# yell/boltzmann-machines

Hardware: AMD Instinct MI355X
Metric: Gibbs-steps/sec (CD-k, 784x1024 RBM, batch 512) (higher is better)
Workload: dtype f32

## Files before the change

### boltzmann_machines_amd/_ffi.py

```python
import ctypes as C
import os

import numpy as np

from . import build as _build

MAX_LAYERS = 4
UNIT_BERNOULLI, UNIT_GAUSSIAN, UNIT_MULTINOMIAL = 0, 1, 2


class Bm355Error(RuntimeError):
    pass


class RbmConfig(C.Structure):
    _fields_ = [('n_visible', C.c_int32), ('n_hidden', C.c_int32), ('v_unit', C.c_int32),
                ('sample_v_states', C.c_int32), ('sample_h_states', C.c_int32),
                ('dbm_first', C.c_int32), ('dbm_last', C.c_int32), ('max_batch', C.c_int32),
                ('l2', C.c_float), ('sparsity_target', C.c_float), ('sparsity_cost', C.c_float),
                ('sparsity_damping', C.c_float), ('dropout', C.c_float),
                ('h_unit', C.c_int32), ('n_samples', C.c_int32)]


class DbmConfig(C.Structure):
# ... 29 lines not shown
    'bm_comm_rank': [_vp, C.POINTER(C.c_int32), C.POINTER(C.c_int32)],
    'bm_rbm_allreduce_grads': [_vp, _vp],
    'bm_rbm_set_grad_slot': [_vp, _i32],
    'bm_rbm_allreduce_grads_async': [_vp, _vp],
    'bm_rbm_wait_grads': [_vp, _i32],
    'bm_dbm_allreduce_grads': [_vp, _vp],
    'bm_xchg_create': [C.c_int32, C.c_int32, _vp, _sz, C.POINTER(_vp)],
    'bm_xchg_blob_bytes': [],
    'bm_xchg_export': [_vp, _vp],
    'bm_xchg_attach': [_vp, _vp],
    'bm_xchg_destroy': [_vp],
    'bm_xchg_allreduce_sum': [_vp, _vp],
    'bm_xchg_allreduce_max1': [_vp, _vp, _vp],
    'bm_xchg_status': [_vp, C.POINTER(C.c_int32)],
    'bm_xchg_info': [_vp, C.POINTER(C.c_int32), C.POINTER(C.c_int32), C.POINTER(_sz)],
    'bm_rbm_xchg_create': [_vp, C.c_int32, C.c_int32, C.POINTER(_vp)],
    'bm_dbm_xchg_create': [_vp, C.c_int32, C.c_int32, C.POINTER(_vp)],
    'bm_rbm_allreduce_grads_direct': [_vp, _vp],
    'bm_dbm_allreduce_grads_direct': [_vp, _vp],
    'bm_rbm_exchange_apply_direct': [_vp, _vp, _i32, C.c_float, C.c_float],
    'bm_rbm_exchange_gather_dw': [_vp, _vp],
    'bm_dbm_exchange_apply_ok': [_vp, _vp, C.POINTER(_i32)],
    'bm_dbm_exchange_apply_direct': [_vp, _vp, _i32, _i32, C.c_float, C.c_float],
    'bm_dbm_exchange_gather_dw': [_vp, _vp],
    'bm_xchg_set_timeout': [_vp, C.c_double],
    'bm_xchg_set_max_workgroups': [_vp, _i32],
    'bm_dbm_set_xchg': [_vp, _vp],
    'bm_dbm_set_fast_binary': [_vp, _i32],
    'bm_dbm_set_ais_literal': [_vp, _i32],
    'bm_dbm_set_sigmoid_literal': [_vp, _i32],
    'bm_rbm_set_fast_binary': [_vp, _i32],
    'bm_rbm64_create': [C.POINTER(RbmConfig), C.POINTER(C.c_double), C.POINTER(_vp)],
    'bm_rbm64_destroy': [_vp],
    'bm_rbm64_sync': [_vp],
    'bm_rbm64_seed': [_vp, C.c_uint64],
    'bm_rbm64_set_row_offset': [_vp, C.c_int64],
    'bm_rbm64_set_param': [_vp, C.c_char_p, _vp, _sz],
    'bm_rbm64_get_param': [_vp, C.c_char_p, _vp, _sz],
    'bm_rbm64_train_step': [_vp, _vp, C.c_int32, C.c_double, C.c_double, C.c_int32],
    'bm_rbm64_train_step_metrics': [_vp, _vp, C.c_int32, C.c_double, C.c_double, C.c_int32, C.POINTER(C.c_double)],
    'bm_rbm64_transform': [_vp, _vp, C.c_int32, C.c_int32, _vp],
    'bm_rbm64_metrics': [_vp, _vp, C.c_int32, C.c_int32, C.POINTER(C.c_double)],
    'bm_rbm64_free_energy': [_vp, _vp, C.c_int32, C.POINTER(C.c_double)],
    'bm_dbm64_create': [C.POINTER(DbmConfig), C.POINTER(C.c_double), C.POINTER(_vp)],
    'bm_dbm64_destroy': [_vp],
    'bm_dbm64_sync': [_vp],
    'bm_dbm64_seed': [_vp, C.c_uint64],
    'bm_dbm64_set_row_offset': [_vp, C.c_int64, C.c_int64],
    'bm_dbm64_set_param': [_vp, C.c_char_p, _vp, _sz],
    'bm_dbm64_get_param': [_vp, C.c_char_p, _vp, _sz],
    'bm_dbm64_train_step': [_vp, _vp, C.c_double, C.c_double, C.c_int32, C.POINTER(C.c_int32), C.POINTER(C.c_double)],
    'bm_dbm64_metrics': [_vp, _vp, C.c_int32, C.POINTER(C.c_int32), C.POINTER(C.c_double)],
    'bm_dbm64_mean_field': [_vp, _vp, _vp, C.POINTER(C.c_int32)],
    'bm_dbm64_reconstruct': [_vp, _vp, _vp],
    'bm_dbm64_sample_v': [_vp, C.c_int32, _vp],
    'bm_dbm64_ais': [_vp, C.c_int32, C.c_int32, C.c_int32, C.c_uint64, C.c_int64, _vp],
    'bm_dbm64_log_proba': [_vp, _vp, _vp],
    'bm_rbm_create': [C.POINTER(RbmConfig), C.POINTER(_vp)],
    'bm_rbm_destroy': [_vp],
    'bm_rbm_sync': [_vp],
    'bm_rbm_set_param': [_vp, C.c_char_p, _vp, _sz],
    'bm_rbm_get_param': [_vp, C.c_char_p, _vp, _sz],
    'bm_rbm_set_param_dev': [_vp, C.c_char_p, _vp, _sz],
    'bm_rbm_dev_ptr': [_vp, C.c_char_p, C.POINTER(_vp), C.POINTER(_sz)],
    'bm_rbm_seed': [_vp, _u64],
    'bm_rbm_set_row_offset': [_vp, _i64],
    'bm_rbm_train_step': [_vp, _vp, _i32, _f32, _f32, _i32],
    'bm_rbm_train_step_metrics': [_vp, _vp, _i32, _f32, _f32, _i32, _fp],
    'bm_rbm_train_step_metrics_async': [_vp, _vp, _i32, _f32, _f32, _i32],
    'bm_rbm_collect_metrics': [_vp, _fp, _i32, C.POINTER(C.c_int32)],
    'bm_rbm_train_epoch': [_vp, _vp, _i64, _i32, _f32, _f32, _i32],
    'bm_rbm_stage': [_vp, _i32],
    'bm_rbm_get_staged': [_vp, _i32, C.c_char_p, _vp, _sz],
    'bm_rbm_grad_step': [_vp, _vp, _i32, _i32],
    'bm_rbm_apply_step': [_vp, _i32, _f32, _f32],
    'bm_rbm_transform': [_vp, _vp, _i32, _i32, _vp],
    'bm_rbm_metrics': [_vp, _vp, _i32, _i32, _fp],
    'bm_rbm_free_energy': [_vp, _vp, _i32, _fp],
    'bm_rbm_gibbs': [_vp, _vp, _vp, _i32, _i32],
    'bm_rbm_stream': [_vp, C.POINTER(_vp)],
    'bm_rbm_profile': [_vp, _i32],
    'bm_rbm_kernel_times': [_vp, _fp, _ip],
    'bm_rbm_chain_stats': [_vp, C.POINTER(C.c_int64)],
    'bm_rbm_timer_start': [_vp],
    'bm_rbm_timer_stop': [_vp, _fp],
    'bm_rbm_timer_mark': [_vp],
    'bm_rbm_timer_elapsed': [_vp, _fp],
    'bm_dbm_create': [C.POINTER(DbmConfig), C.POINTER(_vp)],
    'bm_dbm_destroy': [_vp],
    'bm_dbm_sync': [_vp],
    'bm_dbm_seed': [_vp, _u64],
    'bm_dbm_set_row_offset': [_vp, _i64, _i64],
    'bm_dbm_set_param': [_vp, C.c_char_p, _vp, _sz],
    'bm_dbm_get_param': [_vp, C.c_char_p, _vp, _sz],
    'bm_dbm_dev_ptr': [_vp, C.c_char_p, C.POINTER(_vp), C.POINTER(_sz)],
    'bm_dbm_train_step': [_vp, _vp, _f32, _f32, _i32, _ip, _fp],
    'bm_dbm_metrics': [_vp, _vp, _i32, _ip, _fp],
    'bm_dbm_grad_step': [_vp, _vp, _i32, _ip],
    'bm_dbm_apply_step': [_vp, _i32, _i32, _f32, _f32],
    'bm_dbm_set_mf_allreduce': [_vp, _vp, _vp],
    'bm_dbm_set_comm': [_vp, _vp],
    'bm_dbm_ais_sharded': [_vp, _vp, _i32, _i32, _i32, _u64, _vp],
    'bm_dbm_ais_sharded_direct': [_vp, _vp, _i32, _i32, _i32, _u64, _vp],
    'bm_dbm_stream': [_vp, C.POINTER(_vp)],
    'bm_dbm_mean_field': [_vp, _vp, _vp, _ip],
    'bm_dbm_reconstruct': [_vp, _vp, _vp],
    'bm_dbm_sample_v': [_vp, _i32, _vp],
    'bm_dbm_ais': [_vp, _i32, _i32, _i32, _u64, _i64, _vp],
    'bm_dbm_log_proba': [_vp, _vp, _vp],
    'bm_dbm_timer_start': [_vp],
    'bm_dbm_timer_stop': [_vp, _fp],
    'bm_dbm_timer_mark': [_vp],
    'bm_dbm_timer_elapsed': [_vp, _fp],
}
_RESTYPE = {'bm_last_error': C.c_char_p, 'bm_version': C.c_char_p}
MF_REDUCE_FN = C.CFUNCTYPE(C.c_float, C.c_float, C.c_void_p)

_lib = None


def load(rebuild=True):
    global _lib
    if _lib is not None:
        return _lib
    path = _build.LIB
    if rebuild and _build.needs_build():
        import shutil
        have_hipcc = bool(shutil.which('hipcc')) or os.path.exists('/opt/rocm/bin/hipcc')
        try:
            _build.build()
        except Exception as e:
            if have_hipcc or not os.path.exists(path):
                raise Bm355Error('libbm355.so could not be built from the current sources: %s' % e)
            import warnings
            warnings.warn('libbm355.so is older than its sources and hipcc is not available; using the existing '
                          'library (%s)' % e)
    if not os.path.exists(path):
        raise Bm355Error('libbm355.so not found at %s (run __graft_entry__.build())' % path)
    lib = C.CDLL(path)
    for name, restype in _RESTYPE.items():
        f = getattr(lib, name)
        f.restype = restype
        f.argtypes = []
    for name, argtypes in SIGNATURES.items():
        f = getattr(lib, name)
        f.restype = C.c_int
        f.argtypes = argtypes
    _lib = lib
    return lib


def check(rc):
    if rc != 0:
        raise Bm355Error(load().bm_last_error().decode('utf-8', 'replace'))


def exported_symbols():
    return sorted(list(SIGNATURES) + list(_RESTYPE))


class DeviceArray(object):

    def __init__(self, shape, dtype=np.float32, ptr=None, owner=None):
        self.shape = tuple(int(s) for s in (shape if hasattr(shape, '__iter__') else (shape,)))
        self.dtype = np.dtype(dtype)
        self.nbytes = int(np.prod(self.shape)) * self.dtype.itemsize
# ... 52 lines not shown
```

### boltzmann_machines_amd/csrc/bm_chain.h

```cpp
#pragma once
#include "bm_kernels.h"

namespace bm {

constexpr int CHAIN_MAXPH = 24;
constexpr int CHAIN_MAXTI = 64;
using GeoChain = GeoAct8;

struct ChainPhase {
    Operand P, Q; int K; int p_xm; int I;
    const float *bias, *sigma;
    float mult, bmult; int kind, sample;
    float *means, *states, *negmeans; int ldo;
    PhiloxKey key; long long row0;
};

struct ChainArgs {
    int nph, J, tiles_j, rounds_cap, dbg;
    unsigned gen;
    unsigned *flags;
    unsigned *claim;
    unsigned *claim_zero;
    int *status;
    long long *stamps;
// ... 62 lines not shown
    if (stamps && tid == 0) stamps[2] = wall_clock64();
    (void)act_epilogue<G, 0>(a, key, acc, side, i0, j0);
    if (stamps && tid == 0) stamps[3] = wall_clock64();
}

template <bool COH>
__global__ __launch_bounds__(GeoChain::NT, 1) void act_chain_kernel(ChainArgs c) {
    using G = GeoChain;
    __shared__ __attribute__((aligned(16))) float smem[G::SMEM_FLOATS];
    __shared__ unsigned s_claim;
    const int tid = threadIdx.x;
    unsigned xcc_reg;
    asm volatile("s_getreg_b32 %0, hwreg(HW_REG_XCC_ID)" : "=s"(xcc_reg));
    const int team = (int)(xcc_reg & 7u);
    if ((xcc_reg & 0xfu) > 7u) {
        if (tid == 0) atomicExch(c.status, CHAIN_ERR_XCC);
        return;
    }
    if (blockIdx.x == 0 && tid < 8) c.claim_zero[tid * 32] = 0u;
    unsigned *my_claim = c.claim + team * 32;
    if (tid == 0) s_claim = __hip_atomic_fetch_add(my_claim, 1u, __ATOMIC_RELAXED, __HIP_MEMORY_SCOPE_AGENT);
    __syncthreads();
    int n = (int)s_claim;
    const int T = c.tp0[c.nph];
    const int R = (c.tiles_j - team + 7) >> 3;
    int ntiles = 0;
    while (true) {
        const int r = small_div(n, T);
        if (r >= R) break;
        const int rem = n - r * T;
        int p = 0;
#pragma unroll
        for (int q = 1; q < CHAIN_MAXPH; ++q) p += (q < c.nph && rem >= c.tp0[q]) ? 1 : 0;
        const int ti = rem - c.tp0[p];
        unsigned nxt = 0;
        const ChainPhase &ph = c.ph[p];
        ActArgs a;
        a.P1 = ph.P; a.Q1 = ph.Q; a.K1 = ph.K; a.p_xm = ph.p_xm;
        a.P2 = Operand{nullptr, 0, 0, 0}; a.Q2 = a.P2; a.K2 = 0;
        a.I = ph.I; a.J = c.J;
        a.bias = ph.bias; a.sigma = ph.sigma; a.mult = ph.mult; a.bmult = ph.bmult; a.kind = ph.kind; a.sample = ph.sample;
        a.means = ph.means; a.states = ph.states; a.negmeans = ph.negmeans; a.ldo = ph.ldo;
        a.key = ph.key; a.row0 = ph.row0;
        a.prev = nullptr; a.maxdiff = nullptr; a.maxdiff_blk = nullptr;
        a.rowacc = nullptr; a.beta_a = 0.f; a.beta_b = 0.f; a.rowacc_single = 0; a.rowdot_out = nullptr; a.ld_part = 0;
        a.dot_vec = nullptr; a.dot_mat = nullptr; a.ld_dot = 0;
        a.acc_init = nullptr; a.ld_init = 0; a.skip = nullptr;
        a.chk_ctl = nullptr; a.chk_slots = nullptr; a.chk_n = 0; a.chk_tol = 0.f;
        a.b3 = Bf3Range{}; a.states16 = nullptr; a.ld16 = 0; a.map_xi = 0;
        a.fe_rowacc2 = nullptr; a.fe_flip = nullptr; a.fe_x = nullptr; a.fe_ldx = 0; a.fe_w = nullptr; a.fe_ldw = 0;
        a.fe_zero = nullptr; a.fe_rm = 0; a.fe_key = PhiloxKey{0u, 0u, 0u, 0u};
#ifdef BM_PROBE
        a.dbg = nullptr;
#endif
        unsigned *fl = c.flags + ((size_t)(team * c.rounds_cap + r) * CHAIN_MAXPH) * CHAIN_MAXTI;
        const unsigned *wfl = (p > 0 && !(c.dbg & 2)) ? fl + (size_t)(p - 1) * CHAIN_MAXTI : nullptr;
        const int nwait = p > 0 ? c.tp0[p] - c.tp0[p - 1] : 0;
        const int tj = team + 8 * r;
        long long *stp = c.stamps ? c.stamps + ((size_t)blockIdx.x * 16 + (ntiles < 15 ? ntiles : 15)) * 8 : nullptr;
        if (stp && tid == 0) { stp[0] = wall_clock64(); stp[5] = (long long)p; stp[6] = (long long)ti; stp[7] = (long long)team; }
        if (ph.p_xm) chain_tile<G, XM, COH>(a, ti * G::TI, tj * G::TJ, smem, wfl, nwait, c.gen, c.status, stp, c.dbg & 4, my_claim, nxt);
        else         chain_tile<G, KM, COH>(a, ti * G::TI, tj * G::TJ, smem, wfl, nwait, c.gen, c.status, stp, c.dbg & 4, my_claim, nxt);
        asm volatile("s_waitcnt vmcnt(0)" ::: "memory");
        if (tid == 0) s_claim = nxt;
        wg_barrier();
        if (tid == 0) __hip_atomic_store(fl + (size_t)p * CHAIN_MAXTI + ti, c.gen, __ATOMIC_RELAXED, __HIP_MEMORY_SCOPE_AGENT);
        if (stp && tid == 0) stp[4] = wall_clock64();
        n = (int)s_claim;
        ++ntiles;
    }
    if (tid == 0 && ntiles) atomicAdd(c.status + 1, ntiles);
}

struct ChainState {
    unsigned *flags = nullptr, *claim = nullptr;
    int *status = nullptr;
    int rounds_cap = 0;
    unsigned gen = 0;
    unsigned launches = 0;
    long long tiles_expected = 0;
    bool on = false;
    int mode = -1;
    int ncu = 0;
    std::vector<ActArgs> rec;
    std::vector<Operand> alt_p;
    long long *stamps = nullptr;
    static constexpr int CLAIM_SLOTS = 16;
    static constexpr size_t STAMP_WORDS = 256 * 16 * 8;
    ChainState() = default;
    ChainState(const ChainState &) = delete;
    ChainState &operator=(const ChainState &) = delete;
    ~ChainState() { release(); }
    void release() {
        if (stamps) {
            const char *f = bm::dbg("chain_stamps");
            std::vector<long long> hst(STAMP_WORDS);
            if (f && hipMemcpy(hst.data(), stamps, STAMP_WORDS * 8, hipMemcpyDeviceToHost) == hipSuccess) {
                FILE *fp = fopen(f, "wb");
                if (fp) { fwrite(hst.data(), 8, STAMP_WORDS, fp); fclose(fp); }
            }
            (void)hipFree(stamps); stamps = nullptr;
        }
        if (flags) (void)hipFree(flags);
        if (claim) (void)hipFree(claim);
        if (status) (void)hipFree(status);
        flags = claim = nullptr; status = nullptr;
    }
};

static inline int chain_mode(ChainState &cs) {
    if (cs.mode < 0) {
        const char *e = bm::dbg("chain");
        cs.mode = e ? atoi(e) : 1;
        hipDeviceProp_t pr; int d = 0, nxcc = 0; (void)hipGetDevice(&d);
        const bool have = hipGetDeviceProperties(&pr, d) == hipSuccess;
        cs.ncu = have ? pr.multiProcessorCount : 0;
        if (hipDeviceGetAttribute(&nxcc, hipDeviceAttributeNumberOfXccs, d) != hipSuccess) nxcc = 0;
        const bool arch = have && (strncmp(pr.gcnArchName, "gfx950", 6) == 0 || strncmp(pr.gcnArchName, "gfx942", 6) == 0);
        if (!(arch && nxcc == 8 && cs.ncu == 256)) cs.mode = 0;
    }
    return cs.mode;
}

static inline bool chain_phase_ok(const ActArgs &a) {
    using G = GeoChain;
    if (a.K2 > 0 || a.b3.K1 > 0 || a.prev || a.maxdiff || a.maxdiff_blk || a.rowacc || a.rowdot_out || a.acc_init ||
        a.skip || a.chk_ctl || a.states16 || a.dot_mat || a.fe_flip) return false;
    if (a.kind != 0 && a.kind != 1) return false;
    const int pl = a.p_xm ? XM : KM;
    if (!(operand_fast(a.P1, pl, a.K1) && operand_fast(a.Q1, XM, a.K1))) return false;
    if (a.K1 < G::PF * G::BK) return false;
    if ((a.I + G::TI - 1) / G::TI > CHAIN_MAXTI) return false;
    return true;
}

static inline int chain_flush(ChainState &cs, hipStream_t st, int maxB) {
    cs.on = false;
    std::vector<ActArgs> rec;
    std::vector<Operand> alt;
    rec.swap(cs.rec);
    alt.swap(cs.alt_p);
    if (rec.empty()) return 0;
    alt.resize(rec.size(), Operand{nullptr, 0, 0, 0});
    using G = GeoChain;
    bool ok = chain_mode(cs) > 0 && rec.size() >= (cs.mode == 1 ? 6u : 2u);
    const int J = rec[0].J, tiles_j = (J + G::TJ - 1) / G::TJ;
    for (const ActArgs &a : rec) ok = ok && chain_phase_ok(a) && a.J == J;
    if (ok && cs.mode == 1) {
        ok = tiles_j >= 8;
        for (const ActArgs &a : rec) ok = ok && ((a.I + G::TI - 1) / G::TI) * ((tiles_j + 7) / 8) <= 2 * 32;
    }
    if (!ok) {
        for (size_t i = 0; i < rec.size(); ++i) {
            if (alt[i].ptr) { rec[i].P1 = alt[i]; rec[i].p_xm = 1; }
            launch_act(rec[i], st);
        }
        return 0;
    }
    const int rounds = (tiles_j + 7) / 8;
    if (!cs.flags || rounds > cs.rounds_cap) {
        if (cs.flags) { if (hipStreamSynchronize(st) != hipSuccess) return -1; (void)hipFree(cs.flags); cs.flags = nullptr; }
        const int cap = std::max(rounds, ((maxB + G::TJ - 1) / G::TJ + 7) / 8);
        const size_t nfl = (size_t)8 * cap * CHAIN_MAXPH * CHAIN_MAXTI;
        if (hipMalloc((void **)&cs.flags, nfl * 4) != hipSuccess) return -1;
        if (hipMemsetAsync(cs.flags, 0, nfl * 4, st) != hipSuccess) return -1;
        cs.rounds_cap = cap;
        cs.gen = 0;
        if (!cs.claim) {
            if (hipMalloc((void **)&cs.claim, (size_t)ChainState::CLAIM_SLOTS * 8 * 32 * 4) != hipSuccess) return -1;
            if (hipMemsetAsync(cs.claim, 0, (size_t)ChainState::CLAIM_SLOTS * 8 * 32 * 4, st) != hipSuccess) return -1;
            if (hipMalloc((void **)&cs.status, 2 * sizeof(int)) != hipSuccess) return -1;
            if (hipMemsetAsync(cs.status, 0, 2 * sizeof(int), st) != hipSuccess) return -1;
        }
    }
    for (size_t first = 0; first < rec.size(); first += CHAIN_MAXPH) {
        const int nph = (int)std::min<size_t>(CHAIN_MAXPH, rec.size() - first);
        ChainArgs c;
        memset(&c, 0, sizeof(c));
        c.nph = nph; c.J = J; c.tiles_j = tiles_j; c.rounds_cap = cs.rounds_cap;
        if (++cs.gen == 0) {
            if (hipMemsetAsync(cs.flags, 0, (size_t)8 * cs.rounds_cap * CHAIN_MAXPH * CHAIN_MAXTI * 4, st) != hipSuccess) return -1;
            cs.gen = 1;
        }
        c.gen = cs.gen;
        c.flags = cs.flags;
        c.claim = cs.claim + (size_t)(cs.launches % ChainState::CLAIM_SLOTS) * 8 * 32;
        c.claim_zero = cs.claim + (size_t)((cs.launches + ChainState::CLAIM_SLOTS / 2) % ChainState::CLAIM_SLOTS) * 8 * 32;
        ++cs.launches;
        c.status = cs.status;
        int tiles = 0;
        for (int p = 0; p < nph; ++p) {
            const ActArgs &a = rec[first + p];
            ChainPhase &ph = c.ph[p];
            ph.P = a.P1; ph.Q = a.Q1; ph.K = a.K1; ph.p_xm = a.p_xm; ph.I = a.I;
            ph.bias = a.bias; ph.sigma = a.sigma; ph.mult = a.mult; ph.bmult = a.bmult; ph.kind = a.kind; ph.sample = a.sample;
            ph.means = a.means; ph.states = a.states; ph.negmeans = a.negmeans; ph.ldo = a.ldo;
            ph.key = a.key; ph.row0 = a.row0;
            c.tp0[p] = tiles;
            tiles += (a.I + G::TI - 1) / G::TI;
        }
        for (int p = nph; p <= CHAIN_MAXPH; ++p) c.tp0[p] = tiles;
        cs.tiles_expected += (long long)tiles * tiles_j;
// ... 13 lines not shown
```

### boltzmann_machines_amd/csrc/bm_gemm.h

```cpp
#pragma once
#include <hip/hip_runtime.h>
#include <stdint.h>
#include <stdlib.h>
#include <string.h>

namespace bm {

struct NoSide {
    static constexpr bool kFinalSync = true;
    static constexpr bool kSplitFill = false, kCohQ = false;
    static constexpr bool kCanAbort = false;
    __device__ __forceinline__ void wait_inputs() {}
    __device__ __forceinline__ void post_fill() {}
    __device__ __forceinline__ void fill() {}
    __device__ __forceinline__ void drain() {}
};

#define BM_ABL(bit) ((ABL >> (bit)) & 1)

typedef float f32x4 __attribute__((ext_vector_type(4)));
typedef float f32x2v __attribute__((ext_vector_type(2)));

constexpr int NT = 256;

enum : int { KM = 0, XM = 1 };

template <int WI_, int WJ_, int MI_, int NJ_, int BK_, int NB_ = 4>
struct Geo {
    static constexpr int WI = WI_, WJ = WJ_, MI = MI_, NJ = NJ_, BK = BK_;
    static constexpr int NBUF = NB_;
    static constexpr int PF = NB_ - 1;
    static constexpr int NW = WI * WJ;
    static constexpr int NT = 64 * NW;
    static constexpr int TI = 16 * MI * WI;
    static constexpr int TJ = 16 * NJ * WJ;
    static constexpr int E = 4 * MI;
    static constexpr int P_BUF = TI * BK;
    static constexpr int Q_BUF = TJ * BK;
    static constexpr int SMEM_FLOATS = NBUF * (P_BUF + Q_BUF);
    static constexpr int NPP = P_BUF * 4 / (1024 * NW);
    static constexpr int NPQ = Q_BUF * 4 / (1024 * NW);
    static constexpr int NVP = TI * BK / (4 * NT);
    static constexpr int NVQ = TJ * BK / (4 * NT);
    static constexpr int SP = (MI == 2) ? 8 : 4;
    static constexpr int SQ = (NJ == 2) ? 8 : 4;
    static_assert(MI == 1 || MI == 2, "MI");
    static_assert(NJ == 1 || NJ == 2, "NJ");
    static_assert(BK == 32 || BK == 64, "BK");
    static_assert(NB_ >= 4 && NB_ <= 8, "ring depth");
    static_assert(NPP >= 1 && NPP * 1024 * NW == P_BUF * 4, "P chunk must split into whole DMA pieces per wave");
    static_assert(NPQ >= 1 && NPQ * 1024 * NW == Q_BUF * 4, "Q chunk must split into whole DMA pieces per wave");
    static_assert(NVP >= 1 && NVP * 4 * NT == TI * BK && NVQ >= 1 && NVQ * 4 * NT == TJ * BK, "register path split");
    static_assert(SMEM_FLOATS * 4 <= 160 * 1024 - 1024, "LDS");
};
using GeoAct = Geo<2, 2, 2, 1, 64>;
using GeoAct8 = Geo<2, 4, 1, 1, 64>;
using GeoActS = Geo<2, 2, 1, 1, 64>;
using GeoActS32 = Geo<2, 2, 1, 1, 32>;
using GeoAct32 = Geo<2, 2, 2, 1, 32>;
using GeoGrad = Geo<2, 2, 2, 2, 64>;
using GeoGrad8 = Geo<2, 4, 2, 1, 64>;
using GeoGrad8h = Geo<2, 4, 2, 1, 32>;
using GeoBf3S = Geo<1, 4, 2, 1, 64>;

struct Operand {
    const float *ptr;
    int ld;
    int nx;
    int vec;
};

static inline Operand make_operand(const float *p, int ld, int nx) {
    Operand o;
    o.ptr = p; o.ld = ld; o.nx = nx;
    o.vec = (((uintptr_t)p & 15u) == 0 && (ld & 3) == 0) ? 1 : 0;
    return o;
}

static inline bool operand_fast(const Operand &o, int layout, int K) {
    if (!o.ptr) return true;
    if (!o.vec) return false;
    return layout == KM ? (o.nx % 4 == 0 && o.nx >= 4) : (K % 4 == 0);
}

template <int BK> __device__ __forceinline__ int fx(int row) { return (BK == 64) ? (row & 15) : ((row >> 1) & 7); }
template <int S> __device__ __forceinline__ int fk(int row) { return S * ((row >> 2) & 1); }

template <int L, int TX, int BK, int S>
__device__ __forceinline__ int img_off(int row, int c4) {
    return (L == XM) ? row * BK + ((c4 ^ fx<BK>(row)) << 2) : row * TX + ((c4 ^ fk<S>(row)) << 2);
}

__device__ __forceinline__ float4 load4_guard(const float *p, bool row_ok, int col, int ncols, bool vec) {
    float4 v = make_float4(0.f, 0.f, 0.f, 0.f);
// ... 143 lines not shown
            const float q = f.q[kk][n];
#pragma unroll
            for (int t = 0; t < G::MI; ++t) {
                if (BM_ABL(1)) { acc[t][n][0] += f.p[kk][t] * q; continue; }
                acc[t][n] = __builtin_amdgcn_mfma_f32_16x16x4f32(f.p[kk][t], q, acc[t][n], 0, 0, 0);
            }
        }
    }
}

template <class G, int ABL = 0>
__device__ __forceinline__ void mfma_frags_head(f32x4 (&acc)[G::MI][G::NJ], const Frags<G> &f, int nq) {
#pragma unroll
    for (int q = 0; q < G::BK / 16; ++q) {
        if (q < nq) {
#pragma unroll
            for (int kk = 4 * q; kk < 4 * q + 4; ++kk) {
#pragma unroll
                for (int n = 0; n < G::NJ; ++n) {
                    const float qv = f.q[kk][n];
#pragma unroll
                    for (int t = 0; t < G::MI; ++t) {
                        if (BM_ABL(1)) { acc[t][n][0] += f.p[kk][t] * qv; continue; }
                        acc[t][n] = __builtin_amdgcn_mfma_f32_16x16x4f32(f.p[kk][t], qv, acc[t][n], 0, 0, 0);
                    }
                }
            }
        }
    }
}

template <class G> struct ChunkRegs {
    float4 p[G::NVP];
    float4 q[G::NVQ];
};

struct KRange {
    Operand P1, Q1; int K1;
    Operand P2, Q2; int K2;
};

__device__ __forceinline__ int sel_i(int a, int b, int m) { return a ^ ((a ^ b) & m); }
__device__ __forceinline__ const float *sel_p(const float *a, const float *b, int m) {
    const uintptr_t ua = (uintptr_t)a, ub = (uintptr_t)b;
    return (const float *)(ua ^ ((ua ^ ub) & (uintptr_t)(intptr_t)m));
}

template <class G, int DW = G::NW> struct DmaPlan {
    static constexpr int NPP = G::P_BUF / (256 * DW), NPQ = G::Q_BUF / (256 * DW);
    uint32_t p[NPP], q[NPQ];
};

template <int L, int TX, int BK, int NW, int NP, int S>
__device__ __forceinline__ void plan_offsets(uint32_t (&off)[NP], int ld, int nx, int x0, int wave, int lane) {
    constexpr int RC = (L == KM) ? TX / 4 : BK / 4;
    constexpr int R = 64 / RC;
#pragma unroll
    for (int n = 0; n < NP; ++n) {
        const int pc = wave + n * NW;
        const int row = pc * R + lane / RC, slot = lane % RC;
        if (L == KM) {
            const int c4 = slot ^ fk<S>(row);
            off[n] = (uint32_t)(row * ld + min(x0 + c4 * 4, nx - 4)) * 4u;
        } else {
            const int c4 = slot ^ fx<BK>(row);
            off[n] = (uint32_t)(min(x0 + row, nx - 1) * ld + c4 * 4) * 4u;
        }
    }
}

template <int QL, class G, int PL = KM, int DW = G::NW>
__device__ __forceinline__ void make_plan(DmaPlan<G, DW> &pl, const Operand &P, const Operand &Q, int i0, int j0, int wave, int lane) {
    plan_offsets<PL, G::TI, G::BK, DW, DmaPlan<G, DW>::NPP, G::SP>(pl.p, P.ld, P.nx, i0, wave, lane);
    plan_offsets<QL, G::TJ, G::BK, DW, DmaPlan<G, DW>::NPQ, G::SQ>(pl.q, Q.ld, Q.nx, j0, wave, lane);
}

__device__ __forceinline__ void dma16(const char *src, float *lds_dst) {
    unsigned keep;
    const unsigned lds_addr = (unsigned)(uintptr_t)(__attribute__((address_space(3))) void *)lds_dst;
    asm volatile("s_mov_b32 %0, m0\n\ts_mov_b32 m0, %2\n\ts_nop 0\n\tglobal_load_lds_dwordx4 %1, off\n\ts_mov_b32 m0, %0"
                 : "=&s"(keep) : "v"(src), "s"(__builtin_amdgcn_readfirstlane(lds_addr)) : "memory");
}

__device__ __forceinline__ void dma16s(const void *sbase, uint32_t voff, unsigned lds_byte) {
    asm volatile("s_mov_b32 m0, %2\n\ts_nop 0\n\tglobal_load_lds_dwordx4 %1, %0"
                 :: "s"(sbase), "v"(voff), "s"(lds_byte) : "memory");
}
__device__ __forceinline__ void dma16s_coh(const void *sbase, uint32_t voff, unsigned lds_byte) {
    asm volatile("s_mov_b32 m0, %2\n\ts_nop 0\n\tglobal_load_lds_dwordx4 %1, %0 sc1"
                 :: "s"(sbase), "v"(voff), "s"(lds_byte) : "memory");
}
template <class G, int DW, bool QSC = false, bool QHALF = false>
__device__ __forceinline__ void dma_chunk_s(const DmaPlan<G, DW> &pl, const char *pb, const char *qb, unsigned ldsP, unsigned ldsQ) {
#pragma unroll
    for (int n = 0; n < DmaPlan<G, DW>::NPP; ++n) dma16s(pb, pl.p[n], ldsP + (unsigned)(n * DW * 1024));
#pragma unroll
    for (int n = 0; n < DmaPlan<G, DW>::NPQ; ++n) {
        if (QHALF && (n & 1)) continue;
        if (QSC) dma16s_coh(qb, pl.q[n], ldsQ + (unsigned)(n * DW * 1024));
        else     dma16s(qb, pl.q[n], ldsQ + (unsigned)(n * DW * 1024));
    }
}

template <int QL, class G, bool SEG2, int PL = KM, int DW = G::NW, bool QHALF = false>
__device__ __forceinline__ void dma_chunk(const KRange &kr, const DmaPlan<G, DW> &pl1, const DmaPlan<G, DW> &pl2, int nch1, int c,
                                          float *sP, float *sQ, int wave) {
    constexpr int BK = G::BK;
    const int m = SEG2 ? -(int)(c >= nch1) : 0;
    const int kc = c - (nch1 & m);
    const int ldp = SEG2 ? sel_i(kr.P1.ld, kr.P2.ld, m) : kr.P1.ld;
    const int ldq = SEG2 ? sel_i(kr.Q1.ld, kr.Q2.ld, m) : kr.Q1.ld;
    const char *pb = (const char *)((SEG2 ? sel_p(kr.P1.ptr, kr.P2.ptr, m) : kr.P1.ptr) +
                                    ((PL == KM) ? (size_t)kc * BK * ldp : (size_t)kc * BK));
    const char *qb = (const char *)((SEG2 ? sel_p(kr.Q1.ptr, kr.Q2.ptr, m) : kr.Q1.ptr) +
                                    ((QL == KM) ? (size_t)kc * BK * ldq : (size_t)kc * BK));
#pragma unroll
    for (int n = 0; n < DmaPlan<G, DW>::NPP; ++n) {
        const uint32_t o1 = pl1.p[n], o2 = SEG2 ? pl2.p[n] : 0u;
        const uint32_t o = SEG2 ? (o1 ^ ((o1 ^ o2) & (uint32_t)m)) : o1;
        dma16(pb + o, sP + (wave + n * DW) * 256);
    }
#pragma unroll
    for (int n = 0; n < DmaPlan<G, DW>::NPQ; ++n) {
        if (QHALF && (n & 1)) continue;
        const uint32_t o1 = pl1.q[n], o2 = SEG2 ? pl2.q[n] : 0u;
        const uint32_t o = SEG2 ? (o1 ^ ((o1 ^ o2) & (uint32_t)m)) : o1;
        dma16(qb + o, sQ + (wave + n * DW) * 256);
    }
}

template <int QL, class G, bool FAST, bool SEG2, int PL = KM, bool COHQ = false>
__device__ __forceinline__ void load_chunk(ChunkRegs<G> &r, const KRange &kr, int nch1, int i0, int j0, int c, int tid) {
    constexpr int BK = G::BK;
    if (!SEG2) {
        g2r<PL, G::TI, BK, G::NT, FAST>(r.p, kr.P1.ptr, kr.P1.ld, kr.P1.nx, kr.P1.vec, i0, c * BK, kr.K1, tid);
        g2r<QL, G::TJ, BK, G::NT, FAST, COHQ>(r.q, kr.Q1.ptr, kr.Q1.ld, kr.Q1.nx, kr.Q1.vec, j0, c * BK, kr.K1, tid);
    } else {
        const int m = -(int)((c >= nch1) & (kr.K2 > 0));
        const int kc = c - (nch1 & m);
        const int K = sel_i(kr.K1, kr.K2, m);
        g2r<PL, G::TI, BK, G::NT, FAST>(r.p, sel_p(kr.P1.ptr, kr.P2.ptr, m), sel_i(kr.P1.ld, kr.P2.ld, m),
                                        sel_i(kr.P1.nx, kr.P2.nx, m), sel_i(kr.P1.vec, kr.P2.vec, m), i0, kc * BK, K, tid);
        g2r<QL, G::TJ, BK, G::NT, FAST, COHQ>(r.q, sel_p(kr.Q1.ptr, kr.Q2.ptr, m), sel_i(kr.Q1.ld, kr.Q2.ld, m),
                                              sel_i(kr.Q1.nx, kr.Q2.nx, m), sel_i(kr.Q1.vec, kr.Q2.vec, m), j0, kc * BK, K, tid);
    }
}

template <int QL, class G, bool SEG2, int PL = KM>
__device__ __forceinline__ void store_chunk(const ChunkRegs<G> &r, const KRange &kr, int nch1, int c,
                                            float *sP, float *sQ, int tid) {
    constexpr int BK = G::BK;
    const int m = SEG2 ? -(int)((c >= nch1) & (kr.K2 > 0)) : 0;
    const int kz = sel_i(kr.K1, kr.K2, m) - (c - (nch1 & m)) * BK;
    r2s<PL, G::TI, BK, G::NT, G::SP>(r.p, sP, tid, kz);
    r2s<QL, G::TJ, BK, G::NT, G::SQ>(r.q, sQ, tid, kz);
}

template <class G> struct RegPlan {
    uint32_t p[G::NVP], q[G::NVQ];
};
template <int L, int TX, int BK, int NTH>
__device__ __forceinline__ void reg_offsets(uint32_t (&off)[TX * BK / (4 * NTH)], int ld, int nx, int x0, int tid) {
    constexpr int NV = TX * BK / (4 * NTH);
    constexpr int RC = (L == KM) ? TX / 4 : BK / 4;
#pragma unroll
    for (int n = 0; n < NV; ++n) {
        const int f = tid + n * NTH;
        const int row = f / RC, c4 = f % RC;
        off[n] = (L == KM) ? (uint32_t)(row * ld + min(x0 + c4 * 4, nx - 4)) * 4u
                           : (uint32_t)(min(x0 + row, nx - 1) * ld + c4 * 4) * 4u;
    }
}
template <int QL, class G, int PL = KM>
__device__ __forceinline__ void make_reg_plan(RegPlan<G> &pl, const Operand &P, const Operand &Q, int i0, int j0, int tid) {
    reg_offsets<PL, G::TI, G::BK, G::NT>(pl.p, P.ld, P.nx, i0, tid);
    reg_offsets<QL, G::TJ, G::BK, G::NT>(pl.q, Q.ld, Q.nx, j0, tid);
}
template <int QL, class G, bool SEG2, int PL = KM>
__device__ __forceinline__ void load_chunk_slim(ChunkRegs<G> &r, const KRange &kr, const RegPlan<G> &pl1,
                                                const RegPlan<G> &pl2, int nch1, int c) {
    constexpr int BK = G::BK;
    const int m = SEG2 ? -(int)(c >= nch1) : 0;
    const int kc = c - (nch1 & m);
    const int ldp = SEG2 ? sel_i(kr.P1.ld, kr.P2.ld, m) : kr.P1.ld;
    const int ldq = SEG2 ? sel_i(kr.Q1.ld, kr.Q2.ld, m) : kr.Q1.ld;
    const char *pb = (const char *)((SEG2 ? sel_p(kr.P1.ptr, kr.P2.ptr, m) : kr.P1.ptr) +
                                    ((PL == KM) ? (size_t)kc * BK * ldp : (size_t)kc * BK));
    const char *qb = (const char *)((SEG2 ? sel_p(kr.Q1.ptr, kr.Q2.ptr, m) : kr.Q1.ptr) +
                                    ((QL == KM) ? (size_t)kc * BK * ldq : (size_t)kc * BK));
#pragma unroll
    for (int n = 0; n < G::NVP; ++n) {
        const uint32_t o1 = pl1.p[n], o2 = SEG2 ? pl2.p[n] : 0u;
        const uint32_t o = SEG2 ? (o1 ^ ((o1 ^ o2) & (uint32_t)m)) : o1;
        r.p[n] = *reinterpret_cast<const float4 *>(pb + o);
    }
#pragma unroll
    for (int n = 0; n < G::NVQ; ++n) {
        const uint32_t o1 = pl1.q[n], o2 = SEG2 ? pl2.q[n] : 0u;
        const uint32_t o = SEG2 ? (o1 ^ ((o1 ^ o2) & (uint32_t)m)) : o1;
        r.q[n] = *reinterpret_cast<const float4 *>(qb + o);
    }
}
template <int QL, class G, int PL = KM>
__device__ __forceinline__ void store_chunk_slim(const ChunkRegs<G> &r, float *sP, float *sQ, int tid) {
    r2s<PL, G::TI, G::BK, G::NT, G::SP, false>(r.p, sP, tid, 0);
    r2s<QL, G::TJ, G::BK, G::NT, G::SQ, false>(r.q, sQ, tid, 0);
}

enum : int { STG_DMA = 0, STG_REG = 1, STG_DMAH = 2 };

#define BM_WAIT_VM(n) asm volatile("s_waitcnt vmcnt(%0)" ::"n"(n) : "memory")
template <int NPW, int MAXC>
__device__ __forceinline__ void wait_vm_chunks(int n) {
    static_assert(MAXC * NPW <= 63, "vmcnt range");
    if (MAXC >= 4 && n >= 4)      BM_WAIT_VM(4 * NPW <= 63 ? 4 * NPW : 0);
    else if (MAXC >= 3 && n == 3) BM_WAIT_VM(3 * NPW <= 63 ? 3 * NPW : 0);
    else if (MAXC >= 2 && n == 2) BM_WAIT_VM(2 * NPW <= 63 ? 2 * NPW : 0);
    else if (n == 1)              BM_WAIT_VM(NPW);
    else                          BM_WAIT_VM(0);
}
__device__ __forceinline__ void wg_barrier() {
    asm volatile("s_waitcnt lgkmcnt(0)" ::: "memory");
    __builtin_amdgcn_s_barrier();
    asm volatile("" ::: "memory");
}

template <int QL, class G, bool FAST, bool SEG2, int ABL = 0, int PL = KM, int STG = STG_DMA, class Side = NoSide>
__device__ __forceinline__ void mainloop(f32x4 (&acc)[G::MI][G::NJ], const KRange &kr, int i0, int j0, float *smem,
                                         Side &side, long long *stamps = nullptr) {
#ifdef BM_PROBE
#define BM_MSTAMP(n) do { if (stamps && threadIdx.x == 0) stamps[n] = (long long)__builtin_readcyclecounter(); } while (0)
#else
#define BM_MSTAMP(n) do {} while (0)
#endif
    constexpr int BK = G::BK, P_BUF = G::P_BUF, Q_BUF = G::Q_BUF, NBUF = G::NBUF, PF = G::PF;
    constexpr int DW = (STG == STG_DMAH && G::NW == 8) ? 4 : G::NW;
    constexpr int NPW = DmaPlan<G, DW>::NPP + (BM_ABL(9) ? (DmaPlan<G, DW>::NPQ + 1) / 2 : DmaPlan<G, DW>::NPQ);
    const int tid = threadIdx.x, lane = tid & 63;
    const int w = __builtin_amdgcn_readfirstlane(tid >> 6);
    const int wi = w % G::WI, wj = w / G::WI;
    float *sP = smem, *sQ = smem + NBUF * P_BUF;
    const int nch1 = (kr.K1 + BK - 1) / BK;
    const int nch = nch1 + (SEG2 ? (kr.K2 + BK - 1) / BK : 0);
    const int nfull1 = kr.K1 / BK, nfull2 = SEG2 ? kr.K2 / BK : 0;
    auto is_full = [&](int c) -> bool {
        return (c < nfull1) | (SEG2 && c >= nch1 && c - nch1 < nfull2);
    };
    auto is_dma = [&](int c) -> bool {
        if (!FAST || STG == STG_REG || BM_ABL(6)) return false;
        return is_full(c);
    };
    ChunkRegs<G> gr;
    Frags<G> fa, fb;
    DmaPlan<G, DW> pl1, pl2;
    RegPlan<G> rp1, rp2;
    const bool dmaw = (DW == G::NW) || w < DW;
    ChunkRegs<G> g0, g1;
    if (FAST && STG != STG_REG && dmaw) {
        make_plan<QL, G, PL, DW>(pl1, kr.P1, kr.Q1, i0, j0, w, lane);
        if (SEG2) make_plan<QL, G, PL, DW>(pl2, kr.P2, kr.Q2, i0, j0, w, lane);
    }
    int n_reg = 0;
    if (FAST && STG == STG_REG && !BM_ABL(6) && !BM_ABL(0)) {
        while (n_reg + 4 < nch && is_full(n_reg + 4) && is_full(n_reg + 2)) ++n_reg;
        n_reg &= ~1;
        if (n_reg > 0 && !(is_full(0) && is_full(1) && is_full(2) && is_full(3))) n_reg = 0;
        if (n_reg > 0) {
            make_reg_plan<QL, G, PL>(rp1, kr.P1, kr.Q1, i0, j0, tid);
            if (SEG2) make_reg_plan<QL, G, PL>(rp2, kr.P2, kr.Q2, i0, j0, tid);
        }
    }
    BM_MSTAMP(0);
    if (n_reg > 0) {
        ChunkRegs<G> ga, gb;
        load_chunk_slim<QL, G, SEG2, PL>(ga, kr, rp1, rp2, nch1, 0);
        load_chunk_slim<QL, G, SEG2, PL>(gb, kr, rp1, rp2, nch1, 1);
        load_chunk_slim<QL, G, SEG2, PL>(g0, kr, rp1, rp2, nch1, 2);
        load_chunk_slim<QL, G, SEG2, PL>(g1, kr, rp1, rp2, nch1, 3);
        __builtin_amdgcn_sched_barrier(0);
        side.fill();
        __builtin_amdgcn_sched_barrier(0);
        store_chunk_slim<QL, G, PL>(ga, sP, sQ, tid);
        store_chunk_slim<QL, G, PL>(gb, sP + P_BUF, sQ + Q_BUF, tid);
    } else if constexpr (Side::kSplitFill) {
        static_assert(FAST && STG == STG_DMA && DW == G::NW, "chained fill");
        const unsigned l0 = (unsigned)(uintptr_t)(__attribute__((address_space(3))) void *)smem;
        const unsigned lP = l0 + (unsigned)w * 1024u, lQ = l0 + (unsigned)(NBUF * P_BUF * 4) + (unsigned)w * 1024u;
#pragma unroll
        for (int c = 0; c < PF; ++c) {
            const char *pb = (const char *)kr.P1.ptr + (size_t)c * ((PL == KM) ? (size_t)BK * kr.P1.ld * 4 : (size_t)BK * 4);
#pragma unroll
            for (int n = 0; n < DmaPlan<G, DW>::NPP; ++n) dma16s(pb, pl1.p[n], lP + (unsigned)(c * P_BUF * 4 + n * DW * 1024));
        }
        __builtin_amdgcn_sched_barrier(0);
        side.fill();
        __builtin_amdgcn_sched_barrier(0);
        side.wait_inputs();
#pragma unroll
        for (int c = 0; c < PF; ++c) {
            const char *qb = (const char *)kr.Q1.ptr + (size_t)c * ((QL == KM) ? (size_t)BK * kr.Q1.ld * 4 : (size_t)BK * 4);
#pragma unroll
            for (int n = 0; n < DmaPlan<G, DW>::NPQ; ++n) dma16s_coh(qb, pl1.q[n], lQ + (unsigned)(c * Q_BUF * 4 + n * DW * 1024));
        }
        constexpr int NQ_LEFT = (PF - 2) * DmaPlan<G, DW>::NPQ;
        BM_WAIT_VM(NQ_LEFT);
    } else {
#pragma unroll
        for (int c = 0; c < PF; ++c)
            if (c < nch && is_dma(c) && dmaw && !BM_ABL(0))
                dma_chunk<QL, G, SEG2, PL, DW, (BM_ABL(9) != 0)>(kr, pl1, pl2, nch1, c, sP + (c % NBUF) * P_BUF, sQ + (c % NBUF) * Q_BUF, w);
        __builtin_amdgcn_sched_barrier(0);
        side.fill();
        __builtin_amdgcn_sched_barrier(0);
#pragma unroll
        for (int c = 0; c < 2; ++c)
            if (c < nch && !is_dma(c) && !BM_ABL(0)) {
                load_chunk<QL, G, FAST, SEG2, PL>(gr, kr, nch1, i0, j0, c, tid);
                store_chunk<QL, G, SEG2, PL>(gr, kr, nch1, c, sP + (c % NBUF) * P_BUF, sQ + (c % NBUF) * Q_BUF, tid);
            }
        {
            int n_after = 0;
#pragma unroll
            for (int c = 2; c < PF; ++c) n_after += (c < nch && is_dma(c) && !BM_ABL(0)) ? 1 : 0;
            wait_vm_chunks<NPW, PF - 2>(n_after);
        }
    }
    BM_MSTAMP(1);
    if (!BM_ABL(5)) wg_barrier();
    if constexpr (Side::kCanAbort) {
        side.post_fill();
        if (side.aborted) { BM_WAIT_VM(0); return; }
    }
    read_frags<QL, G, ABL, PL>(fa, sP, sQ, wi, wj, lane);
    BM_MSTAMP(2);
    const int klast = (SEG2 && kr.K2 > 0) ? kr.K2 - (nch - nch1 - 1) * BK : kr.K1 - (nch1 - 1) * BK;
    const int nq_last = (klast + 15) / 16;
    constexpr int NM = (BK / 4) * G::MI * G::NJ;
    constexpr int NRP = (PL == XM) ? BK / 16 : BK / 4;
    constexpr int NRQ = (QL == XM) ? (BK / 16) * G::NJ : BK / 4;
    constexpr int NR = NRP + NRQ;
#define BM_SG(mask, n) __builtin_amdgcn_sched_group_barrier(mask, n, 0);
#ifndef BM_SCHED_VARIANT
#define BM_SCHED_VARIANT 0
#endif
#if BM_SCHED_VARIANT == 0
#define BM_SCHED_STEP                                                                             \
    if (DW == G::NW) { _Pragma("unroll") for (int s_ = 0; s_ < NPW; ++s_) { BM_SG(0x008, 1) BM_SG(0x020, 1) } } \
    _Pragma("unroll") for (int s_ = 0; s_ < NR; ++s_) { BM_SG(0x008, 1) BM_SG(0x100, 1) }         \
    BM_SG(0x008, NM)
#elif BM_SCHED_VARIANT == 1
#define BM_SCHED_STEP                                                                             \
    _Pragma("unroll") for (int s_ = 0; s_ < NR; ++s_) { BM_SG(0x008, 1) BM_SG(0x100, 1) }         \
    _Pragma("unroll") for (int s_ = 0; s_ < NPW; ++s_) { BM_SG(0x008, 1) BM_SG(0x020, 1) }        \
    BM_SG(0x008, NM)
#else
#define BM_SCHED_STEP
#endif
    static_assert(NBUF == 4, "the steps below are written for a 4-slot ring");
    int cc = 0;
    const unsigned lds0 = (unsigned)(uintptr_t)(__attribute__((address_space(3))) void *)smem;
    const unsigned ldsPw = lds0 + (unsigned)w * 1024u, ldsQw = lds0 + (unsigned)(NBUF * P_BUF * 4) + (unsigned)w * 1024u;
    bool in2 = false;
    auto chunk_bases = [&](int c, const char *&pb, const char *&qb) {
        const bool s2 = SEG2 && c >= nch1;
        const Operand &P = s2 ? kr.P2 : kr.P1, &Q = s2 ? kr.Q2 : kr.Q1;
        const int kc = s2 ? c - nch1 : c;
        pb = (const char *)P.ptr + (size_t)kc * ((PL == KM) ? (size_t)BK * P.ld * 4 : (size_t)BK * 4);
        qb = (const char *)Q.ptr + (size_t)kc * ((QL == KM) ? (size_t)BK * Q.ld * 4 : (size_t)BK * 4);
    };
#define BM_DMA_AT(CD, SD)                                                                         \
    {                                                                                             \
        if (SEG2 && !in2 && (CD) >= nch1) { in2 = true; pl1 = pl2; }                              \
        const char *pb_, *qb_;                                                                    \
        chunk_bases((CD), pb_, qb_);                                                              \
        if (dmaw) dma_chunk_s<G, DW, Side::kCohQ, (BM_ABL(9) != 0)>(pl1, pb_, qb_, ldsPw + (unsigned)((SD) * P_BUF * 4), \
                                     ldsQw + (unsigned)((SD) * Q_BUF * 4));                       \
    }
#define BM_STEP_Q(FC, FN, S)                                                                      \
    {                                                                                             \
        BM_DMA_AT(cc + PF, ((S) + PF) % NBUF)                                                     \
        read_frags<QL, G, ABL, PL>(FN, sP + (((S) + 1) % NBUF) * P_BUF, sQ + (((S) + 1) % NBUF) * Q_BUF, wi, wj, lane); \
        mfma_frags<G, ABL>(acc, FC);                                                              \
        BM_SCHED_STEP                                                                             \
        if (!BM_ABL(8)) BM_WAIT_VM((PF - 2) * NPW);                                               \
        if (!BM_ABL(5)) wg_barrier();                                                             \
        ++cc;                                                                                     \
    }
#define BM_STEP_T(FC, FN, S1, S2, S3)       \
    {                                                                                             \
        const int cd = cc + PF, cr = cc + 2;                                                      \
        const bool do_dma = cd < nch && is_dma(cd) && !BM_ABL(0);                                 \
        const bool do_reg = cr < nch && !is_dma(cr) && !BM_ABL(0);                                \
        if (cc == last - 1) side.drain();       \
        if (do_reg) load_chunk<QL, G, FAST, SEG2, PL, Side::kCohQ>(gr, kr, nch1, i0, j0, cr, tid); \
        if (do_dma) BM_DMA_AT(cd, S3)                                                             \
        read_frags<QL, G, ABL, PL>(FN, sP + (S1) * P_BUF, sQ + (S1) * Q_BUF, wi, wj, lane);       \
        mfma_frags<G, ABL>(acc, FC);                                                              \
        _Pragma("unroll") for (int s_ = 0; s_ < NR; ++s_) { BM_SG(0x008, 1) BM_SG(0x100, 1) }     \
        BM_SG(0x008, NM)                                                                          \
        if (do_reg) {                                                                             \
            BM_WAIT_VM(0);                                                                        \
            store_chunk<QL, G, SEG2, PL>(gr, kr, nch1, cr, sP + (S2) * P_BUF, sQ + (S2) * Q_BUF, tid); \
        } else if (cr < nch) {                                                                    \
             \
            int n_after = 0;                                                                      \
            _Pragma("unroll") for (int c_ = 3; c_ <= PF; ++c_) n_after += (cc + c_ < nch && is_dma(cc + c_) && !BM_ABL(0)) ? 1 : 0; \
            wait_vm_chunks<NPW, PF - 2>(n_after);                                                 \
        }                                                                                         \
        if (!BM_ABL(5)) wg_barrier();                                                             \
        ++cc;                                                                                     \
    }
#define BM_STEP_TC(FC, FN, S) BM_STEP_T(FC, FN, ((S) + 1) % NBUF, ((S) + 2) % NBUF, ((S) + 3) % NBUF)
#define BM_STEP_TR(FC, FN)    BM_STEP_T(FC, FN, (cc + 1) % NBUF, (cc + 2) % NBUF, (cc + 3) % NBUF)
    constexpr int NWR = G::NVP + G::NVQ;
#ifndef BM_REG_SCHED_VARIANT
#define BM_REG_SCHED_VARIANT 0
#endif
#if BM_REG_SCHED_VARIANT == 0
#define BM_REG_SCHED(RELOAD)                                                                      \
        _Pragma("unroll") for (int s_ = 0; s_ < NWR; ++s_) { BM_SG(0x008, 1) BM_SG(0x200, 1) }    \
        if (RELOAD) { _Pragma("unroll") for (int s_ = 0; s_ < NWR; ++s_) { BM_SG(0x008, 1) BM_SG(0x020, 1) } } \
        _Pragma("unroll") for (int s_ = 0; s_ < NR; ++s_) { BM_SG(0x008, 1) BM_SG(0x100, 1) }     \
        BM_SG(0x008, NM)
#elif BM_REG_SCHED_VARIANT == 1
#define BM_REG_SCHED(RELOAD)                                                                      \
        _Pragma("unroll") for (int s_ = 0; s_ < NR; ++s_) { BM_SG(0x008, (NM >= 64 ? 2 : 1)) BM_SG(0x100, 2) } \
        _Pragma("unroll") for (int s_ = 0; s_ < NWR; ++s_) { BM_SG(0x008, (NM >= 32 ? 2 : 1)) BM_SG(0x200, 1) } \
        if (RELOAD) { _Pragma("unroll") for (int s_ = 0; s_ < NWR; ++s_) { BM_SG(0x008, 1) BM_SG(0x020, 1) } } \
        BM_SG(0x008, NM)
#else
#define BM_REG_SCHED(RELOAD)
#endif
#define BM_STEP_REG(FC, FN, G_, RELOAD, S)                                                        \
    {                                                                                             \
        store_chunk_slim<QL, G, PL>(G_, sP + (((S) + 2) % NBUF) * P_BUF, sQ + (((S) + 2) % NBUF) * Q_BUF, tid); \
        if (RELOAD) load_chunk_slim<QL, G, SEG2, PL>(G_, kr, rp1, rp2, nch1, cc + 4);             \
        read_frags<QL, G, ABL, PL>(FN, sP + (((S) + 1) % NBUF) * P_BUF, sQ + (((S) + 1) % NBUF) * Q_BUF, wi, wj, lane); \
        mfma_frags<G, ABL>(acc, FC);                                                              \
        BM_REG_SCHED(RELOAD)                                                                      \
        if (!BM_ABL(5)) wg_barrier();                                                             \
        ++cc;                                                                                     \
    }
    if (n_reg > 0) {
        int left = n_reg;
#pragma unroll 1
        while (left >= 4) {
            BM_STEP_REG(fa, fb, g0, true, 0)
            BM_STEP_REG(fb, fa, g1, true, 1)
            BM_STEP_REG(fa, fb, g0, true, 2)
            BM_STEP_REG(fb, fa, g1, true, 3)
            left -= 4;
        }
        if (left == 2) {
            BM_STEP_REG(fa, fb, g0, true, 0)
            BM_STEP_REG(fb, fa, g1, true, 1)
            BM_STEP_REG(fa, fb, g0, false, 2)
            BM_STEP_REG(fb, fa, g1, false, 3)
        } else {
            BM_STEP_REG(fa, fb, g0, false, 0)
            BM_STEP_REG(fb, fa, g1, false, 1)
        }
    }
    int n_steady = 0;
    if (FAST && STG != STG_REG && !BM_ABL(6) && !BM_ABL(0))
        while (n_steady + PF < nch) {
            bool all = true;
#pragma unroll
            for (int c_ = 2; c_ <= PF; ++c_) all = all && is_dma(n_steady + c_);
            if (!all) break;
            ++n_steady;
        }
#pragma unroll 1
    for (int q = 0; q < n_steady / 4; ++q) {
        BM_STEP_Q(fa, fb, 0)
        BM_STEP_Q(fb, fa, 1)
        BM_STEP_Q(fa, fb, 2)
        BM_STEP_Q(fb, fa, 3)
// ... 170 lines not shown
```

### boltzmann_machines_amd/csrc/bm_kernels.h

```cpp
#pragma once
#include <stdio.h>
#include <stdlib.h>
#include <string.h>
#include "bm_gemm.h"
#include "bm_bf3.h"
#include "bm_numerics.h"
#include "bm_rng.h"

namespace bm {

struct MfCtl { unsigned maxdiff; int done; int steps; float resid; };

struct ActArgs {
    Operand P1, Q1; int K1;
    int p_xm;
    Operand P2, Q2; int K2;
    int I, J;
    const float *bias;
    const float *sigma;
    float mult;
    float bmult;
    int kind;
    int sample;
    int lit;
// ... 44 lines not shown
    uint32_t w[4];
    philox_block(key, idx >> 2, w);
    return (int)(w[idx & 3] % (uint32_t)V);
}
#define FE_FLIP_FROM_KEY (reinterpret_cast<const int *>(uintptr_t(1)))
constexpr int BM_MF_SLOTS = 1024;

__device__ __forceinline__ void draw4(const ActArgs &a, const PhiloxKey &key, unsigned long long flat, int ib, int nvalid,
                                      const float *m, float *s, bool aligned) {
    if (aligned) {
        uint32_t wds[4];
        philox_block(key, flat >> 2, wds);
        if (a.kind == 0) {
#pragma unroll
            for (int r = 0; r < 4; ++r) s[r] = (u32_to_uniform(wds[r]) < m[r]) ? 1.f : 0.f;
        } else {
            float n[4];
            box_muller(wds[0], wds[1], n[0], n[1]);
            box_muller(wds[2], wds[3], n[2], n[3]);
#pragma unroll
            for (int r = 0; r < 4; ++r) s[r] = n[r] * a.sigma[ib + r] + m[r];
        }
    } else {
#pragma unroll
        for (int r = 0; r < 4; ++r) {
            if (r >= nvalid) break;
            const unsigned long long idx = flat + r;
            uint32_t wds[4];
            philox_block(key, idx >> 2, wds);
            if (a.kind == 0) {
                s[r] = (u32_to_uniform(wds[idx & 3]) < m[r]) ? 1.f : 0.f;
            } else {
                float n0, n1;
                const int pr = (int)(idx & 3) >> 1;
                box_muller(wds[2 * pr], wds[2 * pr + 1], n0, n1);
                s[r] = ((idx & 1) ? n1 : n0) * a.sigma[ib + r] + m[r];
            }
        }
    }
}

#ifndef BM_NT_STORES
#define BM_NT_STORES 1
#endif
typedef float f32x2 __attribute__((ext_vector_type(2)));
__device__ __forceinline__ void stream_store4(float *p, float x, float y, float z, float w) {
    if (BM_NT_STORES) __builtin_nontemporal_store((f32x4){x, y, z, w}, reinterpret_cast<f32x4 *>(p));
    else *reinterpret_cast<float4 *>(p) = make_float4(x, y, z, w);
}
__device__ __forceinline__ void stream_store2(float *p, float x, float y) {
    if (BM_NT_STORES) __builtin_nontemporal_store((f32x2){x, y}, reinterpret_cast<f32x2 *>(p));
    else *reinterpret_cast<float2 *>(p) = make_float2(x, y);
}

template <bool CACHED = false>
__device__ __forceinline__ void store4(float *dst, size_t o, const float *v, int nvalid, bool v4) {
    if (v4) {
        if (CACHED) *reinterpret_cast<float4 *>(dst + o) = make_float4(v[0], v[1], v[2], v[3]);
        else stream_store4(dst + o, v[0], v[1], v[2], v[3]);
    } else {
#pragma unroll
        for (int r = 0; r < 4; ++r) if (r < nvalid) dst[o + r] = v[r];
    }
}

template <int MI> struct PhiloxFor { typedef PhiloxPair type; };
template <> struct PhiloxFor<1> { typedef PhiloxOne type; };

__device__ __forceinline__ float wave_max_lane63(float v) {
#define BM_DPP_MAX(ctrl, rmask) v = fmaxf(v, __int_as_float(__builtin_amdgcn_update_dpp(__float_as_int(v), __float_as_int(v), ctrl, rmask, 0xf, false)))
    BM_DPP_MAX(0xb1, 0xf);
    BM_DPP_MAX(0x4e, 0xf);
    BM_DPP_MAX(0x124, 0xf);
    BM_DPP_MAX(0x128, 0xf);
    BM_DPP_MAX(0x142, 0xa);
    BM_DPP_MAX(0x143, 0xc);
#undef BM_DPP_MAX
    return v;
}

template <int E, class Rng, bool MF = false, int NTH = 256> struct ActSide {
    static constexpr bool kFinalSync = false;
    static constexpr bool kSplitFill = false, kCohQ = false, kCanAbort = MF;
    static constexpr bool kMF = MF;
    const float *bias, *sigma;
    const float *prev_row;
    int ib0, I, with_rng;
    float bs[E], sg[E], pv[E];
    Rng rng;
    MfCtl *chk_ctl; const float *chk_slots; int chk_n; float chk_tol; const int *skip; float *s_chk; int aborted, nthreads;

    __device__ __forceinline__ void load_inputs() {
        const float *sp = sigma ? sigma : bias;
        const bool has_sigma = sigma != nullptr;
        if (MF && prev_row) {
            if (E == 4 && ib0 + 3 < I && (((uintptr_t)prev_row & 15u) == 0)) {
                const float4 t = *reinterpret_cast<const float4 *>(prev_row);
                pv[0] = t.x; pv[1] = t.y; pv[2] = t.z; pv[E - 1] = t.w;
            } else {
#pragma unroll
                for (int e = 0; e < E; ++e) pv[e] = (ib0 + e < I) ? prev_row[e] : 0.f;
            }
        }
        if (MF && E == 4 && ib0 + 3 < I && (((uintptr_t)(bias + ib0) & 15u) == 0) && (((uintptr_t)(sp + ib0) & 15u) == 0)) {
            const float4 b = *reinterpret_cast<const float4 *>(bias + ib0), v = *reinterpret_cast<const float4 *>(sp + ib0);
            bs[0] = b.x; bs[1] = b.y; bs[2] = b.z; bs[E - 1] = b.w;
            sg[0] = has_sigma ? v.x : 1.0f; sg[1] = has_sigma ? v.y : 1.0f; sg[2] = has_sigma ? v.z : 1.0f; sg[E - 1] = has_sigma ? v.w : 1.0f;
            return;
        }
#pragma unroll
        for (int e = 0; e < E; ++e) {
            const int i = (ib0 + e < I) ? ib0 + e : I - 1;
            bs[e] = bias[i];
            const float sv = sp[i];
            sg[e] = has_sigma ? sv : 1.0f;
        }
    }
    static constexpr int CHK_MAX = 4096;
    float *s_slots;
    static __device__ __forceinline__ void dma4_lane0(const void *src, float *lds_dst) {
        if ((threadIdx.x & 63) == 0) {
            unsigned keep;
            const unsigned lds_addr = (unsigned)(uintptr_t)(__attribute__((address_space(3))) void *)lds_dst;
            asm volatile("s_mov_b32 %0, m0\n\ts_mov_b32 m0, %2\n\ts_nop 0\n\tglobal_load_lds_dword %1, off\n\ts_mov_b32 m0, %0"
                         : "=&s"(keep) : "v"(src), "s"(__builtin_amdgcn_readfirstlane(lds_addr)) : "memory");
        }
    }
    __device__ __forceinline__ void preload() {
        if constexpr (MF) {
            load_inputs();
            aborted = 0;
            const int w = threadIdx.x >> 6, lane = threadIdx.x & 63;
            if (chk_ctl) {
                for (int p = w; p * 256 < chk_n && p * 256 < CHK_MAX; p += nthreads / 64)
                    dma16(reinterpret_cast<const char *>(chk_slots + 256 * p) + 16 * lane, s_slots + 256 * p);
                if (w == 0) dma4_lane0(&chk_ctl->done, s_slots + CHK_MAX);
            } else if (skip) {
                if (w == 0) dma4_lane0(skip, s_slots + CHK_MAX);
            }
        }
    }
    __device__ __forceinline__ void fill() {
        if (!MF) load_inputs();
        if (with_rng) rng.fill();
    }
    __device__ __forceinline__ void post_fill() {
        if constexpr (MF) {
            if (chk_ctl) {
                constexpr int NR = CHK_MAX / (4 * NTH);
                f32x4 v[NR];
#pragma unroll
                for (int q = 0; q < NR; ++q) {
                    const int e = 4 * ((int)threadIdx.x + q * NTH);
                    v[q] = *reinterpret_cast<const f32x4 *>(s_slots + (e < chk_n ? e : 0));
                }
                float m = 0.f;
#pragma unroll
                for (int q = 0; q < NR; ++q) {
                    const bool in = 4 * ((int)threadIdx.x + q * NTH) < chk_n;
                    m = fmaxf(m, in ? fmaxf(fmaxf(v[q][0], v[q][1]), fmaxf(v[q][2], v[q][3])) : 0.f);
                }
                m = wave_max_lane63(m);
                if ((threadIdx.x & 63) == 63) s_chk[threadIdx.x >> 6] = m;
                wg_barrier();
                m = 0.f;
#pragma unroll
// ... 433 lines not shown
                    a.u.vb[c] = a.u.vb[c] + d;
                }
            }
        }
    } else {
        const int c0 = (wv - nv) * 64;
        block_colsum(a.h0m, a.ldh0, a.hm, a.ldh, c0, a.u.H, a.B, true, smem, s1, s2, a.hm_negated != 0);
        if ((lane & 15) == 0) {
#pragma unroll
            for (int r = 0; r < 4; ++r) {
                const int h = c0 + w * 16 + g * 4 + r;
                if (h < a.u.H) {
                    const float sq = s2[r];
                    a.raw_tail[a.u.V + h] = s1[r];
                    a.raw_tail[a.u.V + a.u.H + h] = sq;
                    if (a.raw_only) continue;
                    const float qn = a.u.damping * a.u.q[h] + (1.0f - a.u.damping) * sq;
                    a.u.q[h] = qn;
                    const float pen = a.u.cost * (qn - a.u.target);
                    a.u.pen[h] = pen;
                    float gr = s1[r] / a.u.N;
                    gr = gr - pen;
                    const float d = a.u.lr * (a.u.mom * a.u.dhb[h] + gr);
                    a.u.dhb[h] = d;
                    a.u.hb[h] = a.u.hb[h] + d;
                }
            }
        }
    }
}

__global__ __launch_bounds__(NT) void rbm_bias_fused_kernel(RbmBiasFusedArgs a) {
    __shared__ __attribute__((aligned(16))) float smem[CS_SMEM_FLOATS];
    rbm_bias_fused_block(a, blockIdx.x, smem);
}

struct GradArgs {
    Operand Ppos, Qpos; int Kpos;
    Operand Pneg, Qneg; int Kneg;
    int I, J;
    int form;
    int fused;
    float *raw;
    float *raw2;
    float *W, *dW;
    float *Wt;
    int ldw, ldwt;
    const float *pen;
    float N, M, l2, lr, mom;
    int nbias;
    RbmBiasFusedArgs bias;
    int fetch_at_fill;
    int map_xi;
#ifdef BM_PROBE
    long long *dbg;
#endif
};

__device__ __forceinline__ void apply_w_update(float g, float pen, float l2, float lr, float mom,
                                               float &w, float &dw) {
    g = __fsub_rn(g, __fmul_rn(l2, w));
    g = __fsub_rn(g, pen);
    const float d = __fmul_rn(lr, __fadd_rn(__fmul_rn(mom, dw), g));
    dw = d;
    w = __fadd_rn(w, d);
}
__device__ __forceinline__ bool grad_pow2(float N) { return ((__float_as_uint(N) & 0x007fffffu) == 0u) && N >= 1.0f; }
__device__ __forceinline__ float grad_norm1(float r, float N, float invN, bool pow2) {
    return pow2 ? __fmul_rn(r, invN) : __fdiv_rn(r, N);
}
__device__ __forceinline__ float grad_norm2(float r, float r2, float N, float M, float invN, float invM, bool pow2) {
    return pow2 ? __fsub_rn(__fmul_rn(r, invN), __fmul_rn(r2, invM)) : __fsub_rn(__fdiv_rn(r, N), __fdiv_rn(r2, M));
}

struct DivBy {
    float n, inv; bool pow2;
    __device__ __forceinline__ explicit DivBy(float N) : n(N), inv(1.0f / N),
        pow2(grad_pow2(N)) {}
};

template <int NJ> struct GradSide {
    static constexpr bool kFinalSync = true;
    static constexpr bool kSplitFill = false, kCohQ = false, kCanAbort = false;
    const float *W, *dW; int ldw, I, J, ib0, jb[NJ]; bool on, vec8;
    float4 w[NJ][2], d[NJ][2];
    bool at_fill;
    __device__ __forceinline__ void fill() { if (at_fill) fetch(); }
    __device__ __forceinline__ void drain() { if (!at_fill) fetch(); }
    __device__ __forceinline__ void fetch() {
        if (!on || ib0 >= I) return;
#pragma unroll
        for (int n = 0; n < NJ; ++n) {
            if (jb[n] >= J) continue;
            const size_t o = (size_t)jb[n] * ldw + ib0;
            if (vec8) {
                w[n][0] = *reinterpret_cast<const float4 *>(W + o);  w[n][1] = *reinterpret_cast<const float4 *>(W + o + 4);
                d[n][0] = *reinterpret_cast<const float4 *>(dW + o); d[n][1] = *reinterpret_cast<const float4 *>(dW + o + 4);
            } else {
                float tw[8], td[8];
#pragma unroll
                for (int e = 0; e < 8; ++e) {
                    const bool ok = ib0 + e < I;
                    tw[e] = ok ? W[o + e] : 0.f;
                    td[e] = ok ? dW[o + e] : 0.f;
                }
                w[n][0] = make_float4(tw[0], tw[1], tw[2], tw[3]); w[n][1] = make_float4(tw[4], tw[5], tw[6], tw[7]);
                d[n][0] = make_float4(td[0], td[1], td[2], td[3]); d[n][1] = make_float4(td[4], td[5], td[6], td[7]);
            }
        }
    }
};

template <class G, bool FAST, int ABL = 0, int STG = STG_DMA, int MINB = 1>
__global__ __launch_bounds__(G::NT, MINB) void grad_kernel(GradArgs a, TileMap tmap) {
    constexpr int TI = G::TI, NJ = G::NJ;
    static_assert(G::MI == 2 && G::TI == 64 && G::TJ == 64, "grad_kernel: 64 x 64 tiles, 8 consecutive outputs per lane");
    __shared__ __attribute__((aligned(16))) float smem[G::SMEM_FLOATS];
    constexpr bool kBias = G::SMEM_FLOATS >= CS_SMEM_FLOATS;
    static_assert(G::NT >= NT, "bias path");
    const int ntile_blocks = (int)gridDim.x - a.nbias;
    if ((int)blockIdx.x >= ntile_blocks) {
        if constexpr (kBias) {
            if (G::NT > NT && threadIdx.x >= NT) return;
            rbm_bias_fused_block(a.bias, (int)blockIdx.x - ntile_blocks, smem);
        }
        return;
    }
    asm volatile("" :: "s"(a.Ppos.ptr), "s"(a.Qpos.ptr), "s"(a.Ppos.ld), "s"(a.Qpos.ld), "s"(a.Ppos.nx), "s"(a.Qpos.nx),
                       "s"(a.Pneg.ptr), "s"(a.Qneg.ptr), "s"(a.Pneg.ld), "s"(a.Qneg.ld), "s"(a.Kpos), "s"(a.Kneg),
                       "s"(a.I), "s"(a.J), "s"(a.W), "s"(a.dW), "s"(a.ldw), "s"(a.form), "s"(a.fused));
    constexpr int TJ2 = G::TJ;
    int ti, tj;
    if (tmap.slab) {
        block_to_tile((a.J + TJ2 - 1) / TJ2, ti, tj, 0, a.nbias);
    } else {
        TILE_WORDS(tmap, (int)blockIdx.x);
        TILE_OF_BLOCK(tmap, (int)blockIdx.x, ntile_blocks, ti, tj);
    }
    const int i0 = ti * TI, j0 = tj * TJ2;
    const int tid = threadIdx.x, lane = tid & 63, w = tid >> 6;
    const int wi = w % G::WI, wj = w / G::WI;
    const int g = lane >> 4, l15 = lane & 15;
    const int ib0 = i0 + wi * 32 + g * 8;

#ifdef BM_PROBE
#define BM_GSTAMP(n) do { if (a.dbg && threadIdx.x == 0) a.dbg[blockIdx.x * 4 + (n)] = (long long)__builtin_readcyclecounter(); } while (0)
#else
#define BM_GSTAMP(n) do {} while (0)
#endif
    BM_GSTAMP(0);
    f32x4 pos[2][NJ], neg[2][NJ];
#pragma unroll
    for (int t = 0; t < 2; ++t)
#pragma unroll
        for (int n = 0; n < NJ; ++n) pos[t][n] = neg[t][n] = (f32x4){0.f, 0.f, 0.f, 0.f};
    GradSide<NJ> side;
    side.W = a.W; side.dW = a.dW; side.ldw = a.ldw; side.I = a.I; side.J = a.J; side.ib0 = ib0;
#pragma unroll
    for (int n = 0; n < NJ; ++n) side.jb[n] = j0 + wj * (16 * NJ) + lane_j<KM, G>(l15, n);
    side.vec8 = (ib0 + 7 < a.I) && ((a.ldw & 3) == 0);
    side.at_fill = true;
    side.on = a.fused != 0 && a.fetch_at_fill != 0;
    KRange kr;
    kr.P1 = a.Ppos; kr.Q1 = a.Qpos; kr.K1 = a.Kpos;
    if (a.form == 0) {
        kr.P2 = a.Pneg; kr.Q2 = a.Qneg; kr.K2 = a.Kneg;
        mainloop<KM, G, FAST, true, ABL, KM, STG>(pos, kr, i0, j0, smem, side);
    } else {
        kr.P2 = a.Ppos; kr.Q2 = a.Qpos; kr.K2 = 0;
        mainloop<KM, G, FAST, false, 0, KM, STG>(pos, kr, i0, j0, smem, side);
        kr.P1 = a.Pneg; kr.Q1 = a.Qneg; kr.K1 = a.Kneg;
        mainloop<KM, G, FAST, false, 0, KM, STG>(neg, kr, i0, j0, smem, side);
    }

    BM_GSTAMP(1);
    if (ib0 >= a.I) return;
    if (!a.fetch_at_fill) { side.on = a.fused != 0; side.fetch(); }
    const DivBy divN(a.N), divM(a.M);
    float wt[NJ][8];
    bool jok[NJ];
#pragma unroll
    for (int n = 0; n < NJ; ++n) {
        const int j = side.jb[n];
        jok[n] = j < a.J;
        if (!jok[n]) continue;
        float pv[8], nv[8];
        lane_outputs<G>(pos, n, pv);
        lane_outputs<G>(neg, n, nv);
        const size_t o = (size_t)j * a.ldw + ib0;
        if (!a.fused) {
#pragma unroll
            for (int e = 0; e < 8; ++e) {
                if (ib0 + e >= a.I) break;
                a.raw[o + e] = pv[e];
                if (a.form != 0) a.raw2[o + e] = nv[e];
            }
            continue;
        }
        float wv[8] = {side.w[n][0].x, side.w[n][0].y, side.w[n][0].z, side.w[n][0].w, side.w[n][1].x, side.w[n][1].y, side.w[n][1].z, side.w[n][1].w};
        float dv[8] = {side.d[n][0].x, side.d[n][0].y, side.d[n][0].z, side.d[n][0].w, side.d[n][1].x, side.d[n][1].y, side.d[n][1].z, side.d[n][1].w};
        float pe[8];
#pragma unroll
        for (int e = 0; e < 8; ++e) pe[e] = (a.pen && ib0 + e < a.I) ? a.pen[ib0 + e] : 0.f;
        float gr[8];
        if (divN.pow2 && divM.pow2) {
#pragma unroll
            for (int e = 0; e < 8; ++e) gr[e] = (a.form == 0) ? grad_norm1(pv[e], a.N, divN.inv, true)
                                                              : grad_norm2(pv[e], nv[e], a.N, a.M, divN.inv, divM.inv, true);
        } else {
#pragma unroll
            for (int e = 0; e < 8; ++e) gr[e] = (a.form == 0) ? grad_norm1(pv[e], a.N, 0.f, false)
                                                              : grad_norm2(pv[e], nv[e], a.N, a.M, 0.f, 0.f, false);
        }
#pragma unroll
        for (int e = 0; e < 8; ++e) {
            apply_w_update(gr[e], pe[e], a.l2, a.lr, a.mom, wv[e], dv[e]);
            wt[n][e] = wv[e];
        }
        if (side.vec8) {
            stream_store4(a.W + o, wv[0], wv[1], wv[2], wv[3]);
            stream_store4(a.W + o + 4, wv[4], wv[5], wv[6], wv[7]);
            stream_store4(a.dW + o, dv[0], dv[1], dv[2], dv[3]);
            stream_store4(a.dW + o + 4, dv[4], dv[5], dv[6], dv[7]);
        } else {
#pragma unroll
            for (int e = 0; e < 8; ++e)
                if (ib0 + e < a.I) { a.W[o + e] = wv[e]; a.dW[o + e] = dv[e]; }
        }
    }
    if (a.fused && a.Wt) {
        const int ja = side.jb[0];
        const bool pair = NJ == 2 && jok[0] && jok[NJ - 1] && ((a.ldwt & 1) == 0);
#pragma unroll
        for (int e = 0; e < 8; ++e) {
            if (ib0 + e >= a.I) break;
            float *dst = a.Wt + (size_t)(ib0 + e) * a.ldwt + ja;
            if (pair) {
                stream_store2(dst, wt[0][e], wt[NJ - 1][e]);
            } else {
// ... 739 lines not shown
```

### boltzmann_machines_amd/csrc/bm_launch.h

```cpp
#pragma once
#include <array>
#include <map>
#include <mutex>
#include "bm_common.h"

namespace bm {

template <class G> static inline int tile_grid(int I, int J) { return ((I + G::TI - 1) / G::TI) * ((J + G::TJ - 1) / G::TJ); }

static inline int device_cu_count() {
    static const int n = [] {
        hipDeviceProp_t pr;
        int d = 0;
        (void)hipGetDevice(&d);
        return (hipGetDeviceProperties(&pr, d) == hipSuccess && pr.multiProcessorCount > 0) ? pr.multiProcessorCount : 256;
    }();
    return n;
}
static inline int dbg_int(const char *name) { const char *e = dbg(name); return e ? atoi(e) : 0; }

constexpr int XI_MODEL = 0, XI_SLAB = -1;
struct Tuned { int geo = 0; int xi = XI_MODEL; };
constexpr int TUNE_REP = 4, TUNE_ROUNDS = 3;
constexpr float NOT_TIMED = 1e30f;
// ... 224 lines not shown
static inline void launch_act_bf3(const ActArgs &a, hipStream_t st) {
    static const int geo_env = dbg_int("bf3_geo");
    if (geo_env) { launch_act_bf3_as(geo_env, a, st); return; }
    static TuneMemo<5> memo;
    const long long flags = (long long)((a.sample ? 1 : 0) | (a.kind << 1) | (a.rowacc ? 32 : 0) | (a.rowdot_out ? 256 : 0) |
                                        (a.dot_mat ? 512 : 0) | (a.states ? 1024 : 0) | (a.means ? 2048 : 0));
    const Tuned T = memo.get({a.I, a.J, a.b3.K1, a.b3.K2, flags}, [&] { return tune_bf3_shape(a, st, flags); });
    launch_act_bf3_as(T.geo, a, st);
}
static inline void launch_act_f32(const ActArgs &a, hipStream_t st) {
    static const int geo_env = dbg_int("act_geo");
    const int ov = geo_env ? geo_env : a.geo_hint;
    if (ov) { launch_act_as(ov, a, st); return; }
    static TuneMemo<5> memo;
    const long long flags = (long long)((a.sample ? 1 : 0) | (a.kind << 1) | (a.prev ? 16 : 0) | (a.rowacc ? 32 : 0) |
                                        (a.acc_init ? 64 : 0) | (a.p_xm ? 128 : 0) | (a.rowdot_out ? 256 : 0) |
                                        (a.dot_mat ? 512 : 0) | (a.negmeans ? 1024 : 0));
    const Tuned T = memo.get({a.I, a.J, a.K1, a.K2, flags}, [&] { return tune_act_shape(a, st, flags); });
    if (T.xi != XI_MODEL && !a.map_xi) {
        ActArgs a2 = a;
        a2.map_xi = T.xi;
        launch_act_as(T.geo, a2, st);
        return;
    }
    launch_act_as(T.geo, a, st);
}
static inline void launch_act(const ActArgs &a, hipStream_t st) {
    if (a.b3.K1 > 0) { launch_act_bf3(a, st); return; }
    if (a.fe_flip) { launch_act_fe(a, st); return; }
    if (a.prev || a.maxdiff || a.skip || a.chk_ctl || a.acc_init) { launch_act_mf(a, st); return; }
    if (a.lit && a.kind == 0) { launch_act_lit(a, st); return; }
    launch_act_f32(a, st);
    if (a.states16 && a.states)
        hipLaunchKernelGGL(shadow16_kernel, dim3(256), dim3(256), 0, st, (const float *)a.states, a.ldo, a.J, a.I, a.states16, a.ld16);
}

template <class G, int STG, int MINB = 1>
static inline void launch_grad_geo(const GradArgs &g, hipStream_t st) {
    const double kt = (double)g.Kpos + (double)g.Kneg;
    const TileMap tmap = make_tile_map((g.I + G::TI - 1) / G::TI, (g.J + G::TJ - 1) / G::TJ, kt * G::TI * 4.0, kt * G::TJ * 4.0, g.map_xi);
    const bool fast = operand_fast(g.Ppos, KM, g.Kpos) && operand_fast(g.Qpos, KM, g.Kpos) &&
                      operand_fast(g.Pneg, KM, g.Kneg) && operand_fast(g.Qneg, KM, g.Kneg);
    const dim3 grid(tile_grid<G>(g.I, g.J) + g.nbias), blk(G::NT);
    if (fast) hipLaunchKernelGGL((grad_kernel<G, true, 0, STG, MINB>), grid, blk, 0, st, g, tmap);
    else      hipLaunchKernelGGL((grad_kernel<G, false, 0, STG_DMA, MINB>), grid, blk, 0, st, g, tmap);
}
static inline void launch_grad_as(int geo, const GradArgs &g, hipStream_t st) {
    if (geo == 9 && g.nbias == 0) launch_grad_geo<GeoGrad8h, STG_DMA, 4>(g, st);
    else if (geo == 9)   launch_grad_geo<GeoGrad8, STG_DMA>(g, st);
    else if (geo == 208) launch_grad_geo<GeoGrad8, STG_DMAH>(g, st);
    else if (geo == 108) launch_grad_geo<GeoGrad8, STG_REG>(g, st);
    else if (geo == 104) launch_grad_geo<GeoGrad, STG_REG>(g, st);
    else if (geo == 8)   launch_grad_geo<GeoGrad8, STG_DMA>(g, st);
    else                 launch_grad_geo<GeoGrad, STG_DMA>(g, st);
}
static inline Tuned tune_grad_shape(const GradArgs &g, hipStream_t st) {
    constexpr int NC = 5;
    static const int cand[NC] = {4, 8, 104, 108, 9};
    Tuned T;
    T.geo = 4;
    const size_t mat = (((size_t)g.J * (size_t)g.ldw) + 3) & ~(size_t)3;
    float *s = tune_scratch(4 * mat);
    if (!s) return T;
    GradArgs t = g;
    t.nbias = 0; t.pen = nullptr; t.Wt = nullptr;
    t.W = s; t.dW = s + mat; t.raw = s + 2 * mat; t.raw2 = s + 3 * mat;
    (void)hipMemsetAsync(s, 0, 4 * mat * sizeof(float), st);
#ifdef BM_PROBE
    t.dbg = nullptr;
#endif
    TuneTimer tm;
    if (!tm.init(st)) return T;
    float us[NC], xi_us[5];
    best_of(tm, TUNE_ROUNDS, TUNE_REP, NC, us, [&](int c) { launch_grad_as(cand[c], t, st); });
    const int b = fastest(us, NC);
    if (b >= 0) T.geo = cand[b];
    T.xi = tune_tile_map(tm, t, xi_us, [&] { launch_grad_as(T.geo, t, st); });
    if (tune_log())
        fprintf(stderr, "bm355 tune: grad I=%d J=%d K=%d+%d form=%d fused=%d -> geometry %d (us, dma: 4w %.1f, 8w %.1f; reg: 4w %.1f, 8w %.1f; 8w bk32 x2: %.1f), "
                        "tile map %d (9 slab, else XCD grid xi; us: slab %.1f, 8x1 %.1f, 4x2 %.1f, 2x4 %.1f, 1x8 %.1f)\n",
                g.I, g.J, g.Kpos, g.Kneg, g.form, g.fused, T.geo, us[0], us[1], us[2], us[3], us[4], T.xi == XI_SLAB ? 9 : T.xi, xi_us[4], xi_us[0], xi_us[1], xi_us[2], xi_us[3]);
    return T;
}
static inline void launch_grad(const GradArgs &g_in, hipStream_t st) {
    static const int fetch_env = std::max(0, dbg_int("grad_fetch")), geo_env = dbg_int("grad_geo");
    GradArgs g = g_in;
    g.fetch_at_fill = fetch_env;
    if (geo_env) { launch_grad_as(geo_env, g, st); return; }
    static TuneMemo<6> memo;
    const Tuned T = memo.get({g.I, g.J, g.Kpos, g.Kneg, g.form | (g.fused << 1), g.ldw}, [&] { return tune_grad_shape(g, st); });
    if (T.xi != XI_MODEL && !g.map_xi) g.map_xi = T.xi;
    launch_grad_as(T.geo, g, st);
}

static inline void launch_fe_hidden(const FeArgs &f, hipStream_t st) {
    const bool fast = operand_fast(f.P, KM, f.K) && operand_fast(f.Q, XM, f.K);
    const dim3 grid(tile_grid<GeoAct>(f.I, f.J)), blk(NT);
    if (fast) hipLaunchKernelGGL((fe_hidden_kernel<true>), grid, blk, 0, st, f);
    else      hipLaunchKernelGGL((fe_hidden_kernel<false>), grid, blk, 0, st, f);
}

static inline void launch_apply_w(const ApplyWArgs &a, const RbmBiasArgs *bias, hipStream_t st) {
    const bool tiled = (a.I % 4 == 0) && (a.ldw % 4 == 0) && (!a.Wt || a.ldwt % 4 == 0);
    if (tiled) {
        RbmBiasArgs b;
        memset(&b, 0, sizeof(b));
        int nb = 0;
        if (bias) { b = *bias; nb = (b.V + b.H + 255) / 256; }
        const int ntile = ((a.I + 63) / 64) * ((a.J + 63) / 64);
        hipLaunchKernelGGL(apply_w_tiled_kernel, dim3(ntile + nb), dim3(256), 0, st, a, b, nb);
    } else {
        if (bias) hipLaunchKernelGGL(rbm_bias_kernel, dim3((bias->V + bias->H + 255) / 256), dim3(256), 0, st, *bias);
        hipLaunchKernelGGL(apply_w_kernel, dim3(1024), dim3(256), 0, st, a);
    }
}

}
```

### boltzmann_machines_amd/csrc/bm_rbm.hip

```cpp
#include "../../include/bm355.h"
#include "bm_common.h"
#include "bm_kernels.h"
#include "bm_chain.h"

#include <math.h>
#include <atomic>
#include <memory>

namespace bm {

static thread_local char g_err[1024] = "";
void set_error(const char *fmt, ...) {
    va_list ap;
    va_start(ap, fmt);
    vsnprintf(g_err, sizeof(g_err), fmt, ap);
    va_end(ap);
}

enum : uint32_t { SITE_DROPOUT = 1, SITE_H0 = 2, SITE_V = 3, SITE_H = 4, SITE_PLL = 5, SITE_FE = 6 };

}

using namespace bm;

struct bm_xchg;
static int xchg_check_status(bm_xchg *x);
static void xchg_bind_user(bm_xchg *x, bm_xchg **slot);
static void xchg_dw_replaced(bm_xchg *x);

struct bm_rbm {
    bm_rbm_config cfg;
    bm_xchg *xchg_used = nullptr;
    bool dw_sharded = false;
    int V, H, maxB;
    Stream stream;
    Stream comm_stream;
    Stream stage_stream;
    Event ev0, ev1;
    Mat W, dW;
    Mat Wt;
    bool use_wt = false, wt_valid = false;
    DevBuf vb, hb, dvb, dhb, q, sigma;
    Mat h0m, h0s, hm, hs, hneg;
    Mat vm, vs, Xs, Xd;
    DevBuf grad;
    DevBuf grad_alt;
    int grad_slot = 0;
    Event ev_ready[2], ev_reduced[2];
    DevBuf pen;
    DevBuf rowacc;
    DevBuf hhat;
    DevArray<int> flip;
    DevArray<double> scal;
    bool multinomial() const { return cfg.h_unit == BM_UNIT_MULTINOMIAL; }
    uint64_t seed = 0;
    uint32_t call = 0;
    int64_t row0 = 0;
    const float *Xin = nullptr;
    int Xin_ld = 0;
    bool hm_is_neg = false;
    bool fe_in_chain = false;
    DevBuf fe_part;
    int fast = 0;
    bool fast_now = false;
    Mat16 W3, W3t, hs16, vs16;
    DevArray<int> nonbinary;
    struct Stage { Mat W, dW; DevBuf vb, hb, dvb, dhb, q, sigma; Event ev; bool ready = false;
                   std::atomic<int> readers{0}; } stage[2];
    int last_stage = -1;
    Pinned<float> stage_host;
    int device = 0;
    static constexpr int MRING = 4096;
    Pinned<double> mring;
    double *mring_dev = nullptr;
    std::vector<int> mring_B;
    int mring_n = 0;
    Event ev_mlast;
    bool prof = false;
    struct Rec { int cls; Event a, b; };
    std::vector<Rec> recs;
    size_t grad_tail() const { return (size_t)V * W.ld; }
    ChainState chain;
};

enum { KC_UP = 0, KC_DOWN = 1, KC_GRAD = 2, KC_COLSUM = 3, KC_BIAS = 4, KC_OTHER = 5 };

static int check_dw(const bm_rbm *h, const char *what) {
    BM_CHECK(!h->dw_sharded, "%s: after bm_rbm_exchange_apply_direct this rank holds only its slice of the momentum buffer dW; "
             "every rank must call bm_rbm_exchange_gather_dw first (DirectExchange.gather_dw())", what);
    return 0;
}

struct ProfScope {
    bm_rbm *h; hipEvent_t b = nullptr;
    ProfScope(bm_rbm *h_, int cls) : h(h_) {
        if (!h->prof) return;
        bm_rbm::Rec r{cls};
        (void)create(r.a); (void)create(r.b);
        (void)hipEventRecord(r.a, h->stream);
        b = r.b;
        h->recs.push_back(std::move(r));
    }
    ~ProfScope() { if (b) (void)hipEventRecord(b, h->stream); }
};

static PhiloxKey make_key(const bm_rbm *h, uint32_t site, int t) {
    PhiloxKey k;
    k.k0 = (uint32_t)h->seed;
    k.k1 = (uint32_t)(h->seed >> 32);
    k.site = site + 16u * (uint32_t)t;
    k.call = h->call;
    return k;
}

static void act_pass(bm_rbm *h, const ActArgs &a, const Operand *alt_p = nullptr) {
    if (h->chain.on) {
        h->chain.rec.push_back(a);
        h->chain.alt_p.resize(h->chain.rec.size(), Operand{nullptr, 0, 0, 0});
        if (alt_p) h->chain.alt_p.back() = *alt_p;
    } else if (alt_p) {
        ActArgs b = a;
        b.P1 = *alt_p; b.p_xm = 1;
        launch_act(b, h->stream);
    } else launch_act(a, h->stream);
}
static void chain_begin(bm_rbm *h) {
    h->chain.on = !h->prof && !h->multinomial() && !h->fast_now && chain_mode(h->chain) > 0;
}
static int chain_end(bm_rbm *h) {
    BM_CHECK(chain_flush(h->chain, h->stream, h->maxB) == 0, "chained launch: %s", hipGetErrorString(hipGetLastError()));
    return 0;
}

static void ensure_wt(bm_rbm *h) {
    if (!h->use_wt || h->wt_valid) return;
    const int nt = ((h->V + 31) / 32) * ((h->H + 31) / 32);
    hipLaunchKernelGGL(transpose_kernel, dim3(nt), dim3(256), 0, h->stream, (const float *)h->W.p, h->W.ld, h->Wt.p, h->Wt.ld, h->V, h->H);
    h->wt_valid = true;
}

static void launch_up(bm_rbm *h, const float *v, int ldv, int B, float *means, float *states, int ldo,
                      int sample, uint32_t site, int t, float *negmeans = nullptr, bool fe = false) {
    ProfScope _ps(h, KC_UP);
    ActArgs a;
    memset(&a, 0, sizeof(a));
    a.P1 = make_operand(h->W.p, h->W.ld, h->H);
    a.Q1 = make_operand(v, ldv, B);
    a.K1 = h->V;
    a.I = h->H; a.J = B;
    a.bias = h->hb.p; a.sigma = nullptr;
    a.mult = 1.0f + (h->cfg.dbm_first ? 1.0f : 0.0f);
    a.bmult = a.mult;
    a.kind = BM_UNIT_BERNOULLI;
    a.sample = states ? sample : 0;
    a.means = means; a.states = states; a.negmeans = negmeans; a.ldo = ldo;
    a.key = make_key(h, site, t);
    a.row0 = h->row0;
    if (fe) {
        const int nslot = (h->H + 15) / 16, rm = (nslot + 3) & ~3;
        a.rowacc = h->fe_part.p; a.rowacc_single = 1; a.beta_b = 1.f; a.ld_part = h->maxB; a.fe_rm = rm;
        a.fe_rowacc2 = h->fe_part.p + (size_t)rm * h->maxB;
        a.fe_flip = FE_FLIP_FROM_KEY; a.fe_key = make_key(h, SITE_PLL, 0); a.fe_zero = h->scal.p;
        a.fe_x = v; a.fe_ldx = ldv; a.fe_w = h->W.p; a.fe_ldw = h->W.ld;
    }
    if (h->fast_now && v == h->vs.p) {
        a.b3.P1 = Bf3Operand{h->W3t.p, h->W3t.plane_stride(), h->W3t.ld, h->H};
        a.b3.Q1 = Bf3Operand{h->vs16.p, 0, h->vs16.ld, B};
        a.b3.K1 = h->vs16.ld;
        if (states == h->hs.p) { a.states16 = h->hs16.p; a.ld16 = h->hs16.ld; }
    }
    if (h->multinomial()) {
        if (!means) { means = h->hm.p; ldo = h->hm.ld; }
        a.kind = 3; a.sample = 0; a.means = means; a.ldo = ldo; a.states = nullptr; a.negmeans = nullptr;
        launch_act(a, h->stream);
        SmArgs m;
        memset(&m, 0, sizeof(m));
        m.L = means; m.ld = ldo; m.I = h->H; m.J = B; m.M = h->cfg.n_samples; m.sample = sample;
        m.states = states; m.negmeans = negmeans; m.key = a.key; m.row0 = h->row0;
        hipLaunchKernelGGL(softmax_multinomial_kernel, dim3(B), dim3(64), 2 * (size_t)h->H * sizeof(float), h->stream, m);
        return;
    }
    if (h->use_wt && h->wt_valid && !(h->fast_now && v == h->vs.p)) {
        const Operand wt = make_operand(h->Wt.p, h->Wt.ld, h->H);
        act_pass(h, a, &wt);
    } else act_pass(h, a);
}

static void launch_down(bm_rbm *h, const float *hs, int ldh, int B, float *means, float *states, int ldo,
                        int sample, uint32_t site, int t) {
    ProfScope _ps(h, KC_DOWN);
    ActArgs a;
    memset(&a, 0, sizeof(a));
    a.P1 = make_operand(h->W.p, h->W.ld, h->V);
    a.p_xm = 1;
    a.Q1 = make_operand(hs, ldh, B);
    a.K1 = h->H;
    a.I = h->V; a.J = B;
    a.bias = h->vb.p; a.sigma = h->sigma.p;
    a.mult = 1.0f + (h->cfg.dbm_last ? 1.0f : 0.0f);
    a.bmult = a.mult;
    a.kind = h->cfg.v_unit;
    a.sample = sample;
    a.means = means; a.states = states; a.ldo = ldo;
    a.key = make_key(h, site, t);
    a.row0 = h->row0;
    if (h->fast_now && hs == h->hs.p) {
        a.b3.P1 = Bf3Operand{h->W3.p, h->W3.plane_stride(), h->W3.ld, h->V};
        a.b3.Q1 = Bf3Operand{h->hs16.p, 0, h->hs16.ld, B};
        a.b3.K1 = h->hs16.ld;
        if (states == h->vs.p) { a.states16 = h->vs16.p; a.ld16 = h->vs16.ld; }
    }
    act_pass(h, a);
}

static bool metrics_fused_ok(const bm_rbm *h);
static void metrics_prep(bm_rbm *h, int B);
static int run_chain(bm_rbm *h, const float *X_dev, int B, int k, float *hm_out, bool need_vm = true, bool for_update = false,
                     bool split_step = false, bool fetch = false) {
    BM_CHECK(B >= 1 && B <= h->maxB, "batch %d outside [1, max_batch=%d]", B, h->maxB);
    BM_CHECK(k >= 1, "n_gibbs_steps must be >= 1 (got %d)", k);
    if (!split_step) ensure_wt(h);
    const float *Xin = X_dev;
    int ldx = h->V;
    if (h->cfg.v_unit == BM_UNIT_GAUSSIAN) {
        hipLaunchKernelGGL(div_cols_kernel, dim3(256), dim3(256), 0, h->stream, Xin, ldx, h->sigma.p, h->Xs.p,
                           h->Xs.ld, B, h->V);
        Xin = h->Xs.p; ldx = h->Xs.ld;
    }
    if (h->cfg.dropout >= 0.f) {
        hipLaunchKernelGGL(dropout_kernel, dim3(256), dim3(256), 0, h->stream, Xin, ldx, h->Xd.p, h->Xd.ld, B, h->V,
                           h->cfg.dropout, make_key(h, SITE_DROPOUT, 0),
                           (unsigned long long)h->row0 * (unsigned long long)h->V);
        Xin = h->Xd.p; ldx = h->Xd.ld;
    }
    h->Xin = Xin; h->Xin_ld = ldx;
    const bool fe = fetch && metrics_fused_ok(h);
    if (fe && !h->fe_part.p) BM_TRY(h->fe_part.alloc((size_t)2 * ((((h->H + 15) / 16) + 3) & ~3) * h->maxB));
    h->fe_in_chain = fe;
    if (fetch && !fe) metrics_prep(h, B);
    chain_begin(h);
    launch_up(h, Xin, ldx, B, h->h0m.p, h->h0s.p, h->h0m.ld, 1, SITE_H0, 0, nullptr, fe);
    const float *hstate = h->cfg.sample_h_states ? h->h0s.p : h->h0m.p;
    for (int t = 0; t < k; ++t) {
        const bool last = t == k - 1;
        launch_down(h, hstate, h->hs.ld, B, (need_vm && last) ? h->vm.p : nullptr, h->vs.p, h->vm.ld,
                    h->cfg.sample_v_states, SITE_V, t);
        const bool last_out = hm_out && last;
        const bool neg_only = last && !hm_out && !need_vm && !h->multinomial();
        h->hm_is_neg = neg_only;
        launch_up(h, h->vs.p, h->vs.ld, B, last_out ? hm_out : (neg_only ? nullptr : h->hm.p), last ? nullptr : h->hs.p,
                  last_out ? h->H : h->hm.ld, h->cfg.sample_h_states, SITE_H, t, (!hm_out && last) ? h->hneg.p : nullptr);
        hstate = h->hs.p;
    }
    BM_TRY(chain_end(h));
    return 0;
}

static void fill_bias(bm_rbm *h, float N, float lr, float mom, RbmBiasArgs &b) {
    float *tail = h->grad.p + h->grad_tail();
    b.sv = tail; b.sh = tail + h->V; b.sq = tail + h->V + h->H;
    b.vb = h->vb.p; b.dvb = h->dvb.p; b.hb = h->hb.p; b.dhb = h->dhb.p; b.q = h->q.p; b.pen = h->pen.p;
    b.V = h->V; b.H = h->H;
    b.N = N; b.lr = lr; b.mom = mom;
    b.damping = h->cfg.sparsity_damping; b.cost = h->cfg.sparsity_cost; b.target = h->cfg.sparsity_target;
}

static int fill_bias_fused(bm_rbm *h, int B, float lr, float mom, RbmBiasFusedArgs &a) {
    memset(&a, 0, sizeof(a));
    a.X = h->Xin; a.ldx = h->Xin_ld; a.vs = h->vs.p; a.ldv = h->vs.ld;
    a.h0m = h->h0m.p; a.ldh0 = h->h0m.ld; a.B = B;
    if (h->hm_is_neg) { a.hm = h->hneg.p; a.ldh = h->hneg.ld; a.hm_negated = 1; }
    else              { a.hm = h->hm.p; a.ldh = h->hm.ld; }
    a.raw_tail = h->grad.p + h->grad_tail();
    RbmBiasArgs &b = a.u;
    b.vb = h->vb.p; b.dvb = h->dvb.p; b.hb = h->hb.p; b.dhb = h->dhb.p; b.q = h->q.p; b.pen = h->pen.p;
    b.V = h->V; b.H = h->H;
    b.N = (float)B; b.lr = lr; b.mom = mom;
    b.damping = h->cfg.sparsity_damping; b.cost = h->cfg.sparsity_cost; b.target = h->cfg.sparsity_target;
    return (h->V + 63) / 64 + (h->H + 63) / 64;
}

static void launch_bias_fused(bm_rbm *h, int B, float lr, float mom) {
    ProfScope _ps(h, KC_COLSUM);
    RbmBiasFusedArgs a;
    const int nw = fill_bias_fused(h, B, lr, mom, a);
    hipLaunchKernelGGL(rbm_bias_fused_kernel, dim3(nw), dim3(NT), 0, h->stream, a);
}

static void rbm_grad(bm_rbm *h, int B, int fused, float N, float lr, float mom, bool with_bias);

static void launch_update_fused(bm_rbm *h, int B, float lr, float mom) {
    if (h->cfg.sparsity_cost != 0.f) {
        launch_bias_fused(h, B, lr, mom);
        rbm_grad(h, B, 1, (float)B, lr, mom, false);
    } else {
        rbm_grad(h, B, 1, (float)B, lr, mom, true);
    }
}

static void fill_grad(bm_rbm *h, int B, int fused, float N, float lr, float mom, GradArgs &g) {
    memset(&g, 0, sizeof(g));
    g.Ppos = make_operand(h->h0m.p, h->h0m.ld, h->H);
    g.Qpos = make_operand(h->Xin, h->Xin_ld, h->V);
    g.Kpos = B;
    g.Pneg = make_operand(h->hneg.p, h->hneg.ld, h->H);
    g.Qneg = make_operand(h->vs.p, h->vs.ld, h->V);
    g.Kneg = B;
    g.I = h->H; g.J = h->V;
    g.form = 0; g.fused = fused;
    g.raw = h->grad.p; g.raw2 = nullptr;
    g.W = h->W.p; g.dW = h->dW.p; g.Wt = nullptr;
    g.ldw = h->W.ld; g.ldwt = 0;
    if (h->use_wt && fused) { g.Wt = h->Wt.p; g.ldwt = h->Wt.ld; }
    g.N = N; g.M = N; g.l2 = h->cfg.l2; g.lr = lr; g.mom = mom;
}
static void rbm_grad(bm_rbm *h, int B, int fused, float N, float lr, float mom, bool with_bias) {
    ProfScope _ps(h, KC_GRAD);
    GradArgs g;
    fill_grad(h, B, fused, N, lr, mom, g);
    g.pen = with_bias ? nullptr : h->pen.p;
    if (with_bias) {
        g.nbias = fill_bias_fused(h, B, lr, mom, g.bias);
        g.bias.raw_only = fused ? 0 : 1;
    }
    bm::launch_grad(g, h->stream);
    if (fused && h->use_wt) h->wt_valid = true;
}

static void launch_fe(bm_rbm *h, const float *Xin, int ldx, int B, bool with_flip) {
    FeArgs f;
    memset(&f, 0, sizeof(f));
    f.P = make_operand(h->W.p, h->W.ld, h->H);
    f.Q = make_operand(Xin, ldx, B);
    f.K = h->V; f.I = h->H; f.J = B;
    f.hb = h->hb.p;
    f.rowacc = h->rowacc.p;
    if (with_flip) { f.rowacc2 = h->rowacc.p + h->maxB; f.flip_col = h->flip.p; }
    if (h->multinomial()) {
        (void)hipMemsetAsync(h->hhat.p, 0, 3 * (size_t)h->H * sizeof(float), h->stream);
        const int M = h->cfg.n_samples;
        hipLaunchKernelGGL(mn_hhat_kernel, dim3((M + 255) / 256), dim3(256), 0, h->stream, h->hhat.p, h->H, M,
                           make_key(h, SITE_FE, 0), make_key(h, SITE_FE, 1), make_key(h, SITE_FE, 2));
        f.hvec = h->hhat.p;
        f.rowacc3 = h->rowacc.p + 2 * (size_t)h->maxB;
    }
    launch_fe_hidden(f, h->stream);
    FeRowArgs r;
    memset(&r, 0, sizeof(r));
    r.X = Xin; r.ld = ldx; r.V = h->V; r.B = B;
    r.vb = h->vb.p; r.sigma = (h->cfg.v_unit == BM_UNIT_GAUSSIAN) ? h->sigma.p : nullptr;
    r.rowacc = f.rowacc; r.rowacc2 = f.rowacc2; r.rowacc3 = f.rowacc3; r.flip_col = f.flip_col; r.out = h->scal.p + 2;
    hipLaunchKernelGGL(fe_row_kernel, dim3((B + FE_ROWS_PER_WG - 1) / FE_ROWS_PER_WG), dim3(256), 0, h->stream, r);
}

static double mn_fe_const(const bm_rbm *h) {
    if (!h->multinomial()) return 0.0;
    const double M = h->cfg.n_samples, K = h->H;
    return -lgamma(M + K) + lgamma(M + 1.0) + lgamma(K);
}

static void metrics_to_out4(const bm_rbm *h, const double *host, int B, float *out4);
static bool metrics_fused_ok(const bm_rbm *h) {
    static const bool off = bm::dbg("metrics_fused") && atoi(bm::dbg("metrics_fused")) == 0;
    return !off && !h->multinomial() && !h->cfg.dbm_first && !h->fast_now && (h->W.ld & 3) == 0;
}
static void metrics_prep(bm_rbm *h, int B) {
    MetricsPrepArgs mp;
    mp.scal = h->scal.p; mp.rowacc = h->rowacc.p; mp.n_rowacc = 3 * h->maxB; mp.flip = h->flip.p; mp.B = B; mp.V = h->V;
    mp.key = make_key(h, SITE_PLL, 0); mp.row0 = (unsigned long long)h->row0;
    hipLaunchKernelGGL(metrics_prep_kernel, dim3(8), dim3(256), 0, h->stream, mp);
}
static int metrics_from_chain(bm_rbm *h, int B, float *out4) {
    const SqJob msre{h->Xin, h->Xin_ld, h->vm.p, h->vm.ld, B, h->V, h->scal.p + 0};
    const SqJob l2{h->W.p, h->W.ld, nullptr, 0, h->V, h->H, h->scal.p + 1};
// ... 51 lines not shown
int bm_dev_alloc(size_t bytes, void **out_dev) { BM_HIP(hipMalloc(out_dev, bytes ? bytes : 1)); return 0; }
int bm_dev_free(void *dev) { BM_HIP(hipFree(dev)); return 0; }
int bm_h2d(void *dst, const void *src, size_t bytes) {
    static const bool pin = !(bm::dbg("h2d_pin") && atoi(bm::dbg("h2d_pin")) == 0);
    if (pin && bytes >= ((size_t)32 << 20)) {
        if (hipHostRegister(const_cast<void *>(src), bytes, hipHostRegisterDefault) == hipSuccess) {
            const hipError_t e = hipMemcpy(dst, src, bytes, hipMemcpyHostToDevice);
            (void)hipHostUnregister(const_cast<void *>(src));
            BM_HIP(e);
            return 0;
        }
        (void)hipGetLastError();
    }
    BM_HIP(hipMemcpy(dst, src, bytes, hipMemcpyHostToDevice));
    return 0;
}
int bm_d2h(void *dst, const void *src, size_t bytes) { BM_HIP(hipMemcpy(dst, src, bytes, hipMemcpyDeviceToHost)); return 0; }
int bm_dev_memset(void *dst, int value, size_t bytes) { BM_HIP(hipMemset(dst, value, bytes)); return 0; }

int bm_rbm_create(const bm_rbm_config *cfg, bm_rbm **out) {
    BM_CHECK(cfg && out, "null argument");
    BM_CHECK(cfg->n_visible >= 1 && cfg->n_hidden >= 1, "bad layer sizes %d x %d", cfg->n_visible, cfg->n_hidden);
    BM_CHECK(cfg->max_batch >= 1, "max_batch must be >= 1");
    BM_CHECK(cfg->v_unit == BM_UNIT_BERNOULLI || cfg->v_unit == BM_UNIT_GAUSSIAN, "unknown visible unit %d", cfg->v_unit);
    BM_CHECK(cfg->h_unit == BM_UNIT_BERNOULLI || cfg->h_unit == BM_UNIT_MULTINOMIAL, "unknown hidden unit %d", cfg->h_unit);
    if (cfg->h_unit == BM_UNIT_MULTINOMIAL) {
        BM_CHECK(cfg->n_samples >= 1, "MultinomialRBM: n_samples must be >= 1 (got %d)", cfg->n_samples);
        BM_CHECK(cfg->n_hidden <= 8192, "MultinomialRBM: n_hidden %d > 8192 (softmax row staged in LDS)", cfg->n_hidden);
    }
    BM_CHECK(bm_device_count() > 0, "no HIP device visible: libbm355 has no CPU fallback");
    auto h = std::make_unique<bm_rbm>();
    h->cfg = *cfg;
    h->V = cfg->n_visible; h->H = cfg->n_hidden; h->maxB = cfg->max_batch;
    const int V = h->V, H = h->H, B = h->maxB;
    BM_HIP(hipGetDevice(&h->device));
    BM_TRY(create(h->stream)); BM_TRY(create(h->ev0)); BM_TRY(create(h->ev1));
    BM_TRY(h->W.alloc(V, H)); BM_TRY(h->dW.alloc(V, H));
    {
        const char *e = bm::dbg("up_xm");
        h->use_wt = !(e && atoi(e) == 0) && (V % 4 == 0) && !h->multinomial();
        if (h->use_wt) BM_TRY(h->Wt.alloc(H, V));
    }
    BM_TRY(h->vb.alloc(V)); BM_TRY(h->hb.alloc(H)); BM_TRY(h->dvb.alloc(V)); BM_TRY(h->dhb.alloc(H));
    BM_TRY(h->q.alloc(H)); BM_TRY(h->sigma.alloc(V));
    BM_TRY(h->h0m.alloc(B, H)); BM_TRY(h->h0s.alloc(B, H)); BM_TRY(h->hm.alloc(B, H)); BM_TRY(h->hs.alloc(B, H)); BM_TRY(h->hneg.alloc(B, H));
    BM_TRY(h->vm.alloc(B, V)); BM_TRY(h->vs.alloc(B, V)); BM_TRY(h->Xs.alloc(B, V)); BM_TRY(h->Xd.alloc(B, V));
    BM_TRY(h->grad.alloc(h->grad_tail() + V + 2 * (size_t)H));
    BM_TRY(h->pen.alloc(H));
    BM_TRY(h->rowacc.alloc(3 * (size_t)B)); BM_TRY(h->hhat.alloc(3 * (size_t)H));
    BM_TRY(h->flip.alloc(B)); BM_TRY(h->scal.alloc(6));
    {
        std::vector<float> ones(V, 1.0f);
        BM_HIP(hipMemcpy(h->sigma.p, ones.data(), V * sizeof(float), hipMemcpyHostToDevice));
    }
    *out = h.release();
    return 0;
}

int bm_rbm_destroy(bm_rbm *h) {
    if (!h) return 0;
    for (hipStream_t st : {h->stream.h, h->comm_stream.h, h->stage_stream.h}) if (st) (void)hipStreamSynchronize(st);
    if (h->xchg_used) xchg_bind_user(h->xchg_used, nullptr);
    delete h;
    return 0;
}

static int check_device_status(bm_rbm *h) {
    if (h->xchg_used) BM_TRY(xchg_check_status(h->xchg_used));
    if (h->chain.status) {
        int st[2] = {0, 0};
        BM_HIP(hipMemcpy(st, h->chain.status, sizeof(st), hipMemcpyDeviceToHost));
        const long long expect = h->chain.tiles_expected & 0xffffffffLL;
        if (st[0] != 0 || (long long)(unsigned)st[1] != expect) {
            h->chain.mode = 0;
            h->chain.tiles_expected = 0;
            BM_HIP(hipMemset(h->chain.status, 0, sizeof(st)));
            BM_CHECK(st[0] == 0, "chained propagation launch failed (status %d: %s); the results since the last check are "
                     "invalid, chained launches are now off for this handle", st[0],
                     st[0] == CHAIN_ERR_TIMEOUT ? "a wait for a producing tile expired" : "not an 8-XCD device");
            BM_CHECK(false, "chained propagation launches computed %u tiles, expected %lld; the results since the last check "
                     "are invalid, chained launches are now off for this handle", (unsigned)st[1], expect);
        }
    }
    return 0;
}

int bm_rbm_sync(bm_rbm *h) {
    BM_HIP(hipStreamSynchronize(h->stream));
    BM_TRY(check_device_status(h));
    if (h->nonbinary.p) {
        int bad = 0;
        BM_HIP(hipMemcpy(&bad, h->nonbinary.p, sizeof(int), hipMemcpyDeviceToHost));
        if (bad) {
            BM_HIP(hipMemset(h->nonbinary.p, 0, sizeof(int)));
            BM_CHECK(false, "fast-binary mode: bm_rbm_gibbs was given hidden states that are not a {0,1} bitmap");
        }
    }
    return 0;
}

int bm_rbm_set_fast_binary(bm_rbm *h, int32_t on) {
    BM_CHECK(h, "null argument");
    h->fast = (on >= 2 || (on == 1 && (long long)h->V * h->H >= (8ll << 20))) ? 1 : 0;
    return 0;
}

static DevBuf *find_vec(bm_rbm *h, const std::string &n) {
    if (n == "vb") return &h->vb;
    if (n == "hb") return &h->hb;
    if (n == "dvb") return &h->dvb;
    if (n == "dhb") return &h->dhb;
    if (n == "q_means") return &h->q;
    if (n == "sigma") return &h->sigma;
    return nullptr;
}

int bm_rbm_set_param(bm_rbm *h, const char *name, const float *host, size_t n) {
    const std::string nm(name ? name : "");
    BM_HIP(hipStreamSynchronize(h->stream));
    if (nm == "W" || nm == "dW") {
        BM_CHECK(n == (size_t)h->V * h->H, "variable '%s' has %zu elements, got %zu", name, (size_t)h->V * h->H, n);
        BM_TRY((nm == "W" ? h->W : h->dW).upload(host));
        if (nm == "W") h->wt_valid = false;
        else { h->dw_sharded = false; if (h->xchg_used) xchg_dw_replaced(h->xchg_used); }
        return 0;
    }
    DevBuf *b = find_vec(h, nm);
    BM_CHECK(b, "unknown RBM variable '%s'", name ? name : "(null)");
    BM_CHECK(n == b->n, "variable '%s' has %zu elements, got %zu", name, b->n, n);
    BM_HIP(hipMemcpy(b->p, host, n * sizeof(float), hipMemcpyHostToDevice));
    return 0;
}

int bm_rbm_set_param_dev(bm_rbm *h, const char *name, const float *src_dev, size_t n) {
    const std::string nm(name ? name : "");
    BM_CHECK(h && src_dev, "null argument");
    if (nm == "W" || nm == "dW") {
        BM_CHECK(n == (size_t)h->V * h->H, "variable '%s' has %zu elements, got %zu", name, (size_t)h->V * h->H, n);
        Mat &m = nm == "W" ? h->W : h->dW;
        if (nm == "W") h->wt_valid = false;
        else { h->dw_sharded = false; if (h->xchg_used) xchg_dw_replaced(h->xchg_used); }
        BM_HIP(hipMemcpy2DAsync(m.p, (size_t)m.ld * sizeof(float), src_dev, (size_t)m.cols * sizeof(float),
                                (size_t)m.cols * sizeof(float), m.rows, hipMemcpyDeviceToDevice, h->stream));
        return 0;
    }
    DevBuf *b = find_vec(h, nm);
    BM_CHECK(b, "unknown RBM variable '%s'", name ? name : "(null)");
    BM_CHECK(n == b->n, "variable '%s' has %zu elements, got %zu", name, b->n, n);
    BM_HIP(hipMemcpyAsync(b->p, src_dev, n * sizeof(float), hipMemcpyDeviceToDevice, h->stream));
    return 0;
}

int bm_rbm_get_param(bm_rbm *h, const char *name, float *host, size_t n) {
    const std::string nm(name ? name : "");
    BM_HIP(hipStreamSynchronize(h->stream));
    BM_TRY(check_device_status(h));
    if (nm == "W" || nm == "dW") {
        BM_CHECK(n == (size_t)h->V * h->H, "variable '%s' has %zu elements, got %zu", name, (size_t)h->V * h->H, n);
        if (nm == "dW") BM_TRY(check_dw(h, "bm_rbm_get_param(dW)"));
        return (nm == "W" ? h->W : h->dW).download(host);
    }
    DevBuf *b = find_vec(h, nm);
    BM_CHECK(b, "unknown RBM variable '%s'", name ? name : "(null)");
    BM_CHECK(n == b->n, "variable '%s' has %zu elements, got %zu", name, b->n, n);
    BM_HIP(hipMemcpy(host, b->p, n * sizeof(float), hipMemcpyDeviceToHost));
    return 0;
}

int bm_rbm_stage(bm_rbm *h, int32_t slot) {
    BM_CHECK(h && (slot == 0 || slot == 1), "bad stage slot %d", (int)slot);
    bm_rbm::Stage &sg = h->stage[slot];
    BM_CHECK(sg.readers.load() == 0, "stage slot %d is being read by bm_rbm_get_staged: use the other slot", (int)slot);
    BM_TRY(check_dw(h, "bm_rbm_stage"));
    if (!sg.ev) {
        BM_TRY(sg.W.alloc(h->V, h->H)); BM_TRY(sg.dW.alloc(h->V, h->H));
        BM_TRY(sg.vb.alloc(h->V)); BM_TRY(sg.dvb.alloc(h->V)); BM_TRY(sg.sigma.alloc(h->V));
        BM_TRY(sg.hb.alloc(h->H)); BM_TRY(sg.dhb.alloc(h->H)); BM_TRY(sg.q.alloc(h->H));
        BM_TRY(create(sg.ev, hipEventDisableTiming));
    }
    if (!h->stage_stream) BM_TRY(create(h->stage_stream, hipStreamNonBlocking));
    static const bool bound = !(bm::dbg("stage_ahead") && atoi(bm::dbg("stage_ahead")) == 0);
    if (bound && h->last_stage >= 0) BM_HIP(hipEventSynchronize(h->stage[h->last_stage].ev));
    BM_HIP(hipMemcpyAsync(sg.W.p, h->W.p, h->W.count() * sizeof(float), hipMemcpyDeviceToDevice, h->stream));
    BM_HIP(hipMemcpyAsync(sg.dW.p, h->dW.p, h->dW.count() * sizeof(float), hipMemcpyDeviceToDevice, h->stream));
    DevBuf *src[] = {&h->vb, &h->hb, &h->dvb, &h->dhb, &h->q, &h->sigma};
    DevBuf *dst[] = {&sg.vb, &sg.hb, &sg.dvb, &sg.dhb, &sg.q, &sg.sigma};
    for (int i = 0; i < 6; ++i)
        BM_HIP(hipMemcpyAsync(dst[i]->p, src[i]->p, src[i]->n * sizeof(float), hipMemcpyDeviceToDevice, h->stream));
    BM_HIP(hipEventRecord(sg.ev, h->stream));
    sg.ready = true;
    h->last_stage = slot;
    return 0;
}
int bm_rbm_get_staged(bm_rbm *h, int32_t slot, const char *name, float *host, size_t n) {
    BM_CHECK(h && (slot == 0 || slot == 1) && h->stage[slot].ready, "stage slot %d holds no snapshot", (int)slot);
    BM_HIP(hipSetDevice(h->device));
    bm_rbm::Stage &sg = h->stage[slot];
    struct Reading { std::atomic<int> &n; Reading(std::atomic<int> &r) : n(r) { ++n; } ~Reading() { --n; } } reading(sg.readers);
    const std::string nm(name ? name : "");
    BM_HIP(hipEventSynchronize(sg.ev));
    const size_t need = (size_t)h->V * h->H * sizeof(float);
    if (!h->stage_host) BM_TRY(create(h->stage_host, (size_t)h->V * h->H));
    if (h->chain.status) {
        BM_HIP(hipMemcpyAsync(h->stage_host, h->chain.status, sizeof(int), hipMemcpyDeviceToHost, h->stage_stream));
        BM_HIP(hipStreamSynchronize(h->stage_stream));
        BM_CHECK(*(const int *)h->stage_host.h == 0, "a chained propagation launch failed (status %d) before this snapshot: "
                 "it is invalid (bm_rbm_sync reports and recovers)", *(const int *)h->stage_host.h);
    }
    if (nm == "W" || nm == "dW") {
        BM_CHECK(n == (size_t)h->V * h->H, "variable '%s' has %zu elements, got %zu", name, (size_t)h->V * h->H, n);
        const Mat &m = nm == "W" ? sg.W : sg.dW;
        BM_HIP(hipMemcpy2DAsync(h->stage_host, (size_t)m.cols * sizeof(float), m.p, (size_t)m.ld * sizeof(float),
                                (size_t)m.cols * sizeof(float), m.rows, hipMemcpyDeviceToHost, h->stage_stream));
    } else {
        const char *names[] = {"vb", "hb", "dvb", "dhb", "q_means", "sigma"};
        DevBuf *bufs[] = {&sg.vb, &sg.hb, &sg.dvb, &sg.dhb, &sg.q, &sg.sigma};
        DevBuf *b = nullptr;
        for (int i = 0; i < 6; ++i) if (nm == names[i]) b = bufs[i];
        BM_CHECK(b, "unknown RBM variable '%s'", name ? name : "(null)");
        BM_CHECK(n == b->n, "variable '%s' has %zu elements, got %zu", name, b->n, n);
        BM_CHECK(n * sizeof(float) <= need, "variable '%s' larger than the bounce buffer", name);
        BM_HIP(hipMemcpyAsync(h->stage_host, b->p, n * sizeof(float), hipMemcpyDeviceToHost, h->stage_stream));
    }
    BM_HIP(hipStreamSynchronize(h->stage_stream));
    memcpy(host, h->stage_host, n * sizeof(float));
    return 0;
}

int bm_rbm_dev_ptr(bm_rbm *h, const char *name, void **out_dev, size_t *out_n) {
    const std::string nm(name ? name : "");
    DevBuf *b = (nm == "grad") ? &h->grad : find_vec(h, nm);
    BM_CHECK(b, "no device view for '%s' (matrices are pitched; use get/set_param)", name ? name : "(null)");
    *out_dev = b->p;
    if (out_n) *out_n = b->n;
    return 0;
}

int bm_rbm_seed(bm_rbm *h, uint64_t seed) { h->seed = seed; h->call = 0; return 0; }
int bm_rbm_set_row_offset(bm_rbm *h, int64_t row0) { h->row0 = row0; return 0; }

int bm_rbm_train_step(bm_rbm *h, const float *X_dev, int32_t B, float lr, float mom, int32_t k) {
    BM_TRY(check_dw(h, "bm_rbm_train_step"));
    BM_TRY(run_chain(h, X_dev, B, k, nullptr, false, true));
    launch_update_fused(h, B, lr, mom);
    h->call++;
    BM_HIP(hipGetLastError());
    return 0;
}

int bm_rbm_train_step_metrics(bm_rbm *h, const float *X_dev, int32_t B, float lr, float mom, int32_t k,
                              float *out4) {
    BM_TRY(check_dw(h, "bm_rbm_train_step_metrics"));
    BM_TRY(run_chain(h, X_dev, B, k, nullptr, true, false, false, true));
    BM_TRY(metrics_from_chain(h, B, out4));
    launch_update_fused(h, B, lr, mom);
    h->call++;
    BM_HIP(hipGetLastError());
    return 0;
}

int bm_rbm_train_step_metrics_async(bm_rbm *h, const float *X_dev, int32_t B, float lr, float mom, int32_t k) {
    if (!h->mring) {
        Pinned<double> ring;
        BM_TRY(create(ring, (size_t)bm_rbm::MRING * 6));
        BM_TRY(create(h->ev_mlast, hipEventDisableTiming));
        BM_HIP(hipHostGetDevicePointer((void **)&h->mring_dev, ring, 0));
        h->mring_B.resize(bm_rbm::MRING);
        h->mring = std::move(ring);
    }
    BM_CHECK(h->mring_n < bm_rbm::MRING, "%d metric fetches are pending: call bm_rbm_collect_metrics", h->mring_n);
    BM_TRY(check_dw(h, "bm_rbm_train_step_metrics_async"));
    BM_TRY(run_chain(h, X_dev, B, k, nullptr, true, false, false, true));
    BM_TRY(metrics_from_chain(h, B, nullptr));
    hipLaunchKernelGGL(scal_to_host_kernel, dim3(1), dim3(64), 0, h->stream, (const double *)h->scal.p,
                       h->mring_dev + (size_t)h->mring_n * 6);
    BM_HIP(hipEventRecord(h->ev_mlast, h->stream));
    h->mring_B[h->mring_n++] = B;
    launch_update_fused(h, B, lr, mom);
    h->call++;
    BM_HIP(hipGetLastError());
    return 0;
}
int bm_rbm_collect_metrics(bm_rbm *h, float *out4n, int32_t max_n, int32_t *out_n) {
    BM_CHECK(h && out_n && (out4n || max_n == 0), "null argument");
    BM_CHECK(h->mring_n <= max_n, "%d fetches pending, room for %d", h->mring_n, (int)max_n);
    if (h->mring_n > 0 && h->ev_mlast) BM_HIP(hipEventSynchronize(h->ev_mlast));
    if (h->chain.status || h->xchg_used) {
        BM_HIP(hipStreamSynchronize(h->stream));
        const int rc = check_device_status(h);
        if (rc) { h->mring_n = 0; *out_n = 0; return rc; }
    }
    for (int i = 0; i < h->mring_n; ++i) metrics_to_out4(h, h->mring + (size_t)i * 6, h->mring_B[i], out4n + 4 * (size_t)i);
    *out_n = h->mring_n;
    h->mring_n = 0;
    return 0;
}

int bm_rbm_train_epoch(bm_rbm *h, const float *X_dev, int64_t N, int32_t batch, float lr, float mom, int32_t k) {
    BM_CHECK(batch >= 1 && N >= 1, "bad N=%lld batch=%d", (long long)N, batch);
    for (int64_t s = 0; s < N; s += batch) {
        const int B = (int)((N - s < batch) ? (N - s) : batch);
        BM_TRY(bm_rbm_train_step(h, X_dev + (size_t)s * h->V, B, lr, mom, k));
    }
    return 0;
}

int bm_rbm_grad_step(bm_rbm *h, const float *X_dev, int32_t B, int32_t k) {
    BM_TRY(run_chain(h, X_dev, B, k, nullptr, false, false, true));
    rbm_grad(h, B, 0, (float)B, 0.f, 0.f, true);
    h->call++;
    BM_HIP(hipGetLastError());
    return 0;
}

static int ensure_delayed(bm_rbm *h) {
    if (h->comm_stream) return 0;
    BM_TRY(h->grad_alt.alloc(h->grad.n));
    for (int i = 0; i < 2; ++i) {
        BM_TRY(create(h->ev_ready[i], hipEventDisableTiming));
        BM_TRY(create(h->ev_reduced[i], hipEventDisableTiming));
    }
    return create(h->comm_stream);
}
int bm_rbm_set_grad_slot(bm_rbm *h, int32_t slot) {
    BM_CHECK(h && (slot == 0 || slot == 1), "slot must be 0 or 1");
    if (slot == h->grad_slot) return 0;
    BM_TRY(ensure_delayed(h));
    std::swap(h->grad, h->grad_alt);
    h->grad_slot = slot;
    return 0;
}
int bm_rbm_allreduce_grads_async(bm_rbm *h, bm_comm *c) {
    BM_CHECK(h && c, "null argument");
    BM_TRY(ensure_delayed(h));
    const int s = h->grad_slot;
    BM_HIP(hipEventRecord(h->ev_ready[s], h->stream));
    BM_HIP(hipStreamWaitEvent(h->comm_stream, h->ev_ready[s], 0));
    BM_TRY(bm_comm_allreduce_sum(c, h->grad.p, h->grad.n, (void *)h->comm_stream));
    BM_HIP(hipEventRecord(h->ev_reduced[s], h->comm_stream));
    return 0;
}
int bm_rbm_wait_grads(bm_rbm *h, int32_t slot) {
    BM_CHECK(h && (slot == 0 || slot == 1) && h->comm_stream, "no reduction was started on slot %d", slot);
    BM_HIP(hipStreamWaitEvent(h->stream, h->ev_reduced[slot], 0));
    return 0;
}

int bm_rbm_apply_step(bm_rbm *h, int32_t B_global, float lr, float mom) {
    BM_TRY(check_dw(h, "bm_rbm_apply_step"));
    ProfScope _ps(h, KC_BIAS);
    RbmBiasArgs b;
    fill_bias(h, (float)B_global, lr, mom, b);
    ApplyWArgs a;
    memset(&a, 0, sizeof(a));
    a.raw = h->grad.p; a.raw2 = nullptr;
    a.W = h->W.p; a.dW = h->dW.p; a.Wt = nullptr;
    h->wt_valid = false;
    a.I = h->H; a.J = h->V; a.ldw = h->W.ld; a.ldwt = 0; a.form = 0;
    a.N = (float)B_global; a.M = a.N; a.l2 = h->cfg.l2; a.lr = lr; a.mom = mom;
    if (h->cfg.sparsity_cost != 0.f) {
        hipLaunchKernelGGL(rbm_bias_kernel, dim3((h->V + h->H + 255) / 256), dim3(256), 0, h->stream, b);
        a.pen = h->pen.p;
        launch_apply_w(a, nullptr, h->stream);
    } else {
        a.pen = nullptr;
        launch_apply_w(a, &b, h->stream);
    }
    BM_HIP(hipGetLastError());
    return 0;
}
// ... 47 lines not shown
    BM_CHECK(n_steps >= 1, "n_steps must be >= 1");
    struct FastScope { bm_rbm *h; ~FastScope() { h->fast_now = false; } } fast_scope{h};
    const bool fast = h->fast && h->cfg.v_unit == BM_UNIT_BERNOULLI && !h->multinomial() && h->cfg.sample_v_states &&
                      h->cfg.sample_h_states && h->cfg.dropout < 0.f;
    if (!fast && !h->multinomial()) {
        ensure_wt(h);
        chain_begin(h);
        for (int t = 0; t < n_steps; ++t) {
            const bool first = t == 0, last = t == n_steps - 1;
            launch_down(h, first ? H_dev : h->hs.p, first ? h->H : h->hs.ld, B, nullptr, last ? V_dev : h->vs.p,
                        last ? h->V : h->vs.ld, h->cfg.sample_v_states, SITE_V, t);
            launch_up(h, last ? V_dev : h->vs.p, last ? h->V : h->vs.ld, B, nullptr, last ? H_dev : h->hs.p,
                      last ? h->H : h->hs.ld, h->cfg.sample_h_states, SITE_H, t);
        }
        BM_TRY(chain_end(h));
        h->call++;
        BM_HIP(hipGetLastError());
        return 0;
    }
    hipLaunchKernelGGL(copy2d_kernel, dim3(256), dim3(256), 0, h->stream, (const float *)H_dev, h->H, h->hs.p, h->hs.ld, B, h->H);
    if (fast) {
        if (!h->nonbinary.p) {
            BM_TRY(h->W3.alloc(3, h->V, h->H)); BM_TRY(h->W3t.alloc(3, h->H, h->V));
            BM_TRY(h->hs16.alloc(1, h->maxB, h->H)); BM_TRY(h->vs16.alloc(1, h->maxB, h->V));
            BM_TRY(h->nonbinary.alloc(1));
            BM_HIP(hipMemsetAsync(h->nonbinary.p, 0, sizeof(int), h->stream));
        }
        hipLaunchKernelGGL(split3_kernel, dim3(512), dim3(256), 0, h->stream, (const float *)h->W.p, h->W.ld, h->V, h->H,
                           h->W3.p, h->W3.plane_stride(), h->W3.ld, 0);
        hipLaunchKernelGGL(split3_kernel, dim3(512), dim3(256), 0, h->stream, (const float *)h->W.p, h->W.ld, h->V, h->H,
                           h->W3t.p, h->W3t.plane_stride(), h->W3t.ld, 1);
        hipLaunchKernelGGL(shadow16_check_kernel, dim3(256), dim3(256), 0, h->stream, (const float *)h->hs.p, h->hs.ld, B, h->H,
                           h->hs16.p, h->hs16.ld, h->nonbinary.p);
        h->fast_now = true;
    }
    for (int t = 0; t < n_steps; ++t) {
        launch_down(h, h->hs.p, h->hs.ld, B, nullptr, h->vs.p, h->vs.ld, h->cfg.sample_v_states, SITE_V, t);
        launch_up(h, h->vs.p, h->vs.ld, B, nullptr, h->hs.p, h->hs.ld, h->cfg.sample_h_states, SITE_H, t);
    }
    hipLaunchKernelGGL(copy2d_kernel, dim3(256), dim3(256), 0, h->stream, (const float *)h->hs.p, h->hs.ld, H_dev, h->H, B, h->H);
    hipLaunchKernelGGL(copy2d_kernel, dim3(256), dim3(256), 0, h->stream, (const float *)h->vs.p, h->vs.ld, V_dev, h->V, B, h->V);
    h->call++;
    BM_HIP(hipGetLastError());
    return 0;
}

int bm_debug_tile_map(int32_t tiles_i, int32_t tiles_j, double bytes_i, double bytes_j, int32_t *out_ti, int32_t *out_tj,
                      int32_t *out_map5) {
    BM_CHECK(tiles_i >= 1 && tiles_j >= 1 && out_ti && out_tj, "bad arguments");
    const TileMap m = make_tile_map(tiles_i, tiles_j, bytes_i, bytes_j);
    const int nb = tiles_i * tiles_j;
    for (int b = 0; b < nb; ++b) { int ti = -1, tj = -1; tile_of_block(m, b, nb, ti, tj); out_ti[b] = ti; out_tj[b] = tj; }
    if (out_map5) { out_map5[0] = m.xi; out_map5[1] = m.xj; out_map5[2] = m.gj; out_map5[3] = m.tiles_i; out_map5[4] = m.tiles_j; }
    return 0;
}

int bm_rbm_stream(bm_rbm *h, void **out_stream) { *out_stream = (void *)h->stream; return 0; }

int bm_rbm_profile(bm_rbm *h, int32_t enable) {
    BM_HIP(hipStreamSynchronize(h->stream));
    h->recs.clear();
    h->prof = enable != 0;
    return 0;
}

int bm_rbm_kernel_times(bm_rbm *h, float *ms6, int32_t *n6) {
    BM_HIP(hipStreamSynchronize(h->stream));
    for (int c = 0; c < BM_NUM_KERNEL_CLASSES; ++c) { ms6[c] = 0.f; n6[c] = 0; }
    for (auto &r : h->recs) {
        float ms = 0.f;
        BM_HIP(hipEventElapsedTime(&ms, r.a, r.b));
        ms6[r.cls] += ms;
        n6[r.cls] += 1;
    }
    return 0;
}

int bm_rbm_chain_stats(bm_rbm *h, int64_t *out3) {
    BM_CHECK(h && out3, "null argument");
    out3[0] = (int64_t)h->chain.launches; out3[1] = (int64_t)h->chain.tiles_expected; out3[2] = (int64_t)chain_mode(h->chain);
    return 0;
}

int bm_rbm_timer_start(bm_rbm *h) { BM_HIP(hipEventRecord(h->ev0, h->stream)); return 0; }
int bm_rbm_timer_mark(bm_rbm *h) { BM_HIP(hipEventRecord(h->ev1, h->stream)); return 0; }
int bm_rbm_timer_elapsed(bm_rbm *h, float *out_ms) {
    BM_HIP(hipEventSynchronize(h->ev1));
    BM_HIP(hipEventElapsedTime(out_ms, h->ev0, h->ev1));
    return 0;
}
int bm_rbm_timer_stop(bm_rbm *h, float *out_ms) {
    BM_HIP(hipEventRecord(h->ev1, h->stream));
    BM_HIP(hipEventSynchronize(h->ev1));
    BM_HIP(hipEventElapsedTime(out_ms, h->ev0, h->ev1));
    return 0;
}

}
```

### boltzmann_machines_amd/engine.py

```python
import ctypes as C

import numpy as np

from . import _ffi
from ._ffi import DeviceArray, check

RBM_VARS = ('W', 'vb', 'hb', 'dW', 'dvb', 'dhb', 'q_means', 'sigma')


def as_device(X):
    if isinstance(X, DeviceArray):
        return X
    return DeviceArray.from_numpy(np.asarray(X), np.float32)


class RbmEngine(object):
    dtype = np.float32

    def __init__(self, n_visible, n_hidden, v_unit=_ffi.UNIT_BERNOULLI, sample_v_states=False,
                 sample_h_states=True, dbm_first=False, dbm_last=False, max_batch=10, l2=1e-4,
                 sparsity_target=0.1, sparsity_cost=0., sparsity_damping=0.9, dropout=None,
                 h_unit=_ffi.UNIT_BERNOULLI, n_samples=0):
        self.lib = _ffi.load()
        self.V, self.H, self.max_batch = int(n_visible), int(n_hidden), int(max_batch)
# ... 44 lines not shown
    def set_fast_binary(self, on, everywhere=False):
        check(self.lib.bm_rbm_set_fast_binary(self._h, (2 if everywhere else 1) if on else 0))

    def set_from_device(self, name, darr):
        check(self.lib.bm_rbm_set_param_dev(self._h, name.encode(), darr.ptr, int(np.prod(darr.shape))))

    def device_view(self, name):
        p, n = C.c_void_p(), C.c_size_t()
        check(self.lib.bm_rbm_dev_ptr(self._h, name.encode(), C.byref(p), C.byref(n)))
        return DeviceArray((n.value,), np.float32, ptr=p.value, owner=self)

    def seed(self, seed):
        check(self.lib.bm_rbm_seed(self._h, int(seed)))

    def set_row_offset(self, row0):
        check(self.lib.bm_rbm_set_row_offset(self._h, int(row0)))

    def sync(self):
        check(self.lib.bm_rbm_sync(self._h))

    def train_step(self, Xd, B, lr, momentum, k, row=0):
        check(self.lib.bm_rbm_train_step(self._h, Xd.offset_ptr(row * self.V), B, lr, momentum, k))

    def train_step_metrics(self, Xd, B, lr, momentum, k, row=0):
        out = (C.c_float * 4)()
        check(self.lib.bm_rbm_train_step_metrics(self._h, Xd.offset_ptr(row * self.V), B, lr, momentum, k, out))
        return np.array(out[:], dtype=np.float32)

    MAX_PENDING_METRICS = 4096

    def train_step_metrics_async(self, Xd, B, lr, momentum, k, row=0):
        check(self.lib.bm_rbm_train_step_metrics_async(self._h, Xd.offset_ptr(row * self.V), B, lr, momentum, k))

    def collect_metrics(self):
        out = np.empty((self.MAX_PENDING_METRICS, 4), dtype=np.float32)
        n = C.c_int32(0)
        check(self.lib.bm_rbm_collect_metrics(self._h, out.ctypes.data_as(C.POINTER(C.c_float)),
                                              self.MAX_PENDING_METRICS, C.byref(n)))
        return out[:n.value].copy()

    def train_epoch(self, Xd, N, batch, lr, momentum, k, row=0):
        check(self.lib.bm_rbm_train_epoch(self._h, Xd.offset_ptr(row * self.V), N, batch, lr, momentum, k))

    def grad_step(self, Xd, B, k, row=0):
        check(self.lib.bm_rbm_grad_step(self._h, Xd.offset_ptr(row * self.V), B, k))

    def apply_step(self, B_global, lr, momentum):
        check(self.lib.bm_rbm_apply_step(self._h, B_global, lr, momentum))

    def set_grad_slot(self, slot):
        check(self.lib.bm_rbm_set_grad_slot(self._h, slot))

    def allreduce_grads_async(self, comm):
        check(self.lib.bm_rbm_allreduce_grads_async(self._h, comm._c))

    def wait_grads(self, slot):
        check(self.lib.bm_rbm_wait_grads(self._h, slot))

    def transform(self, Xd, B, k, Hd, row=0, out_row=0):
        check(self.lib.bm_rbm_transform(self._h, Xd.offset_ptr(row * self.V), B, k, Hd.offset_ptr(out_row * self.H)))

    def metrics(self, Xd, B, k, row=0):
        out = (C.c_float * 4)()
        check(self.lib.bm_rbm_metrics(self._h, Xd.offset_ptr(row * self.V), B, k, out))
        return np.array(out[:], dtype=np.float32)

    def free_energy(self, Xd, B, row=0):
        out = C.c_float()
        check(self.lib.bm_rbm_free_energy(self._h, Xd.offset_ptr(row * self.V), B, C.byref(out)))
        return float(out.value)

    def gibbs(self, Hd, Vd, B, n_steps):
        check(self.lib.bm_rbm_gibbs(self._h, Hd.ptr, Vd.ptr, B, n_steps))

    def stream(self):
        p = C.c_void_p()
        check(self.lib.bm_rbm_stream(self._h, C.byref(p)))
        return p.value

    def chain_stats(self):
        out = (C.c_int64 * 3)()
        check(self.lib.bm_rbm_chain_stats(self._h, out))
        return int(out[0]), int(out[1]), int(out[2])

    def profile(self, enable):
        check(self.lib.bm_rbm_profile(self._h, int(bool(enable))))

    def kernel_times(self):
        ms, n = (C.c_float * 6)(), (C.c_int32 * 6)()
        check(self.lib.bm_rbm_kernel_times(self._h, ms, n))
        names = ('act_up', 'act_down', 'grad', 'colsum', 'bias', 'other')
        return {k: (float(ms[i]), int(n[i])) for i, k in enumerate(names)}

    def timer_start(self):
        check(self.lib.bm_rbm_timer_start(self._h))

    def timer_stop(self):
        ms = C.c_float()
        check(self.lib.bm_rbm_timer_stop(self._h, C.byref(ms)))
        return float(ms.value)

    def timer_mark(self):
        check(self.lib.bm_rbm_timer_mark(self._h))

    def timer_elapsed(self):
        ms = C.c_float()
        check(self.lib.bm_rbm_timer_elapsed(self._h, C.byref(ms)))
        return float(ms.value)


class RbmEngine64(object):

    dtype = np.float64

    def __init__(self, n_visible, n_hidden, v_unit=_ffi.UNIT_BERNOULLI, sample_v_states=False,
                 sample_h_states=True, dbm_first=False, dbm_last=False, max_batch=10, l2=1e-4,
                 sparsity_target=0.1, sparsity_cost=0., sparsity_damping=0.9, dropout=None,
                 h_unit=_ffi.UNIT_BERNOULLI, n_samples=0):
        self.lib = _ffi.load()
        self.V, self.H, self.max_batch = int(n_visible), int(n_hidden), int(max_batch)
        drop = -1.0 if dropout is None else float(dropout)
        cfg = _ffi.RbmConfig(self.V, self.H, int(v_unit), int(bool(sample_v_states)),
                             int(bool(sample_h_states)), int(bool(dbm_first)), int(bool(dbm_last)),
                             self.max_batch, float(l2), float(sparsity_target), float(sparsity_cost),
                             float(sparsity_damping), drop, int(h_unit), int(n_samples))
        hyper = (C.c_double * 5)(float(l2), float(sparsity_target), float(sparsity_cost), float(sparsity_damping), drop)
        self._h = C.c_void_p()
        check(self.lib.bm_rbm64_create(C.byref(cfg), hyper, C.byref(self._h)))

    def close(self):
        if getattr(self, '_h', None) is not None and self._h:
            self.lib.bm_rbm64_destroy(self._h)
            self._h = None

    def __del__(self):
        try:
            self.close()
        except Exception:
            pass

    def _shape(self, name):
        if name in ('W', 'dW'):
            return (self.V, self.H)
        return (self.V,) if name in ('vb', 'dvb', 'sigma') else (self.H,)

    def set(self, name, value):
        a = np.ascontiguousarray(np.broadcast_to(np.asarray(value, dtype=np.float64), self._shape(name)))
        check(self.lib.bm_rbm64_set_param(self._h, name.encode(), a.ctypes.data_as(C.c_void_p), a.size))

    def get(self, name):
        a = np.empty(self._shape(name), dtype=np.float64)
        check(self.lib.bm_rbm64_get_param(self._h, name.encode(), a.ctypes.data_as(C.c_void_p), a.size))
        return a

    def seed(self, seed):
        check(self.lib.bm_rbm64_seed(self._h, int(seed) & 0xFFFFFFFFFFFFFFFF))

    def set_row_offset(self, row0):
        check(self.lib.bm_rbm64_set_row_offset(self._h, int(row0)))

    def sync(self):
        check(self.lib.bm_rbm64_sync(self._h))

    def train_step(self, Xd, B, lr, momentum, k, row=0):
        check(self.lib.bm_rbm64_train_step(self._h, Xd.offset_ptr(row * self.V), B, lr, momentum, k))

# ... 286 lines not shown
```

### include/bm355.h

```cpp
#ifndef BM355_H
#define BM355_H

#include <stddef.h>
#include <stdint.h>

#ifdef __cplusplus
extern "C" {
#endif

const char *bm_last_error(void);
const char *bm_version(void);
int bm_device_count(void);
int bm_set_device(int device);

int bm_dev_alloc(size_t bytes, void **out_dev);
int bm_dev_free(void *dev);
int bm_h2d(void *dst_dev, const void *src_host, size_t bytes);
int bm_d2h(void *dst_host, const void *src_dev, size_t bytes);
int bm_dev_memset(void *dst_dev, int value, size_t bytes);

int bm_debug_tile_map(int32_t tiles_i, int32_t tiles_j, double bytes_i, double bytes_j, int32_t *out_ti,
                      int32_t *out_tj, int32_t *out_map5);

typedef struct bm_rbm bm_rbm;

enum { BM_UNIT_BERNOULLI = 0, BM_UNIT_GAUSSIAN = 1, BM_UNIT_MULTINOMIAL = 2 };

typedef struct bm_rbm_config {
    int32_t n_visible;
    int32_t n_hidden;
    int32_t v_unit;
    int32_t sample_v_states;
    int32_t sample_h_states;
    int32_t dbm_first;
    int32_t dbm_last;
    int32_t max_batch;
    float   l2;
    float   sparsity_target;
    float   sparsity_cost;
    float   sparsity_damping;
    float   dropout;
    int32_t h_unit;
    int32_t n_samples;
} bm_rbm_config;

int bm_rbm_create(const bm_rbm_config *cfg, bm_rbm **out);
int bm_rbm_destroy(bm_rbm *h);
int bm_rbm_sync(bm_rbm *h);

int bm_rbm_set_param(bm_rbm *h, const char *name, const float *host, size_t n);
int bm_rbm_set_param_dev(bm_rbm *h, const char *name, const float *src_dev, size_t n);
int bm_rbm_get_param(bm_rbm *h, const char *name, float *host, size_t n);
int bm_rbm_dev_ptr(bm_rbm *h, const char *name, void **out_dev, size_t *out_n);

int bm_rbm_seed(bm_rbm *h, uint64_t seed);
int bm_rbm_set_row_offset(bm_rbm *h, int64_t row0);

int bm_rbm_train_step(bm_rbm *h, const float *X_dev, int32_t B,
                      float learning_rate, float momentum, int32_t n_gibbs_steps);
int bm_rbm_train_step_metrics(bm_rbm *h, const float *X_dev, int32_t B,
                              float learning_rate, float momentum, int32_t n_gibbs_steps,
                              float *out4);
int bm_rbm_train_step_metrics_async(bm_rbm *h, const float *X_dev, int32_t B,
                                    float learning_rate, float momentum, int32_t n_gibbs_steps);
int bm_rbm_collect_metrics(bm_rbm *h, float *out4n, int32_t max_n, int32_t *out_n);
int bm_rbm_train_epoch(bm_rbm *h, const float *X_dev, int64_t N, int32_t batch,
                       float learning_rate, float momentum, int32_t n_gibbs_steps);

int bm_rbm_stage(bm_rbm *h, int32_t slot);
int bm_rbm_get_staged(bm_rbm *h, int32_t slot, const char *name, float *host, size_t n);

int bm_rbm_grad_step(bm_rbm *h, const float *X_dev, int32_t B_local, int32_t n_gibbs_steps);
int bm_rbm_apply_step(bm_rbm *h, int32_t B_global, float learning_rate, float momentum);

int bm_rbm_transform(bm_rbm *h, const float *X_dev, int32_t B, int32_t n_gibbs_steps,
                     float *H_dev);

int bm_rbm_metrics(bm_rbm *h, const float *X_dev, int32_t B, int32_t n_gibbs_steps,
                   float *out4);
int bm_rbm_free_energy(bm_rbm *h, const float *X_dev, int32_t B, float *out1);

int bm_rbm_gibbs(bm_rbm *h, float *H_dev, float *V_dev, int32_t B, int32_t n_steps);

int bm_rbm_stream(bm_rbm *h, void **out_stream);

#define BM_NUM_KERNEL_CLASSES 6
int bm_rbm_profile(bm_rbm *h, int32_t enable);
int bm_rbm_kernel_times(bm_rbm *h, float *ms6, int32_t *n6);

int bm_rbm_chain_stats(bm_rbm *h, int64_t *out3);

int bm_rbm_timer_start(bm_rbm *h);
int bm_rbm_timer_stop(bm_rbm *h, float *out_ms);
int bm_rbm_timer_mark(bm_rbm *h);
int bm_rbm_timer_elapsed(bm_rbm *h, float *out_ms);

typedef struct bm_rbm64 bm_rbm64;
int bm_rbm64_create(const bm_rbm_config *cfg, const double *hyper5, bm_rbm64 **out);
int bm_rbm64_destroy(bm_rbm64 *h);
int bm_rbm64_sync(bm_rbm64 *h);
int bm_rbm64_seed(bm_rbm64 *h, uint64_t seed);
int bm_rbm64_set_row_offset(bm_rbm64 *h, int64_t row0);
int bm_rbm64_set_param(bm_rbm64 *h, const char *name, const double *host, size_t n);
int bm_rbm64_get_param(bm_rbm64 *h, const char *name, double *host, size_t n);
int bm_rbm64_train_step(bm_rbm64 *h, const double *X_dev, int32_t B,
                        double learning_rate, double momentum, int32_t n_gibbs_steps);
int bm_rbm64_train_step_metrics(bm_rbm64 *h, const double *X_dev, int32_t B,
                                double learning_rate, double momentum, int32_t n_gibbs_steps, double *out4);
int bm_rbm64_transform(bm_rbm64 *h, const double *X_dev, int32_t B, int32_t n_gibbs_steps,
                       double *H_dev);
int bm_rbm64_metrics(bm_rbm64 *h, const double *X_dev, int32_t B, int32_t n_gibbs_steps,
                     double *out4);
int bm_rbm64_free_energy(bm_rbm64 *h, const double *X_dev, int32_t B, double *out1);


typedef struct bm_dbm bm_dbm;

#define BM_DBM_MAX_LAYERS 4

typedef struct bm_dbm_config {
    int32_t n_layers;
    int32_t n_visible;
    int32_t n_hiddens[BM_DBM_MAX_LAYERS];
    int32_t v_unit;
    int32_t sample_v_states;
    int32_t sample_h_states[BM_DBM_MAX_LAYERS];
    int32_t n_particles;
    int32_t batch_size;
    int32_t max_mf_updates;
    float   mf_tol;
    float   l2;
    float   max_norm;
    float   sparsity_target[BM_DBM_MAX_LAYERS];
    float   sparsity_cost[BM_DBM_MAX_LAYERS];
    float   sparsity_damping;
    int32_t h_unit[BM_DBM_MAX_LAYERS];
    int32_t n_samples[BM_DBM_MAX_LAYERS];
} bm_dbm_config;

int bm_dbm_create(const bm_dbm_config *cfg, bm_dbm **out);
int bm_dbm_destroy(bm_dbm *h);
int bm_dbm_sync(bm_dbm *h);
int bm_dbm_seed(bm_dbm *h, uint64_t seed);
int bm_dbm_set_row_offset(bm_dbm *h, int64_t row0, int64_t particle0);

int bm_dbm_set_param(bm_dbm *h, const char *name, const float *host, size_t n);
int bm_dbm_get_param(bm_dbm *h, const char *name, float *host, size_t n);
int bm_dbm_dev_ptr(bm_dbm *h, const char *name, void **out_dev, size_t *out_n);

int bm_dbm_train_step(bm_dbm *h, const float *X_dev, float learning_rate, float momentum,
                      int32_t n_gibbs_steps, int32_t *out_n_mf, float *out_msre);
int bm_dbm_metrics(bm_dbm *h, const float *X_dev, int32_t n_gibbs_steps, int32_t *out_n_mf, float *out_msre);
int bm_dbm_grad_step(bm_dbm *h, const float *X_dev, int32_t n_gibbs_steps, int32_t *out_n_mf);
int bm_dbm_apply_step(bm_dbm *h, int32_t N_global, int32_t M_global,
                      float learning_rate, float momentum);
int bm_dbm_set_mf_allreduce(bm_dbm *h, float (*fn)(float local_max, void *ctx), void *ctx);
int bm_dbm_stream(bm_dbm *h, void **out_stream);

int bm_dbm_mean_field(bm_dbm *h, const float *X_dev, float *MU_top_dev, int32_t *out_n_mf);
int bm_dbm_reconstruct(bm_dbm *h, const float *X_dev, float *R_dev);
int bm_dbm_sample_v(bm_dbm *h, int32_t n_gibbs_steps, float *V_dev);
int bm_dbm_ais(bm_dbm *h, int32_t n_betas, int32_t n_runs, int32_t n_gibbs_steps,
               uint64_t seed, int64_t chain0, float *values_host);
int bm_dbm_log_proba(bm_dbm *h, const float *X_dev, float *out_host);

int bm_dbm_timer_start(bm_dbm *h);
int bm_dbm_timer_stop(bm_dbm *h, float *out_ms);
int bm_dbm_timer_mark(bm_dbm *h);
int bm_dbm_timer_elapsed(bm_dbm *h, float *out_ms);


typedef struct bm_comm bm_comm;
int bm_comm_unique_id(void *out_id128);
// ... 67 lines not shown
```

Measured before the change: 15890.

## Fuse final hidden activation pass with gradient and bias update in persistent tail kernel

Adds a persistent 'tail' kernel that defers the last up-pass (negative hidden means) of a CD-k step and runs it together with the weight-gradient tiles and the fused bias update. Work items are claimed dynamically, and flag-based per-row waits let gradient tiles start as soon as the hidden rows they need are written. This removes kernel-launch boundaries and the idle tail between the act and grad kernels. Second-segment operand loads switch to coherent (sc1) loads so the grad tiles see data produced by other workgroups in the same launch. It adds spin-wait synchronisation, is enabled by default only on 8-XCC/256-CU gfx942/950 devices and small k, and falls back otherwise.

```diff
diff --git a/boltzmann_machines_amd/_ffi.py b/boltzmann_machines_amd/_ffi.py
--- a/boltzmann_machines_amd/_ffi.py
+++ b/boltzmann_machines_amd/_ffi.py
@@ -135,6 +135,7 @@
     'bm_rbm_profile': [_vp, _i32],
     'bm_rbm_kernel_times': [_vp, _fp, _ip],
     'bm_rbm_chain_stats': [_vp, C.POINTER(C.c_int64)],
+    'bm_rbm_tail_stats': [_vp, C.POINTER(C.c_int64)],
     'bm_rbm_timer_start': [_vp],
     'bm_rbm_timer_stop': [_vp, _fp],
     'bm_rbm_timer_mark': [_vp],
diff --git a/boltzmann_machines_amd/csrc/bm_chain.h b/boltzmann_machines_amd/csrc/bm_chain.h
--- a/boltzmann_machines_amd/csrc/bm_chain.h
+++ b/boltzmann_machines_amd/csrc/bm_chain.h
@@ -168,6 +168,7 @@
     bool on = false;
     int mode = -1;
     int ncu = 0;
+    bool dev_ok = false;
     std::vector<ActArgs> rec;
     std::vector<Operand> alt_p;
     long long *stamps = nullptr;
@@ -203,7 +204,8 @@
         cs.ncu = have ? pr.multiProcessorCount : 0;
         if (hipDeviceGetAttribute(&nxcc, hipDeviceAttributeNumberOfXccs, d) != hipSuccess) nxcc = 0;
         const bool arch = have && (strncmp(pr.gcnArchName, "gfx950", 6) == 0 || strncmp(pr.gcnArchName, "gfx942", 6) == 0);
-        if (!(arch && nxcc == 8 && cs.ncu == 256)) cs.mode = 0;
+        cs.dev_ok = arch && nxcc == 8 && cs.ncu == 256;
+        if (!cs.dev_ok) cs.mode = 0;
     }
     return cs.mode;
 }
diff --git a/boltzmann_machines_amd/csrc/bm_gemm.h b/boltzmann_machines_amd/csrc/bm_gemm.h
--- a/boltzmann_machines_amd/csrc/bm_gemm.h
+++ b/boltzmann_machines_amd/csrc/bm_gemm.h
@@ -10,6 +10,8 @@
     static constexpr bool kFinalSync = true;
     static constexpr bool kSplitFill = false, kCohQ = false;
     static constexpr bool kCanAbort = false;
+    static constexpr bool kSeg2Wait = false, kCohP2 = false;
+    __device__ __forceinline__ void wait_seg2() {}
     __device__ __forceinline__ void wait_inputs() {}
     __device__ __forceinline__ void post_fill() {}
     __device__ __forceinline__ void fill() {}
@@ -319,6 +321,13 @@
                  : "=&s"(keep) : "v"(src), "s"(__builtin_amdgcn_readfirstlane(lds_addr)) : "memory");
 }
 
+__device__ __forceinline__ void dma16_coh(const char *src, float *lds_dst) {
+    unsigned keep;
+    const unsigned lds_addr = (unsigned)(uintptr_t)(__attribute__((address_space(3))) void *)lds_dst;
+    asm volatile("s_mov_b32 %0, m0\n\ts_mov_b32 m0, %2\n\ts_nop 0\n\tglobal_load_lds_dwordx4 %1, off sc1\n\ts_mov_b32 m0, %0"
+                 : "=&s"(keep) : "v"(src), "s"(__builtin_amdgcn_readfirstlane(lds_addr)) : "memory");
+}
+
 __device__ __forceinline__ void dma16s(const void *sbase, uint32_t voff, unsigned lds_byte) {
     asm volatile("s_mov_b32 m0, %2\n\ts_nop 0\n\tglobal_load_lds_dwordx4 %1, %0"
                  :: "s"(sbase), "v"(voff), "s"(lds_byte) : "memory");
@@ -327,10 +336,13 @@
     asm volatile("s_mov_b32 m0, %2\n\ts_nop 0\n\tglobal_load_lds_dwordx4 %1, %0 sc1"
                  :: "s"(sbase), "v"(voff), "s"(lds_byte) : "memory");
 }
-template <class G, int DW, bool QSC = false, bool QHALF = false>
+template <class G, int DW, bool QSC = false, bool QHALF = false, bool PSC = false>
 __device__ __forceinline__ void dma_chunk_s(const DmaPlan<G, DW> &pl, const char *pb, const char *qb, unsigned ldsP, unsigned ldsQ) {
 #pragma unroll
-    for (int n = 0; n < DmaPlan<G, DW>::NPP; ++n) dma16s(pb, pl.p[n], ldsP + (unsigned)(n * DW * 1024));
+    for (int n = 0; n < DmaPlan<G, DW>::NPP; ++n) {
+        if (PSC) dma16s_coh(pb, pl.p[n], ldsP + (unsigned)(n * DW * 1024));
+        else     dma16s(pb, pl.p[n], ldsP + (unsigned)(n * DW * 1024));
+    }
 #pragma unroll
     for (int n = 0; n < DmaPlan<G, DW>::NPQ; ++n) {
         if (QHALF && (n & 1)) continue;
@@ -339,7 +351,7 @@
     }
 }
 
-template <int QL, class G, bool SEG2, int PL = KM, int DW = G::NW, bool QHALF = false>
+template <int QL, class G, bool SEG2, int PL = KM, int DW = G::NW, bool QHALF = false, bool PCOH2 = false>
 __device__ __forceinline__ void dma_chunk(const KRange &kr, const DmaPlan<G, DW> &pl1, const DmaPlan<G, DW> &pl2, int nch1, int c,
                                           float *sP, float *sQ, int wave) {
     constexpr int BK = G::BK;
@@ -355,7 +367,8 @@
     for (int n = 0; n < DmaPlan<G, DW>::NPP; ++n) {
         const uint32_t o1 = pl1.p[n], o2 = SEG2 ? pl2.p[n] : 0u;
         const uint32_t o = SEG2 ? (o1 ^ ((o1 ^ o2) & (uint32_t)m)) : o1;
-        dma16(pb + o, sP + (wave + n * DW) * 256);
+        if (PCOH2 && SEG2 && m) dma16_coh(pb + o, sP + (wave + n * DW) * 256);
+        else                    dma16(pb + o, sP + (wave + n * DW) * 256);
     }
 #pragma unroll
     for (int n = 0; n < DmaPlan<G, DW>::NPQ; ++n) {
@@ -366,7 +379,7 @@
     }
 }
 
-template <int QL, class G, bool FAST, bool SEG2, int PL = KM, bool COHQ = false>
+template <int QL, class G, bool FAST, bool SEG2, int PL = KM, bool COHQ = false, bool COHP2 = false>
 __device__ __forceinline__ void load_chunk(ChunkRegs<G> &r, const KRange &kr, int nch1, int i0, int j0, int c, int tid) {
     constexpr int BK = G::BK;
     if (!SEG2) {
@@ -376,6 +389,10 @@
         const int m = -(int)((c >= nch1) & (kr.K2 > 0));
         const int kc = c - (nch1 & m);
         const int K = sel_i(kr.K1, kr.K2, m);
+        if constexpr (COHP2) {
+            if (m) g2r<PL, G::TI, BK, G::NT, FAST, true>(r.p, kr.P2.ptr, kr.P2.ld, kr.P2.nx, kr.P2.vec, i0, kc * BK, K, tid);
+            else   g2r<PL, G::TI, BK, G::NT, FAST>(r.p, kr.P1.ptr, kr.P1.ld, kr.P1.nx, kr.P1.vec, i0, kc * BK, K, tid);
+        } else
         g2r<PL, G::TI, BK, G::NT, FAST>(r.p, sel_p(kr.P1.ptr, kr.P2.ptr, m), sel_i(kr.P1.ld, kr.P2.ld, m),
                                         sel_i(kr.P1.nx, kr.P2.nx, m), sel_i(kr.P1.vec, kr.P2.vec, m), i0, kc * BK, K, tid);
         g2r<QL, G::TJ, BK, G::NT, FAST, COHQ>(r.q, sel_p(kr.Q1.ptr, kr.Q2.ptr, m), sel_i(kr.Q1.ld, kr.Q2.ld, m),
@@ -487,6 +504,13 @@
         if (!FAST || STG == STG_REG || BM_ABL(6)) return false;
         return is_full(c);
     };
+    static_assert(!Side::kSeg2Wait || STG == STG_DMA, "wait_seg2: DMA staging only (the REG steady steps request chunks on their own)");
+    bool seg2_open = false;
+    auto seg2_gate = [&](int c) {
+        if constexpr (SEG2 && Side::kSeg2Wait) {
+            if (!seg2_open && c >= nch1 && c < nch) { seg2_open = true; side.wait_seg2(); }
+        }
+    };
     ChunkRegs<G> gr;
     Frags<G> fa, fb;
     DmaPlan<G, DW> pl1, pl2;
@@ -543,16 +567,18 @@
         BM_WAIT_VM(NQ_LEFT);
     } else {
 #pragma unroll
-        for (int c = 0; c < PF; ++c)
+        for (int c = 0; c < PF; ++c) {
+            seg2_gate(c);
             if (c < nch && is_dma(c) && dmaw && !BM_ABL(0))
-                dma_chunk<QL, G, SEG2, PL, DW, (BM_ABL(9) != 0)>(kr, pl1, pl2, nch1, c, sP + (c % NBUF) * P_BUF, sQ + (c % NBUF) * Q_BUF, w);
+                dma_chunk<QL, G, SEG2, PL, DW, (BM_ABL(9) != 0), Side::kCohP2>(kr, pl1, pl2, nch1, c, sP + (c % NBUF) * P_BUF, sQ + (c % NBUF) * Q_BUF, w);
+        }
         __builtin_amdgcn_sched_barrier(0);
         side.fill();
         __builtin_amdgcn_sched_barrier(0);
 #pragma unroll
         for (int c = 0; c < 2; ++c)
             if (c < nch && !is_dma(c) && !BM_ABL(0)) {
-                load_chunk<QL, G, FAST, SEG2, PL>(gr, kr, nch1, i0, j0, c, tid);
+                load_chunk<QL, G, FAST, SEG2, PL, false, Side::kCohP2>(gr, kr, nch1, i0, j0, c, tid);
                 store_chunk<QL, G, SEG2, PL>(gr, kr, nch1, c, sP + (c % NBUF) * P_BUF, sQ + (c % NBUF) * Q_BUF, tid);
             }
         {
@@ -610,11 +636,16 @@
         if (SEG2 && !in2 && (CD) >= nch1) { in2 = true; pl1 = pl2; }                              \
         const char *pb_, *qb_;                                                                    \
         chunk_bases((CD), pb_, qb_);                                                              \
+        if (Side::kCohP2 && in2) {                                                                \
+            if (dmaw) dma_chunk_s<G, DW, Side::kCohQ, (BM_ABL(9) != 0), true>(pl1, pb_, qb_, ldsPw + (unsigned)((SD) * P_BUF * 4), \
+                                         ldsQw + (unsigned)((SD) * Q_BUF * 4));                   \
+        } else                                                                                    \
         if (dmaw) dma_chunk_s<G, DW, Side::kCohQ, (BM_ABL(9) != 0)>(pl1, pb_, qb_, ldsPw + (unsigned)((SD) * P_BUF * 4), \
                                      ldsQw + (unsigned)((SD) * Q_BUF * 4));                       \
     }
 #define BM_STEP_Q(FC, FN, S)                                                                      \
     {                                                                                             \
+        seg2_gate(cc + PF);                                                                       \
         BM_DMA_AT(cc + PF, ((S) + PF) % NBUF)                                                     \
         read_frags<QL, G, ABL, PL>(FN, sP + (((S) + 1) % NBUF) * P_BUF, sQ + (((S) + 1) % NBUF) * Q_BUF, wi, wj, lane); \
         mfma_frags<G, ABL>(acc, FC);                                                              \
@@ -626,10 +657,11 @@
 #define BM_STEP_T(FC, FN, S1, S2, S3)       \
     {                                                                                             \
         const int cd = cc + PF, cr = cc + 2;                                                      \
+        seg2_gate(cd);                                                                            \
         const bool do_dma = cd < nch && is_dma(cd) && !BM_ABL(0);                                 \
         const bool do_reg = cr < nch && !is_dma(cr) && !BM_ABL(0);                                \
         if (cc == last - 1) side.drain();       \
-        if (do_reg) load_chunk<QL, G, FAST, SEG2, PL, Side::kCohQ>(gr, kr, nch1, i0, j0, cr, tid); \
+        if (do_reg) load_chunk<QL, G, FAST, SEG2, PL, Side::kCohQ, Side::kCohP2>(gr, kr, nch1, i0, j0, cr, tid); \
         if (do_dma) BM_DMA_AT(cd, S3)                                                             \
         read_frags<QL, G, ABL, PL>(FN, sP + (S1) * P_BUF, sQ + (S1) * Q_BUF, wi, wj, lane);       \
         mfma_frags<G, ABL>(acc, FC);                                                              \
diff --git a/boltzmann_machines_amd/csrc/bm_kernels.h b/boltzmann_machines_amd/csrc/bm_kernels.h
--- a/boltzmann_machines_amd/csrc/bm_kernels.h
+++ b/boltzmann_machines_amd/csrc/bm_kernels.h
@@ -150,6 +150,8 @@
 template <int E, class Rng, bool MF = false, int NTH = 256> struct ActSide {
     static constexpr bool kFinalSync = false;
     static constexpr bool kSplitFill = false, kCohQ = false, kCanAbort = MF;
+    static constexpr bool kSeg2Wait = false, kCohP2 = false;
+    __device__ __forceinline__ void wait_seg2() {}
     static constexpr bool kMF = MF;
     const float *bias, *sigma;
     const float *prev_row;
@@ -749,6 +751,8 @@
 template <int NJ> struct GradSide {
     static constexpr bool kFinalSync = true;
     static constexpr bool kSplitFill = false, kCohQ = false, kCanAbort = false;
+    static constexpr bool kSeg2Wait = false, kCohP2 = false;
+    __device__ __forceinline__ void wait_seg2() {}
     const float *W, *dW; int ldw, I, J, ib0, jb[NJ]; bool on, vec8;
     float4 w[NJ][2], d[NJ][2];
     bool at_fill;
@@ -777,6 +781,9 @@
         }
     }
 };
+
+template <class G, bool FAST, int ABL, int STG, class SideT>
+__device__ __forceinline__ void grad_tile(const GradArgs &a, int i0, int j0, float *smem, SideT &side, int stamp_blk = 0);
 
 template <class G, bool FAST, int ABL = 0, int STG = STG_DMA, int MINB = 1>
 __global__ __launch_bounds__(G::NT, MINB) void grad_kernel(GradArgs a, TileMap tmap) {
@@ -804,14 +811,20 @@
         TILE_WORDS(tmap, (int)blockIdx.x);
         TILE_OF_BLOCK(tmap, (int)blockIdx.x, ntile_blocks, ti, tj);
     }
-    const int i0 = ti * TI, j0 = tj * TJ2;
+    GradSide<NJ> side;
+    grad_tile<G, FAST, ABL, STG>(a, ti * TI, tj * TJ2, smem, side, (int)blockIdx.x);
+}
+
+template <class G, bool FAST, int ABL, int STG, class SideT>
+__device__ __forceinline__ void grad_tile(const GradArgs &a, int i0, int j0, float *smem, SideT &side, int stamp_blk) {
+    constexpr int NJ = G::NJ;
     const int tid = threadIdx.x, lane = tid & 63, w = tid >> 6;
     const int wi = w % G::WI, wj = w / G::WI;
     const int g = lane >> 4, l15 = lane & 15;
     const int ib0 = i0 + wi * 32 + g * 8;
 
 #ifdef BM_PROBE
-#define BM_GSTAMP(n) do { if (a.dbg && threadIdx.x == 0) a.dbg[blockIdx.x * 4 + (n)] = (long long)__builtin_readcyclecounter(); } while (0)
+#define BM_GSTAMP(n) do { if (a.dbg && threadIdx.x == 0) a.dbg[stamp_blk * 4 + (n)] = (long long)__builtin_readcyclecounter(); } while (0)
 #else
 #define BM_GSTAMP(n) do {} while (0)
 #endif
@@ -821,7 +834,6 @@
     for (int t = 0; t < 2; ++t)
 #pragma unroll
         for (int n = 0; n < NJ; ++n) pos[t][n] = neg[t][n] = (f32x4){0.f, 0.f, 0.f, 0.f};
-    GradSide<NJ> side;
     side.W = a.W; side.dW = a.dW; side.ldw = a.ldw; side.I = a.I; side.J = a.J; side.ib0 = ib0;
 #pragma unroll
     for (int n = 0; n < NJ; ++n) side.jb[n] = j0 + wj * (16 * NJ) + lane_j<KM, G>(l15, n);
diff --git a/boltzmann_machines_amd/csrc/bm_launch.h b/boltzmann_machines_amd/csrc/bm_launch.h
--- a/boltzmann_machines_amd/csrc/bm_launch.h
+++ b/boltzmann_machines_amd/csrc/bm_launch.h
@@ -330,15 +330,28 @@
                 g.I, g.J, g.Kpos, g.Kneg, g.form, g.fused, T.geo, us[0], us[1], us[2], us[3], us[4], T.xi == XI_SLAB ? 9 : T.xi, xi_us[4], xi_us[0], xi_us[1], xi_us[2], xi_us[3]);
     return T;
 }
-static inline void launch_grad(const GradArgs &g_in, hipStream_t st) {
+static inline int grad_tuned(GradArgs &g, hipStream_t st) {
     static const int fetch_env = std::max(0, dbg_int("grad_fetch")), geo_env = dbg_int("grad_geo");
-    GradArgs g = g_in;
     g.fetch_at_fill = fetch_env;
-    if (geo_env) { launch_grad_as(geo_env, g, st); return; }
+    if (geo_env) return geo_env;
     static TuneMemo<6> memo;
     const Tuned T = memo.get({g.I, g.J, g.Kpos, g.Kneg, g.form | (g.fused << 1), g.ldw}, [&] { return tune_grad_shape(g, st); });
     if (T.xi != XI_MODEL && !g.map_xi) g.map_xi = T.xi;
-    launch_grad_as(T.geo, g, st);
+    return T.geo;
+}
+static inline void launch_grad(const GradArgs &g_in, hipStream_t st) {
+    GradArgs g = g_in;
+    const int geo = grad_tuned(g, st);
+    launch_grad_as(geo, g, st);
+}
+
+template <class GG, int STG, int PL, class A> __global__ void tail_kernel(A c);
+static inline bool tail_geo_ok(int geo) { return geo == 8; }
+template <class A>
+static inline void launch_tail_as(int geo, const A &c, int grid, hipStream_t st) {
+    (void)geo;
+    if (c.up.p_xm) hipLaunchKernelGGL((tail_kernel<GeoGrad8, STG_DMA, XM, A>), dim3(grid), dim3(GeoGrad8::NT), 0, st, c);
+    else           hipLaunchKernelGGL((tail_kernel<GeoGrad8, STG_DMA, KM, A>), dim3(grid), dim3(GeoGrad8::NT), 0, st, c);
 }
 
 static inline void launch_fe_hidden(const FeArgs &f, hipStream_t st) {
diff --git a/boltzmann_machines_amd/csrc/bm_rbm.hip b/boltzmann_machines_amd/csrc/bm_rbm.hip
--- a/boltzmann_machines_amd/csrc/bm_rbm.hip
+++ b/boltzmann_machines_amd/csrc/bm_rbm.hip
@@ -2,6 +2,7 @@
 #include "bm_common.h"
 #include "bm_kernels.h"
 #include "bm_chain.h"
+#include "bm_tail.h"
 
 #include <math.h>
 #include <atomic>
@@ -81,6 +82,9 @@
     std::vector<Rec> recs;
     size_t grad_tail() const { return (size_t)V * W.ld; }
     ChainState chain;
+    TailState tail;
+    bool tail_pending = false;
+    ActArgs tail_up;
 };
 
 enum { KC_UP = 0, KC_DOWN = 1, KC_GRAD = 2, KC_COLSUM = 3, KC_BIAS = 4, KC_OTHER = 5 };
@@ -140,7 +144,7 @@
 }
 
 static void launch_up(bm_rbm *h, const float *v, int ldv, int B, float *means, float *states, int ldo,
-                      int sample, uint32_t site, int t, float *negmeans = nullptr, bool fe = false) {
+                      int sample, uint32_t site, int t, float *negmeans = nullptr, bool fe = false, bool defer = false) {
     ProfScope _ps(h, KC_UP);
     ActArgs a;
     memset(&a, 0, sizeof(a));
@@ -182,8 +186,10 @@
     }
     if (h->use_wt && h->wt_valid && !(h->fast_now && v == h->vs.p)) {
         const Operand wt = make_operand(h->Wt.p, h->Wt.ld, h->H);
+        if (defer) { h->tail_up = a; h->tail_up.P1 = wt; h->tail_up.p_xm = 1; h->tail_pending = true; return; }
         act_pass(h, a, &wt);
-    } else act_pass(h, a);
+    } else if (defer) { h->tail_up = a; h->tail_pending = true; }
+    else act_pass(h, a);
 }
 
 static void launch_down(bm_rbm *h, const float *hs, int ldh, int B, float *means, float *states, int ldo,
@@ -215,6 +221,12 @@
 
 static bool metrics_fused_ok(const bm_rbm *h);
 static void metrics_prep(bm_rbm *h, int B);
+static bool tail_wanted(bm_rbm *h, int B, int k) {
+    const int mode = tail_mode(h->tail, h->chain);
+    if (mode <= 0 || h->prof || h->multinomial() || h->fast_now || h->cfg.sparsity_cost != 0.f) return false;
+    if ((h->H + 63) / 64 < 8 || 2 * ((B + 63) / 64) > CHAIN_MAXTI) return false;
+    return mode >= 2 || k <= 2;
+}
 static int run_chain(bm_rbm *h, const float *X_dev, int B, int k, float *hm_out, bool need_vm = true, bool for_update = false,
                      bool split_step = false, bool fetch = false) {
     BM_CHECK(B >= 1 && B <= h->maxB, "batch %d outside [1, max_batch=%d]", B, h->maxB);
@@ -238,6 +250,7 @@
     if (fe && !h->fe_part.p) BM_TRY(h->fe_part.alloc((size_t)2 * ((((h->H + 15) / 16) + 3) & ~3) * h->maxB));
     h->fe_in_chain = fe;
     if (fetch && !fe) metrics_prep(h, B);
+    const bool tail = for_update && !split_step && !fetch && !hm_out && !need_vm && tail_wanted(h, B, k);
     chain_begin(h);
     launch_up(h, Xin, ldx, B, h->h0m.p, h->h0s.p, h->h0m.ld, 1, SITE_H0, 0, nullptr, fe);
     const float *hstate = h->cfg.sample_h_states ? h->h0s.p : h->h0m.p;
@@ -249,7 +262,8 @@
         const bool neg_only = last && !hm_out && !need_vm && !h->multinomial();
         h->hm_is_neg = neg_only;
         launch_up(h, h->vs.p, h->vs.ld, B, last_out ? hm_out : (neg_only ? nullptr : h->hm.p), last ? nullptr : h->hs.p,
-                  last_out ? h->H : h->hm.ld, h->cfg.sample_h_states, SITE_H, t, (!hm_out && last) ? h->hneg.p : nullptr);
+                  last_out ? h->H : h->hm.ld, h->cfg.sample_h_states, SITE_H, t, (!hm_out && last) ? h->hneg.p : nullptr,
+                  false, tail && neg_only);
         hstate = h->hs.p;
     }
     BM_TRY(chain_end(h));
@@ -288,8 +302,26 @@
 }
 
 static void rbm_grad(bm_rbm *h, int B, int fused, float N, float lr, float mom, bool with_bias);
+static void fill_grad(bm_rbm *h, int B, int fused, float N, float lr, float mom, GradArgs &g);
 
 static void launch_update_fused(bm_rbm *h, int B, float lr, float mom) {
+    if (h->tail_pending) {
+        h->tail_pending = false;
+        GradArgs g;
+        fill_grad(h, B, 1, (float)B, lr, mom, g);
+        g.pen = nullptr;
+        g.nbias = fill_bias_fused(h, B, lr, mom, g.bias);
+        g.bias.raw_only = 0;
+        const int geo = bm::grad_tuned(g, h->stream);
+        const bool ok = tail_shape_ok(h->tail_up, g) && (h->tail.mode >= 2 || tail_geo_ok(geo)) &&
+                        tail_launch(h->tail, h->chain.ncu, h->tail_up, g, h->tail.mode >= 2 ? 8 : geo, h->stream);
+        if (ok) {
+            if (h->use_wt) h->wt_valid = true;
+            return;
+        }
+        ++h->tail.fallbacks;
+        launch_act(h->tail_up, h->stream);
+    }
     if (h->cfg.sparsity_cost != 0.f) {
         launch_bias_fused(h, B, lr, mom);
         rbm_grad(h, B, 1, (float)B, lr, mom, false);
@@ -507,6 +539,21 @@
                      "are invalid, chained launches are now off for this handle", (unsigned)st[1], expect);
         }
     }
+    if (h->tail.status) {
+        int st[2] = {0, 0};
+        BM_HIP(hipMemcpy(st, h->tail.status, sizeof(st), hipMemcpyDeviceToHost));
+        const long long expect = h->tail.items_expected & 0xffffffffLL;
+        if (st[0] != 0 || (long long)(unsigned)st[1] != expect) {
+            h->tail.mode = 0;
+            h->tail.items_expected = 0;
+            BM_HIP(hipMemset(h->tail.status, 0, sizeof(st)));
+            BM_CHECK(st[0] == 0, "fused update-tail launch failed (status %d: %s); the results since the last check are "
+                     "invalid, fused tail launches are now off for this handle", st[0],
+                     st[0] == CHAIN_ERR_TIMEOUT ? "a wait for a producing tile expired" : "not an 8-XCD device");
+            BM_CHECK(false, "fused update-tail launches completed %u work items, expected %lld; the results since the last check "
+                     "are invalid, fused tail launches are now off for this handle", (unsigned)st[1], expect);
+        }
+    }
     return 0;
 }
 
@@ -626,6 +673,12 @@
     BM_HIP(hipEventSynchronize(sg.ev));
     const size_t need = (size_t)h->V * h->H * sizeof(float);
     if (!h->stage_host) BM_TRY(create(h->stage_host, (size_t)h->V * h->H));
+    if (h->tail.status) {
+        BM_HIP(hipMemcpyAsync(h->stage_host, h->tail.status, sizeof(int), hipMemcpyDeviceToHost, h->stage_stream));
+        BM_HIP(hipStreamSynchronize(h->stage_stream));
+        BM_CHECK(*(const int *)h->stage_host.h == 0, "a fused update-tail launch failed (status %d) before this snapshot: "
+                 "it is invalid (bm_rbm_sync reports and recovers)", *(const int *)h->stage_host.h);
+    }
     if (h->chain.status) {
         BM_HIP(hipMemcpyAsync(h->stage_host, h->chain.status, sizeof(int), hipMemcpyDeviceToHost, h->stage_stream));
         BM_HIP(hipStreamSynchronize(h->stage_stream));
@@ -710,7 +763,7 @@
     BM_CHECK(h && out_n && (out4n || max_n == 0), "null argument");
     BM_CHECK(h->mring_n <= max_n, "%d fetches pending, room for %d", h->mring_n, (int)max_n);
     if (h->mring_n > 0 && h->ev_mlast) BM_HIP(hipEventSynchronize(h->ev_mlast));
-    if (h->chain.status || h->xchg_used) {
+    if (h->chain.status || h->tail.status || h->xchg_used) {
         BM_HIP(hipStreamSynchronize(h->stream));
         const int rc = check_device_status(h);
         if (rc) { h->mring_n = 0; *out_n = 0; return rc; }
@@ -924,6 +977,13 @@
     return 0;
 }
 
+int bm_rbm_tail_stats(bm_rbm *h, int64_t *out4) {
+    BM_CHECK(h && out4, "null argument");
+    out4[0] = (int64_t)h->tail.launches; out4[1] = (int64_t)h->tail.items_expected;
+    out4[2] = (int64_t)tail_mode(h->tail, h->chain); out4[3] = (int64_t)h->tail.fallbacks;
+    return 0;
+}
+
 int bm_rbm_timer_start(bm_rbm *h) { BM_HIP(hipEventRecord(h->ev0, h->stream)); return 0; }
 int bm_rbm_timer_mark(bm_rbm *h) { BM_HIP(hipEventRecord(h->ev1, h->stream)); return 0; }
 int bm_rbm_timer_elapsed(bm_rbm *h, float *out_ms) {
diff --git a/boltzmann_machines_amd/csrc/bm_tail.h b/boltzmann_machines_amd/csrc/bm_tail.h
--- /dev/null
+++ b/boltzmann_machines_amd/csrc/bm_tail.h
@@ -0,0 +1,263 @@
+#pragma once
+#include "bm_chain.h"
+
+namespace bm {
+
+struct TailArgs {
+    ChainPhase up;
+    int B, tiles_b;
+    GradArgs g;
+    int ncb, ntv, nvb;
+    int rcap, dbg;
+    unsigned gen;
+    unsigned *flags;
+    unsigned *claim;
+    unsigned *claim_zero;
+    int *status;
+    long long *stamps;
+};
+static_assert(sizeof(TailArgs) <= 4096, "kernel arguments");
+
+template <int NJ> struct TailGradSide : GradSide<NJ> {
+    static constexpr bool kSeg2Wait = true, kCohP2 = true;
+    const unsigned *wflags;
+    int nwait;
+    unsigned gen;
+    int *status;
+    long long *stamp;
+    unsigned *claim;
+    unsigned nxt;
+    __device__ __forceinline__ void wait_seg2() {
+        if (stamp && threadIdx.x == 0) stamp[1] = wall_clock64();
+        if (wflags) {
+            const int lane = threadIdx.x & 63;
+            unsigned spins = 0;
+            for (;;) {
+                unsigned v = gen;
+                if (lane < nwait) v = __hip_atomic_load(wflags + lane, __ATOMIC_RELAXED, __HIP_MEMORY_SCOPE_AGENT);
+                if (__all(v == gen)) break;
+                __builtin_amdgcn_s_sleep(1);
+                if ((++spins & 1023u) == 0) {
+                    const int st = __hip_atomic_load(status, __ATOMIC_RELAXED, __HIP_MEMORY_SCOPE_AGENT);
+                    if (st || spins > (1u << 21)) {
+                        if (lane == 0 && !st) atomicExch(status, CHAIN_ERR_TIMEOUT);
+                        break;
+                    }
+                }
+            }
+        }
+        if (stamp && threadIdx.x == 0) stamp[2] = wall_clock64();
+    }
+    __device__ __forceinline__ void drain() {
+        GradSide<NJ>::drain();
+        if (threadIdx.x == 0) nxt = __hip_atomic_fetch_add(claim, 1u, __ATOMIC_RELAXED, __HIP_MEMORY_SCOPE_AGENT);
+        if (stamp && threadIdx.x == 0) stamp[3] = wall_clock64();
+    }
+};
+
+__device__ __forceinline__ void tail_wait_block(const unsigned *wflags, int nwait, unsigned gen, int *status) {
+    if ((threadIdx.x >> 6) == 0) {
+        const int lane = threadIdx.x & 63;
+        unsigned spins = 0;
+        for (;;) {
+            unsigned v = gen;
+            if (lane < nwait) v = __hip_atomic_load(wflags + lane, __ATOMIC_RELAXED, __HIP_MEMORY_SCOPE_AGENT);
+            if (__all(v == gen)) break;
+            __builtin_amdgcn_s_sleep(1);
+            if ((++spins & 1023u) == 0) {
+                const int st = __hip_atomic_load(status, __ATOMIC_RELAXED, __HIP_MEMORY_SCOPE_AGENT);
+                if (st || spins > (1u << 21)) {
+                    if (lane == 0 && !st) atomicExch(status, CHAIN_ERR_TIMEOUT);
+                    break;
+                }
+            }
+        }
+    }
+    wg_barrier();
+}
+
+template <class GG, int STG, int PL, class A>
+__global__ __launch_bounds__(GG::NT, 1) void tail_kernel(A c) {
+    using GP = GeoChain;
+    static_assert(GP::NT == GG::NT, "one workgroup size for both tile bodies");
+    static_assert(GP::SMEM_FLOATS <= GG::SMEM_FLOATS && CS_SMEM_FLOATS <= GG::SMEM_FLOATS, "one LDS allocation: the larger image");
+    static_assert(GG::TI == 64 && GG::TJ == 64 && GP::TI == 32 && GP::TJ == 64, "tile extents");
+    __shared__ __attribute__((aligned(16))) float smem[GG::SMEM_FLOATS];
+    __shared__ unsigned s_claim;
+    const int tid = threadIdx.x;
+    unsigned xcc_reg;
+    asm volatile("s_getreg_b32 %0, hwreg(HW_REG_XCC_ID)" : "=s"(xcc_reg));
+    const int team = (int)(xcc_reg & 7u);
+    if ((xcc_reg & 0xfu) > 7u) {
+        if (tid == 0) atomicExch(c.status, CHAIN_ERR_XCC);
+        return;
+    }
+    if (blockIdx.x == 0 && tid < 8) c.claim_zero[tid * 32] = 0u;
+    unsigned *my_claim = c.claim + team * 32;
+    if (tid == 0) s_claim = __hip_atomic_fetch_add(my_claim, 1u, __ATOMIC_RELAXED, __HIP_MEMORY_SCOPE_AGENT);
+    __syncthreads();
+    int n = (int)s_claim;
+    const int R = (c.ncb - team + 7) >> 3;
+    const int per = 2 * c.tiles_b;
+    const int nA = R * per, nB = R * c.ntv, nV = (c.nvb - team + 7) >> 3;
+    const int total = nA + nB + R + nV;
+    int nitems = 0;
+    while (n < total) {
+        unsigned nxt = 0;
+        long long *stp = c.stamps ? c.stamps + ((size_t)blockIdx.x * 16 + (nitems < 15 ? nitems : 15)) * 8 : nullptr;
+        if (stp && tid == 0) { stp[0] = wall_clock64(); stp[6] = (long long)n; stp[7] = (long long)team; }
+        if (n < nA) {
+            const int r = small_div(n, per), q = n - r * per;
+            const int ih = q >= c.tiles_b ? 1 : 0, tj = q - ih * c.tiles_b;
+            const int i0 = (team + 8 * r) * 64 + ih * GP::TI;
+            if (stp && tid == 0) stp[5] = 0;
+            if (i0 < c.up.I) {
+                const ChainPhase &ph = c.up;
+                ActArgs a{};
+                a.P1 = ph.P; a.Q1 = ph.Q; a.K1 = ph.K; a.p_xm = ph.p_xm;
+                a.I = ph.I; a.J = c.B;
+                a.bias = ph.bias; a.sigma = ph.sigma; a.mult = ph.mult; a.bmult = ph.bmult; a.kind = ph.kind; a.sample = ph.sample;
+                a.means = ph.means; a.states = ph.states; a.negmeans = ph.negmeans; a.ldo = ph.ldo;
+                a.key = ph.key; a.row0 = ph.row0;
+                chain_tile<GP, PL, true>(a, i0, tj * GP::TJ, smem, nullptr, 0, c.gen, c.status, stp, 0, my_claim, nxt);
+            } else if (tid == 0) {
+                nxt = __hip_atomic_fetch_add(my_claim, 1u, __ATOMIC_RELAXED, __HIP_MEMORY_SCOPE_AGENT);
+            }
+            asm volatile("s_waitcnt vmcnt(0)" ::: "memory");
+            if (tid == 0) s_claim = nxt;
+            wg_barrier();
+            if (tid == 0) __hip_atomic_store(c.flags + (size_t)(team * c.rcap + r) * CHAIN_MAXTI + q, c.gen, __ATOMIC_RELAXED, __HIP_MEMORY_SCOPE_AGENT);
+        } else if (n < nA + nB) {
+            const int m = n - nA, r = small_div(m, c.ntv), tv = m - r * c.ntv;
+            if (stp && tid == 0) stp[5] = 1;
+            TailGradSide<GG::NJ> side;
+            side.wflags = (c.dbg & 2) ? nullptr : c.flags + (size_t)(team * c.rcap + r) * CHAIN_MAXTI;
+            side.nwait = per; side.gen = c.gen; side.status = c.status; side.stamp = stp; side.claim = my_claim; side.nxt = 0;
+            grad_tile<GG, true, 0, STG>(c.g, (team + 8 * r) * GG::TI, tv * GG::TJ, smem, side);
+            if (tid == 0) s_claim = side.nxt;
+            wg_barrier();
+        } else {
+            const int m = n - nA - nB;
+            if (tid == 0) nxt = __hip_atomic_fetch_add(my_claim, 1u, __ATOMIC_RELAXED, __HIP_MEMORY_SCOPE_AGENT);
+            if (stp && tid == 0) stp[5] = m < R ? 2 : 3;
+            int wv;
+            if (m < R) {
+                if (!(c.dbg & 2)) tail_wait_block(c.flags + (size_t)(team * c.rcap + m) * CHAIN_MAXTI, per, c.gen, c.status);
+                wv = c.nvb + team + 8 * m;
+            } else wv = team + 8 * (m - R);
+            if (stp && tid == 0) stp[2] = wall_clock64();
+            if (tid < NT) rbm_bias_fused_block(c.g.bias, wv, smem);
+            else for (int r0 = 0; r0 < c.B; r0 += CS_ROWS) { wg_barrier(); wg_barrier(); }
+            if (tid == 0) s_claim = nxt;
+            wg_barrier();
+        }
+        if (stp && tid == 0) stp[4] = wall_clock64();
+        n = (int)s_claim;
+        ++nitems;
+    }
+    if (tid == 0 && nitems) atomicAdd(c.status + 1, nitems);
+}
+
+struct TailState {
+    unsigned *flags = nullptr, *claim = nullptr;
+    int *status = nullptr;
+    int rcap = 0;
+    unsigned gen = 0;
+    unsigned launches = 0;
+    long long items_expected = 0;
+    long long fallbacks = 0;
+    int mode = -1;
+    long long *stamps = nullptr;
+    static constexpr int CLAIM_SLOTS = ChainState::CLAIM_SLOTS;
+    static constexpr size_t STAMP_WORDS = ChainState::STAMP_WORDS;
+    TailState() = default;
+    TailState(const TailState &) = delete;
+    TailState &operator=(const TailState &) = delete;
+    ~TailState() { release(); }
+    void release() {
+        if (stamps) {
+            const char *f = bm::dbg("tail_stamps");
+            std::vector<long long> hst(STAMP_WORDS);
+            if (f && hipMemcpy(hst.data(), stamps, STAMP_WORDS * 8, hipMemcpyDeviceToHost) == hipSuccess) {
+                FILE *fp = fopen(f, "wb");
+                if (fp) { fwrite(hst.data(), 8, STAMP_WORDS, fp); fclose(fp); }
+            }
+            (void)hipFree(stamps); stamps = nullptr;
+        }
+        if (flags) (void)hipFree(flags);
+        if (claim) (void)hipFree(claim);
+        if (status) (void)hipFree(status);
+        flags = claim = nullptr; status = nullptr;
+    }
+};
+
+static inline int tail_mode(TailState &ts, ChainState &cs) {
+    if (ts.mode < 0) {
+        const char *e = bm::dbg("tail");
+        ts.mode = e ? atoi(e) : 1;
+        (void)chain_mode(cs);
+        if (!cs.dev_ok) ts.mode = 0;
+    }
+    return ts.mode;
+}
+
+static inline bool tail_shape_ok(const ActArgs &up, const GradArgs &g) {
+    using GP = GeoChain;
+    if (!chain_phase_ok(up) || !up.negmeans || up.means || up.states) return false;
+    if (up.negmeans != g.Pneg.ptr || up.I != g.I || up.J != g.Kneg || up.J != g.Kpos) return false;
+    if (g.form != 0 || !g.fused || g.pen) return false;
+    if (!(operand_fast(g.Ppos, KM, g.Kpos) && operand_fast(g.Qpos, KM, g.Kpos) &&
+          operand_fast(g.Pneg, KM, g.Kneg) && operand_fast(g.Qneg, KM, g.Kneg))) return false;
+    if ((g.I + 63) / 64 < 8) return false;
+    if (2 * ((up.J + GP::TJ - 1) / GP::TJ) > CHAIN_MAXTI) return false;
+    return true;
+}
+
+static inline bool tail_launch(TailState &ts, int ncu, const ActArgs &up, const GradArgs &g, int geo, hipStream_t st) {
+    if (!tail_geo_ok(geo)) return false;
+    TailArgs c;
+    memset(&c, 0, sizeof(c));
+    c.ncb = (g.I + 63) / 64; c.ntv = (g.J + 63) / 64; c.nvb = (g.bias.u.V + 63) / 64;
+    c.B = up.J; c.tiles_b = (up.J + GeoChain::TJ - 1) / GeoChain::TJ;
+    const int rcap = (c.ncb + 7) / 8;
+    if (!ts.flags || rcap > ts.rcap) {
+        if (ts.flags) { if (hipStreamSynchronize(st) != hipSuccess) return false; (void)hipFree(ts.flags); ts.flags = nullptr; }
+        const size_t nfl = (size_t)8 * rcap * CHAIN_MAXTI;
+        if (hipMalloc((void **)&ts.flags, nfl * 4) != hipSuccess) { (void)hipGetLastError(); return false; }
+        if (hipMemsetAsync(ts.flags, 0, nfl * 4, st) != hipSuccess) return false;
+        ts.rcap = rcap;
+        ts.gen = 0;
+        if (!ts.claim) {
+            const size_t ncl = (size_t)TailState::CLAIM_SLOTS * 8 * 32;
+            if (hipMalloc((void **)&ts.claim, ncl * 4) != hipSuccess) { (void)hipGetLastError(); return false; }
+            if (hipMemsetAsync(ts.claim, 0, ncl * 4, st) != hipSuccess) return false;
+            if (hipMalloc((void **)&ts.status, 2 * sizeof(int)) != hipSuccess) { (void)hipGetLastError(); return false; }
+            if (hipMemsetAsync(ts.status, 0, 2 * sizeof(int), st) != hipSuccess) return false;
+        }
+    }
+    if (++ts.gen == 0) {
+        if (hipMemsetAsync(ts.flags, 0, (size_t)8 * ts.rcap * CHAIN_MAXTI * 4, st) != hipSuccess) return false;
+        ts.gen = 1;
+    }
+    c.rcap = ts.rcap; c.gen = ts.gen; c.flags = ts.flags; c.status = ts.status;
+    c.claim = ts.claim + (size_t)(ts.launches % TailState::CLAIM_SLOTS) * 8 * 32;
+    c.claim_zero = ts.claim + (size_t)((ts.launches + TailState::CLAIM_SLOTS / 2) % TailState::CLAIM_SLOTS) * 8 * 32;
+    ++ts.launches;
+    ChainPhase &ph = c.up;
+    ph.P = up.P1; ph.Q = up.Q1; ph.K = up.K1; ph.p_xm = up.p_xm; ph.I = up.I;
+    ph.bias = up.bias; ph.sigma = up.sigma; ph.mult = up.mult; ph.bmult = up.bmult; ph.kind = up.kind; ph.sample = up.sample;
+    ph.means = up.means; ph.states = up.states; ph.negmeans = up.negmeans; ph.ldo = up.ldo;
+    ph.key = up.key; ph.row0 = up.row0;
+    c.g = g;
+    const int items = c.ncb * (2 * c.tiles_b + c.ntv + 1) + c.nvb;
+    ts.items_expected += items;
+    static const int dbg = bm::dbg("tail_dbg") ? atoi(bm::dbg("tail_dbg")) : 0;
+    if (bm::dbg("tail_stamps") && !ts.stamps && hipMalloc((void **)&ts.stamps, TailState::STAMP_WORDS * 8) != hipSuccess) ts.stamps = nullptr;
+    if (ts.stamps) (void)hipMemsetAsync(ts.stamps, 0, TailState::STAMP_WORDS * 8, st);
+    c.stamps = ts.stamps;
+    c.dbg = dbg;
+    launch_tail_as(geo, c, ncu, st);
+    return true;
+}
+
+}
diff --git a/boltzmann_machines_amd/engine.py b/boltzmann_machines_amd/engine.py
--- a/boltzmann_machines_amd/engine.py
+++ b/boltzmann_machines_amd/engine.py
@@ -150,6 +150,11 @@
         out = (C.c_int64 * 3)()
         check(self.lib.bm_rbm_chain_stats(self._h, out))
         return int(out[0]), int(out[1]), int(out[2])
+
+    def tail_stats(self):
+        out = (C.c_int64 * 4)()
+        check(self.lib.bm_rbm_tail_stats(self._h, out))
+        return tuple(int(v) for v in out)
 
     def profile(self, enable):
         check(self.lib.bm_rbm_profile(self._h, int(bool(enable))))
diff --git a/include/bm355.h b/include/bm355.h
--- a/include/bm355.h
+++ b/include/bm355.h
@@ -89,6 +89,7 @@
 int bm_rbm_kernel_times(bm_rbm *h, float *ms6, int32_t *n6);
 
 int bm_rbm_chain_stats(bm_rbm *h, int64_t *out3);
+int bm_rbm_tail_stats(bm_rbm *h, int64_t *out4);
 
 int bm_rbm_timer_start(bm_rbm *h);
 int bm_rbm_timer_stop(bm_rbm *h, float *out_ms);
```

New measurement: 12090. 0.761x the previous value.
